# gattia/pyfocusr

Hardware: AMD Instinct MI355X
Metric: lowest-k eigenpairs/sec + KNN-correspondence wall-clock, 250k-vertex mesh pair k=5 (higher is better)
Workload: dtype f64

## Files before the change

pyfocusr_amd/csrc/pf_api.hip:

```cpp
#include <stdarg.h>
#include <stdio.h>
#include <stdlib.h>
#include <string.h>

#include <algorithm>
#include <chrono>
#include <mutex>

#include "pf_internal.h"
#include "pf_launch.h"

static thread_local char g_err[1024] = "";
static std::mutex g_ctx_mutex;
static std::vector<pf_ctx*> g_ctxs;

__global__ __launch_bounds__(PF_BLOCK) void k_copy_words(const unsigned long long* __restrict__ src, unsigned long long* __restrict__ dst,
                                                         size_t n) {
    const size_t i = (size_t)blockIdx.x * PF_BLOCK + threadIdx.x;
    if (i < n) dst[i] = src[i];
}

int pf_copy_by_kernel(hipStream_t st, const void* src, void* dst, size_t bytes) {
    if (bytes == 0) return PF_OK;
    const size_t n = (bytes + 7) / 8;
    k_copy_words<<<(unsigned)((n + PF_BLOCK - 1) / PF_BLOCK), PF_BLOCK, 0, st>>>(static_cast<const unsigned long long*>(src),
                                                                                 static_cast<unsigned long long*>(dst), n);
    PF_HIP(hipGetLastError());
    return PF_OK;
}

static pf_ctx* ctx_of_stream(hipStream_t st) {
    std::lock_guard<std::mutex> lk(g_ctx_mutex);
    for (pf_ctx* c : g_ctxs)
        if (c->stream == st || (c->stream_b && c->stream_b == st)) return c;
    return nullptr;
}

int pf_pinned_scratch(pf_ctx* c, size_t bytes, void** out, int which) {
    void*& buf = which == 2 ? c->pinned_scratch_knn : (which ? c->pinned_scratch_b : c->pinned_scratch);
    size_t& have = which == 2 ? c->pinned_scratch_knn_bytes : (which ? c->pinned_scratch_b_bytes : c->pinned_scratch_bytes);
    if (bytes > have) {
        if (buf) {
            PF_HIP(hipStreamSynchronize(c->stream));
            PF_HIP(hipHostFree(buf));
            buf = nullptr;
            have = 0;
        }
        const size_t cap = bytes > ((size_t)1 << 16) ? bytes : ((size_t)1 << 16);
        PF_HIP(hipHostMalloc(&buf, cap, hipHostMallocDefault));
        have = cap;
    }
    *out = buf;
    return PF_OK;
}

hipError_t pf_create_side_stream(hipStream_t* s, bool low) {
    int least = 0, greatest = 0;
    if (hipDeviceGetStreamPriorityRange(&least, &greatest) == hipSuccess && greatest != least) {
        return hipStreamCreateWithPriority(s, hipStreamNonBlocking, low ? least : greatest);
    }
    (void)hipGetLastError();
    return hipStreamCreateWithFlags(s, hipStreamNonBlocking);
}

hipStream_t pf_stream_b(pf_ctx* c) {
    if (!c->stream_b) {
        hipStream_t s = nullptr;
        if (pf_create_side_stream(&s, true) != hipSuccess ||
            hipEventCreateWithFlags(&c->join_ev, hipEventDisableTiming) != hipSuccess ||
            hipEventCreateWithFlags(&c->fork_ev, hipEventDisableTiming) != hipSuccess) {
            (void)hipGetLastError();
            if (s) (void)hipStreamDestroy(s);
            return nullptr;
        }
        std::lock_guard<std::mutex> lk(g_ctx_mutex);
        c->stream_b = s;
    }
    return c->stream_b;
}

hipError_t pf_malloc(hipStream_t st, void** p, size_t bytes) {
    *p = nullptr;
    pf_ctx* c = ctx_of_stream(st);
    if (!c) return hipErrorInvalidValue;
    std::lock_guard<std::mutex> lk(c->alloc_mutex);
    bytes = (std::max<size_t>(bytes, 1) + 255) & ~(size_t)255;
    const auto it = c->free_blocks.lower_bound(bytes);
    if (it != c->free_blocks.end() && it->first == bytes) {
        *p = it->second;
        c->free_blocks.erase(it);
    }
    if (!*p) {
        c->alloc_misses += 1;
        static const bool dbg_alloc = getenv("PF_DEBUG_ALLOC") != nullptr;
        const auto t_miss = std::chrono::steady_clock::now();
        hipError_t e = hipMalloc(p, bytes);
        if (dbg_alloc)
            fprintf(stderr, "libpyfocusr_hip: allocation %lld of ctx %p went to the driver: %zu bytes, %.0f us\n", (long long)c->alloc_misses,
                    (void*)c, bytes, std::chrono::duration<double, std::micro>(std::chrono::steady_clock::now() - t_miss).count());
        if (e != hipSuccess) {
            (void)hipStreamSynchronize(c->stream);
            if (c->stream_b) (void)hipStreamSynchronize(c->stream_b);
            for (auto& kv : c->free_blocks) (void)hipFree(kv.second);
            c->free_blocks.clear();
            e = hipMalloc(p, bytes);
            if (e != hipSuccess) return e;
        }
    }
    c->live_blocks[*p] = bytes;
    return hipSuccess;
}

void pf_free(hipStream_t st, void* p) {
    if (!p) return;
    if (pfl::tl_rec) {
        pfl::tl_rec->frees.emplace_back(st, p);
        return;
    }
    pf_ctx* c = ctx_of_stream(st);
    if (!c) return;
    std::lock_guard<std::mutex> lk(c->alloc_mutex);
    auto it = c->live_blocks.find(p);
    if (it == c->live_blocks.end()) return;
    c->free_blocks.emplace(it->second, p);
    c->live_blocks.erase(it);
}

namespace pfl {

void flush(Recorder& a, Recorder* b) {
    Recorder* const saved = tl_rec;
    tl_rec = nullptr;
    size_t i = 0, j = 0;
    const size_t na = a.ops.size(), nb = b ? b->ops.size() : 0;
    auto alone = [](const Op& o) { o.key ? o.run1(o, o.st) : o.call(o.st); };
    while (i < na && j < nb) {
        const Op& x = a.ops[i];
        const Op& y = b->ops[j];
        if (x.key != y.key) {
            if (!x.key) {
                alone(x);
                ++i;
                continue;
            }
            if (!y.key) {
                alone(y);
                ++j;
                continue;
            }
            break;
        }
        if (x.key && x.st == y.st && x.block.x == y.block.x && x.block.y == y.block.y && x.block.z == y.block.z) {
            x.run2(x, y, x.st);
        } else {
            alone(x);
            alone(y);
        }
        ++i, ++j;
    }
    for (; i < na; ++i) alone(a.ops[i]);
    for (; j < nb; ++j) alone(b->ops[j]);
    a.ops.clear();
    for (auto& f : a.frees) pf_free(f.first, f.second);
    a.frees.clear();
    if (b) {
        b->ops.clear();
        for (auto& f : b->frees) pf_free(f.first, f.second);
        b->frees.clear();
    }
    tl_rec = saved;
}

void flush_self() {
    if (tl_rec) flush(*tl_rec, nullptr);
}

}

// ... 199 lines not shown
```

pyfocusr_amd/csrc/pf_eigs.hip:

```cpp
#include <math.h>

#include <algorithm>
#include <vector>

#include "pf_internal.h"
#include "pf_krylov.h"

namespace {

struct DeviceOps final : pfk::Ops {
    pf_graph* g;
    explicit DeviceOps(pf_graph* graph) : g(graph) {}
    int64_t n() const override { return g->n; }
    int64_t n_isolated() const override { return g->n_isolated; }
    int32_t n_components() const override { return g->n_components; }
    int32_t n_oneway() const override { return g->n_oneway; }
    bool symmetric() const override { return g->is_symmetric; }
    double spectral_bound() const override { return g->spectral_bound; }
    int ws_ensure(int32_t slots) override { return pf_ws_ensure(g, slots); }
    int lock_nulls(int32_t op, int32_t* locked) override { return pf_lock_null_vectors(g, op, locked); }
    int orth_strict(bool on) override { return pf_orth_strict(g, on ? 1 : 0); }
    int orth_always_twice(bool on, bool strict_otherwise) override { return pf_orth_strict(g, on ? 2 : (strict_otherwise ? 1 : 0)); }
    int orth_device_passes(bool on) override { return pf_orth_device_passes(g, on ? 1 : 0); }
    int start_vector(int32_t slot, uint64_t seed) override { return pf_start_vector(g, slot, seed); }
    int orth_begin(int32_t w, int32_t first, int32_t count) override { return pf_orth_begin(g, w, first, count, 1); }
    int orth_end(double* h, double* nrm, bool* redone) override {
        PF_TRY(pf_orth_end(g, h, nrm));
        const int r = pf_orth_redone(g);
        *redone = r == 1;
        last_twice = r == 2;
        return PF_OK;
    }
    int cheb(int32_t op, int32_t src, int32_t dst, int32_t degree, double c, double e, double rho) override {
        return pf_cheb(g, op, src, dst, degree, c, e, rho);
    }
    int combine(int32_t src_first, int32_t m, const double* Y, int32_t k, int32_t dst_first) override {
        return pf_combine(g, src_first, m, Y, k, dst_first);
    }
    int combine2(int32_t src_first, int32_t m, const double* Y, int32_t k, int32_t dst_first, int32_t src_first2, int32_t dst_first2) override {
        return pf_combine2(g, src_first, m, Y, k, dst_first, src_first2, dst_first2);
    }
    int copy(int32_t src, int32_t dst, int32_t count) override { return pf_ws_copy(g, src, dst, count); }
    int spmv_multi(int32_t op, int32_t src_first, int32_t dst_first, int32_t count) override {
        return pf_spmv_multi(g, op, src_first, dst_first, count);
    }
    int gram(int32_t first_a, int32_t count_a, int32_t first_b, int32_t count_b, double* out) override {
        return pf_gram(g, first_a, count_a, first_b, count_b, out);
    }
    int resnorms(int32_t ax_first, int32_t x_first, const double* lam, int32_t count, double* out) override {
        return pf_resnorms(g, ax_first, x_first, lam, count, out);
    }
    int gram_begin(int32_t first_a, int32_t count_a, int32_t first_b, int32_t count_b, bool self_b) override {
        PF_TRY(pf_gram_begin(g, first_a, count_a, first_b, count_b, 0));
        return self_b ? pf_gram_begin(g, first_b, count_b, first_b, count_b, 1) : PF_OK;
    }
    bool orth_split(int32_t first2, int32_t split) override { return pf_orth_split(g, first2, split) == PF_OK; }
    int gram_end(double* out) override { return pf_small_end(g, out); }
    int resnorms_begin(int32_t ax_first, int32_t x_first, const double* lam, int32_t count) override {
        return pf_resnorms_begin(g, ax_first, x_first, lam, count);
    }
    int resnorms_end(double* out) override { return pf_small_end(g, out); }
    int orth_begin_pair(pfk::Ops& other, const int32_t* o) override {
        return pf_orth_begin2(g, o[0], o[1], o[2], o[3], static_cast<DeviceOps&>(other).g, o[4], o[5], o[6], o[7]);
    }
    int cheb_pair(pfk::Ops& other, const int32_t* ci, const double* cd) override {
        return pf_cheb2(g, ci[0], ci[1], ci[2], ci[3], cd[0], cd[1], cd[2], static_cast<DeviceOps&>(other).g, ci[4], ci[5], ci[6], ci[7], cd[3],
                        cd[4], cd[5]);
    }
    int orth_cheb_pair(pfk::Ops& other, const int32_t* orth, const int32_t* ci, const double* cd) override {
        return pf_orth_cheb2(g, static_cast<DeviceOps&>(other).g, orth, ci, cd);
    }
};

int ellipse_hint() {
    const char* ev = getenv("PF_EIGS_ELLIPSE");
    return ev ? atoi(ev) : -1;
}

void give_up(pf_graph* g) {
    if (!g) return;
    if (g->orth_pending >= 0) {
        std::vector<double> h((size_t)g->orth_pending + 1);
        double nrm = 0.0;
        (void)pf_orth_end(g, h.data(), &nrm);
    }
    if (g->small_pending > 0) {
        (void)hipEventSynchronize(g->small_ev);
        g->small_pending = 0;
    }
    (void)pf_download_cancel(g);
}

int finish(pf_graph* g, pfk::Solver& s, int32_t minmax, double* vals, double* vecs, double* residuals, int32_t* n_out, pf_eigs_stats* stats,
           bool async) {
    *n_out = s.n_out;
    for (int i = 0; i < s.n_out; ++i) {
        vals[i] = s.vals[(size_t)i];
        if (residuals) residuals[i] = s.residuals[(size_t)i];
    }
    if (stats) *stats = s.st;
    if (s.n_out > 0) {
        PF_TRY(pf_finalize_vectors_begin(g, s.first_slot, s.n_out, s.sym ? 1 : 0, minmax ? 1 : 0, vecs));
        if (!async) PF_TRY(pf_finalize_vectors_end(g));
    }
    return PF_OK;
}

}

extern "C" int pf_eigs_smallest_ex(pf_graph* g, int32_t n_wanted, int32_t minmax, int32_t async_download, double* vals, double* vecs,
                                   double* residuals, int32_t* n_out, pf_eigs_stats* stats_out) {
    PF_CHECK(g && vals && vecs && n_out && n_wanted >= 1, PF_E_ARG, "pf_eigs_smallest: bad argument");
    int rc = PF_OK;
    for (int attempt = 0; attempt < 3; ++attempt) {
        DeviceOps ops(g);
        pfk::Solver s;
        *n_out = 0;
        rc = s.init(&ops, n_wanted, ellipse_hint());
        if (rc == PF_OK) rc = pfk::drive_single(s);
        if (rc == PF_OK) rc = pf_sync(g->ctx);
        if (rc == PF_OK) rc = finish(g, s, minmax, vals, vecs, residuals, n_out, stats_out, async_download != 0);
        if (rc != PF_OK) give_up(g);
        if (rc != PF_E_PERSIST_TIMEOUT) break;
    }
    return rc;
}

extern "C" int pf_eigs_smallest(pf_graph* g, int32_t n_wanted, int32_t minmax, double* vals, double* vecs, int32_t* n_out,
                                pf_eigs_stats* stats_out) {
    return pf_eigs_smallest_ex(g, n_wanted, minmax, 0, vals, vecs, nullptr, n_out, stats_out);
}

extern "C" int pf_eigs_smallest2(pf_graph* ga, pf_graph* gb, int32_t n_wanted_a, int32_t n_wanted_b, int32_t minmax, int32_t async_download,
                                 double* vals_a, double* vecs_a, double* res_a, int32_t* n_out_a, pf_eigs_stats* stats_a,
                                 double* vals_b, double* vecs_b, double* res_b, int32_t* n_out_b, pf_eigs_stats* stats_b) {
    PF_CHECK(ga && gb && ga != gb && vals_a && vecs_a && n_out_a && vals_b && vecs_b && n_out_b && n_wanted_a >= 1 && n_wanted_b >= 1,
             PF_E_ARG, "pf_eigs_smallest2: bad argument");
    PF_CHECK(ga->ctx == gb->ctx, PF_E_ARG, "pf_eigs_smallest2: the two graphs must share one ctx (stream)");
    int rc = PF_OK;
    for (int attempt = 0; attempt < 3; ++attempt) {
        DeviceOps oa(ga), ob(gb);
        pfk::Solver a, b;
        *n_out_a = *n_out_b = 0;
        rc = a.init(&oa, n_wanted_a, ellipse_hint());
        if (rc == PF_OK) rc = b.init(&ob, n_wanted_b, ellipse_hint());
        if (rc == PF_OK) rc = pfk::drive_pair(a, b);
        if (rc == PF_OK) rc = pf_sync(ga->ctx);
        if (rc == PF_OK) rc = finish(ga, a, minmax, vals_a, vecs_a, res_a, n_out_a, stats_a, async_download != 0);
        if (rc == PF_OK) rc = finish(gb, b, minmax, vals_b, vecs_b, res_b, n_out_b, stats_b, async_download != 0);
        if (rc != PF_OK) {
            give_up(ga);
            give_up(gb);
        }
        if (rc != PF_E_PERSIST_TIMEOUT) break;
    }
    return rc;
}
```

pyfocusr_amd/csrc/pf_krylov.h:

```cpp
#pragma once
#include <math.h>
#include <stdint.h>
#include <stdio.h>
#include <stdlib.h>
#include <time.h>

#include <algorithm>
#include <condition_variable>
#include <memory>
#include <mutex>
#include <thread>
#include <vector>

#include "../../include/pyfocusr_hip.h"
#include "pf_dense.h"

void pf_set_error(const char* fmt, ...);

#define PFK_CHECK(cond, code, ...)       \
    do {                                 \
        if (!(cond)) {                   \
            pf_set_error(__VA_ARGS__);   \
            return (code);               \
        }                                \
    } while (0)
#define PFK_TRY(call)                \
    do {                             \
        int r_ = (call);             \
        if (r_ != PF_OK) return r_;  \
    } while (0)

namespace pfk {

const int NEED_ELLIPSE = 1000;

struct Ops {
    virtual ~Ops() {}
    bool last_twice = false;
    virtual int64_t n() const = 0;
    virtual int64_t n_isolated() const = 0;
    virtual int32_t n_components() const = 0;
    virtual int32_t n_oneway() const = 0;
    virtual bool symmetric() const = 0;
    virtual double spectral_bound() const = 0;
    virtual int ws_ensure(int32_t slots) = 0;
    virtual int lock_nulls(int32_t op, int32_t* locked) = 0;
    virtual int orth_strict(bool on) = 0;
    virtual int orth_device_passes(bool on) { return on ? PF_OK : PF_OK; }
    virtual int start_vector(int32_t slot, uint64_t seed) = 0;
    virtual int orth_begin(int32_t w, int32_t first, int32_t count) = 0;
    virtual int orth_end(double* h, double* nrm, bool* redone) = 0;
    virtual int cheb(int32_t op, int32_t src, int32_t dst, int32_t degree, double c, double e, double rho) = 0;
    virtual int combine(int32_t src_first, int32_t m, const double* Y, int32_t k, int32_t dst_first) = 0;
    virtual int combine2(int32_t src_first, int32_t m, const double* Y, int32_t k, int32_t dst_first, int32_t src_first2, int32_t dst_first2) {
        const int rc = combine(src_first, m, Y, k, dst_first);
        return rc ? rc : combine(src_first2, m, Y, k, dst_first2);
    }
    virtual int copy(int32_t src, int32_t dst, int32_t count) = 0;
    virtual int spmv_multi(int32_t op, int32_t src_first, int32_t dst_first, int32_t count) = 0;
    virtual int gram(int32_t first_a, int32_t count_a, int32_t first_b, int32_t count_b, double* out) = 0;
    virtual int resnorms(int32_t ax_first, int32_t x_first, const double* lam, int32_t count, double* out) = 0;
    virtual int gram_begin(int32_t first_a, int32_t count_a, int32_t first_b, int32_t count_b, bool self_b = false) {
        held.assign((size_t)count_a * count_b + (self_b ? (size_t)count_b * count_b : 0), 0.0);
        const int rc = gram(first_a, count_a, first_b, count_b, held.data());
        if (rc || !self_b) return rc;
        return gram(first_b, count_b, first_b, count_b, held.data() + (size_t)count_a * count_b);
    }
    virtual int gram_end(double* out) {
        std::copy(held.begin(), held.end(), out);
        return 0;
    }
    virtual int resnorms_begin(int32_t ax_first, int32_t x_first, const double* lam, int32_t count) {
        held.assign((size_t)count, 0.0);
        return resnorms(ax_first, x_first, lam, count, held.data());
    }
    virtual int resnorms_end(double* out) {
        std::copy(held.begin(), held.end(), out);
        return 0;
    }
    std::vector<double> held;
    virtual int orth_always_twice(bool on, bool strict_otherwise) {
        (void)on, (void)strict_otherwise;
        return 0;
    }
    virtual bool orth_split(int32_t first2, int32_t split) {
        (void)first2, (void)split;
        return false;
    }
    virtual int orth_begin_pair(Ops& other, const int32_t* orth ) {
        PFK_TRY(orth_begin(orth[0], orth[1], orth[2]));
        return other.orth_begin(orth[4], orth[5], orth[6]);
    }
    virtual int cheb_pair(Ops& other, const int32_t* ci , const double* cd ) {
        PFK_TRY(cheb(ci[0], ci[1], ci[2], ci[3], cd[0], cd[1], cd[2]));
        return other.cheb(ci[4], ci[5], ci[6], ci[7], cd[3], cd[4], cd[5]);
    }
    virtual int orth_cheb_pair(Ops& other, const int32_t* orth, const int32_t* ci, const double* cd) {
        PFK_TRY(orth_begin_pair(other, orth));
        return cheb_pair(other, ci, cd);
    }
};

inline double cheb_value(double lam, double c, double e, int p) {
    const double t = (c - lam) / e;
    if (fabs(t) <= 1.0) return cos(p * acos(t));
    const double s = (t > 0 || p % 2 == 0) ? 1.0 : -1.0;
    return s * cosh(p * acosh(fabs(t)));
}

inline double cheb_value_scaled(double lam, double c, double e, int p, double rho) {
    if (rho == 1.0) return cheb_value(lam, c, e, p);
    const double t = (c - lam) / e;
    if (fabs(t) <= 1.0) return cos(p * acos(t)) * exp(-p * log(rho));
    const double u = acosh(fabs(t));
    const double s = (t > 0 || p % 2 == 0) ? 1.0 : -1.0;
    return s * 0.5 * exp(p * (u - log(rho))) * (1.0 + exp(-2.0 * p * u));
}

inline double cheb_inverse(double theta, double c, double e, int p) { return c - e * cosh(acosh(std::max(theta, 1.0)) / p); }

inline void choose_filter(double cut, double hi, double strength, int max_degree, double* c, double* e, int* p) {
    cut = std::min(std::max(cut, 1e-12), 0.5 * hi);
    *c = 0.5 * (hi + cut);
    *e = 0.5 * (hi - cut);
    const double growth = acosh((*c - 0.5 * cut) / *e);
    *p = std::max(8, std::min(max_degree, (int)ceil(strength / growth)));
}

inline void choose_filter_ellipse(double cut, double half_height, double hi, double strength, int max_degree, double* c, double* e,
                                  int* p, double* rho) {
    cut = std::min(std::max(cut, 1e-12), 0.5 * hi);
    *c = 0.5 * (hi + cut);
    const double a = 0.5 * (hi - cut);
    const double b = std::min(half_height, 0.9 * a);
    *e = sqrt(a * a - b * b);
    *rho = (a + b) / *e;
    const double t = (*c - 0.5 * cut) / *e;
    const double growth = log(t + sqrt(t * t - 1.0)) - log(*rho);
    *p = std::max(8, std::min(max_degree, (int)ceil(strength / std::max(growth, 1e-12))));
}

struct Dominant {
    int q = 0, n_found = 0;
    double thr = -1.0;
    std::vector<int> order;
};

inline Dominant select_dominant(const std::vector<pfd::cplx>& ev, int n_real, int n_extra, bool count_all) {
    Dominant d;
    const int m = (int)ev.size();
    d.order.resize(m);
    for (int i = 0; i < m; ++i) d.order[i] = i;
    std::stable_sort(d.order.begin(), d.order.end(), [&](int a, int b) { return std::abs(ev[a]) > std::abs(ev[b]); });
    std::vector<char> is_real(m);
    std::vector<int> cnt(m);
    int run = 0;
    for (int i = 0; i < m; ++i) {
        const pfd::cplx z = ev[d.order[i]];
        is_real[i] = count_all || (fabs(z.imag()) <= 1e-9 * std::abs(z) && z.real() > 0);
        run += is_real[i] ? 1 : 0;
        cnt[i] = run;
    }
    int q = m;
    for (int i = 0; i < m; ++i)
        if (cnt[i] >= n_real) {
            q = i + 1;
            break;
        }
    int extra = 0;
    while (q < m && extra < n_extra) {
        const pfd::cplx z = ev[d.order[q]];
        const int step = (is_real[q] || fabs(z.imag()) <= 1e-9 * std::abs(z)) ? 1 : 2;
        if (q + step > m) break;
        q += step;
        extra += step;
    }
    if (q < m) {
        double lo = std::abs(ev[d.order[q - 1]]), nx = std::abs(ev[d.order[q]]);
        d.thr = 0.5 * (lo + nx);
        if (lo == nx) {
            q += 1;
            d.thr = q < m ? 0.5 * (std::abs(ev[d.order[q - 1]]) + std::abs(ev[d.order[q]])) : -1.0;
        }
    }
    d.q = q;
    d.n_found = m ? std::min(cnt[m - 1], n_real) : 0;
    return d;
}

enum ReqKind { REQ_NONE = 0, REQ_CHEB, REQ_ORTH, REQ_ORTH_CHEB };

struct Request {
    ReqKind kind = REQ_NONE;
    int32_t cheb_src = 0, cheb_dst = 0;
    int32_t orth_w = 0, orth_first = 0, orth_count = 0;
};

struct Solver {
    Ops* ops = nullptr;
    int32_t n_wanted = 0;
    std::vector<double> vals, residuals;
    int32_t n_out = 0, first_slot = 0;
    pf_eigs_stats st{};
    bool done = false;
    Request req;
    bool req_launched = false;
    bool sym = true;
    int32_t op = PF_OP_SYM;
    double hi = 2.0, strength = 1.8, tol = 1e-12;
    int64_t n_active = 0;
    int c0 = 0, want = 0, q_target = 0, m_max = 0, reg = 0, A0 = 0, B0 = 0;
    int out_cap = 16;
    int m_max_limit = 0;
    bool ellipse = false, interval_tried = false;
    double half_height = 0.0;
    int ellipse_tries = 0, degree_cap = 4000;
    double cut = 0.0, cut0 = 0.0, c = 0.0, e = 0.0, rho = 1.0, theta0 = 0.0, band = 1.5;
    int p = 0;
    uint64_t seed = 0;
    std::vector<double> H, b, h;
    int j = 0, q = 0, restarts = 0, resets = 0;
    bool hess = true;
    bool spec = false, near_conv = false, have_seen = false, start_pending = false;
    bool expect_final = false;
    int next_check = 0, seen_j = 0;
    double seen_worst = 0.0;
    std::vector<double> theta_re, theta_im;
    std::vector<double> U, T;
    double theta_min = 0.0, theta_absmax = 0.0;
    int n_real = 0;
    std::vector<double> res;
    bool analysis_due = false, inline_analysis = true, exhausted = false;
    int outcome = 0, analysis_rc = PF_OK;
    enum { S_TOP, S_AFTER_CHEB, S_AFTER_ORTH, S_AFTER_ANALYSIS, S_EXTRACT_B, S_EXTRACT_C, S_DONE } state = S_TOP;
    bool stepwise_extract = false, extracting = false;
    bool pro = false, pro_local = false;
    int pro_force = 0;
    double pro_thresh = 1e-9;
    std::vector<double> om_prev, om_cur;
    std::vector<double> ex_Rk;
    int ex_nk = 0;

    int init(Ops* o, int32_t wanted, int ellipse_hint = -1) {
        ops = o;
        n_wanted = wanted;
        PFK_CHECK(ops && n_wanted >= 1, PF_E_ARG, "pf_eigs_smallest: bad argument");
        sym = ops->symmetric();
        op = sym ? PF_OP_SYM : PF_OP_RW;
        hi = sym ? ops->spectral_bound() : 2.0;
        strength = 1.8;
        n_active = ops->n() - ops->n_isolated();
        vals.assign((size_t)n_wanted, 0.0);
// ... 568 lines not shown
            std::vector<double> Zs, wr, wi;
            PFK_CHECK(pfd::real_schur(HA, q, Zs, wr, wi), PF_E_DEGENERATE, "pf_eigs_smallest: QR iteration of the Rayleigh quotient failed");
            std::vector<int> all(q);
            for (int i = 0; i < q; ++i) all[i] = i;
            std::vector<pfd::cplx> Vc, lam_c;
            pfd::schur_eigenvectors(HA, Zs, q, all, Vc, lam_c);
            std::vector<int> order(q);
            for (int i = 0; i < q; ++i) order[i] = i;
            std::stable_sort(order.begin(), order.end(), [&](int a, int bb) { return lam_c[a].real() < lam_c[bb].real(); });
            int take = std::min(q_target, q);
            if (take < q && fabs(lam_c[order[take - 1]].imag()) > 1e-9 &&
                fabs(lam_c[order[take - 1]].real() - lam_c[order[take]].real()) <= 1e-9 * fabs(lam_c[order[take]].real()))
                take += 1;
            std::vector<char> is_cplx(take);
            bool any_cplx = false, above = false;
            for (int i = 0; i < take; ++i) {
                const pfd::cplx z = lam_c[order[i]];
                is_cplx[i] = fabs(z.imag()) > 1e-9 * std::max(std::abs(z), 1e-300);
                any_cplx = any_cplx || is_cplx[i];
                above = above || z.real() > cut;
            }
            (void)any_cplx;
            if (ellipse && above) return NEED_ELLIPSE;
            std::vector<int> keep;
            for (int i = 0; i < take; ++i)
                if (lam_c[order[i]].real() > 1e-10) keep.push_back(i);
            st.n_null = std::min(q_target, take) - (int)keep.size();
            nk = (int)keep.size();
            if (nk == 0) return NEED_ELLIPSE;
            nk = std::min(nk, (int)n_wanted);
            Rk.assign((size_t)q * nk, 0.0);
            for (int cidx = 0; cidx < nk; ++cidx) {
                const int col = order[keep[cidx]];
                pfd::cplx phase = 1.0;
                if (is_cplx[keep[cidx]]) {
                    int piv = 0;
                    double best = -1.0;
                    for (int r = 0; r < q; ++r)
                        if (std::abs(Vc[(size_t)r * q + col]) > best) best = std::abs(Vc[(size_t)r * q + col]), piv = r;
                    phase = std::conj(Vc[(size_t)piv * q + col]) / std::abs(Vc[(size_t)piv * q + col]);
                }
                double nrm = 0.0;
                for (int r = 0; r < q; ++r) {
                    const double v = (Vc[(size_t)r * q + col] * phase).real();
                    Rk[(size_t)r * nk + cidx] = v;
                    nrm += v * v;
                }
                nrm = sqrt(nrm);
                for (int r = 0; r < q; ++r) Rk[(size_t)r * nk + cidx] /= nrm;
                vals[cidx] = lam_c[col].real();
            }
        }
        const int X0 = B0 + q, AX0 = A0 + q;
        PFK_CHECK(X0 + nk <= 2 * reg && AX0 + nk <= reg, PF_E_STATE, "pf_eigs_smallest: workspace too small for the extraction");
        n_out = nk;
        first_slot = X0;
        ex_nk = nk;
        if (nk > 0) {
            PFK_TRY(ops->combine2(B0, q, Rk.data(), nk, X0, A0, AX0));
            PFK_TRY(ops->resnorms_begin(AX0, X0, vals.data(), nk));
        }
        return PF_OK;
    }

    int extract_c() {
        if (ex_nk > 0) {
            PFK_TRY(ops->resnorms_end(residuals.data()));
            st.max_residual = 0.0;
            for (int i = 0; i < ex_nk; ++i) st.max_residual = std::max(st.max_residual, residuals[i]);
        }
        return PF_OK;
    }

    void cheb_args(int32_t* ci, double* cd) const {
        ci[0] = op, ci[1] = req.cheb_src, ci[2] = req.cheb_dst, ci[3] = p;
        cd[0] = c, cd[1] = e, cd[2] = rho;
    }
    void orth_args(int32_t* o) const { o[0] = req.orth_w, o[1] = req.orth_first, o[2] = req.orth_count, o[3] = 1; }
    int run_cheb() { return ops->cheb(op, req.cheb_src, req.cheb_dst, p, c, e, rho); }
    int run_orth() { return ops->orth_begin(req.orth_w, req.orth_first, req.orth_count); }
};

inline int drive_single(Solver& s) {
    for (;;) {
        PFK_TRY(s.advance());
        if (s.done) return PF_OK;
        switch (s.req.kind) {
            case REQ_CHEB: PFK_TRY(s.run_cheb()); break;
            case REQ_ORTH: PFK_TRY(s.run_orth()); break;
            case REQ_ORTH_CHEB:
                PFK_TRY(s.run_orth());
                PFK_TRY(s.run_cheb());
                break;
            default: break;
        }
    }
}

struct AnalysisHelper {
    std::thread th;
    std::mutex m;
    std::condition_variable cv;
    Solver* job = nullptr;
    bool busy = false, quit = false;
    AnalysisHelper() { th = std::thread([this] { loop(); }); }
    ~AnalysisHelper() {
        {
            std::lock_guard<std::mutex> lk(m);
            quit = true;
        }
        cv.notify_all();
        th.join();
    }
    void submit(Solver* s) {
        {
            std::lock_guard<std::mutex> lk(m);
            job = s;
            busy = true;
        }
        cv.notify_all();
    }
    void wait() {
        std::unique_lock<std::mutex> lk(m);
        cv.wait(lk, [&] { return !busy; });
    }
    void loop() {
        std::unique_lock<std::mutex> lk(m);
        for (;;) {
            cv.wait(lk, [&] { return job != nullptr || quit; });
            if (quit) return;
            Solver* s = job;
            job = nullptr;
            lk.unlock();
            s->analyse();
            lk.lock();
            busy = false;
            cv.notify_all();
        }
    }
};

inline int launch_request(Solver& s) {
    switch (s.req.kind) {
        case REQ_CHEB: return s.run_cheb();
        case REQ_ORTH: return s.run_orth();
        case REQ_ORTH_CHEB:
            PFK_TRY(s.run_orth());
            return s.run_cheb();
        default: return PF_OK;
    }
}

inline int advance_pair(Solver& a, Solver& b, bool do_a, bool do_b, AnalysisHelper* helper) {
    if (do_a) PFK_TRY(a.advance());
    if (do_b) PFK_TRY(b.advance());
    auto extractions = [&]() -> int {
        for (;;) {
            bool any = false;
            if (do_a && !a.done && a.extracting) {
                PFK_TRY(a.advance());
                any = true;
            }
            if (do_b && !b.done && b.extracting) {
                PFK_TRY(b.advance());
                any = true;
            }
            if (!any) return PF_OK;
        }
    };
    PFK_TRY(extractions());
    for (;;) {
        const bool da = do_a && !a.done && a.analysis_due, db = do_b && !b.done && b.analysis_due;
        if (!da && !db) return PF_OK;
        if (da && db && helper) {
            helper->submit(&b);
            a.analyse();
            helper->wait();
        } else {
            if (da) a.analyse();
            if (db) b.analyse();
        }
        const bool ea = da && a.analysis_rc == PF_OK && a.outcome == 1, eb = db && b.analysis_rc == PF_OK && b.outcome == 1;
        if (ea != eb) {
            Solver& ex = ea ? a : b;
            Solver& other = ea ? b : a;
            const bool other_due = ea ? db : da, other_active = ea ? do_b : do_a;
            if (other_due) PFK_TRY(other.advance());
            if (other_active && !other.done && !other.analysis_due && !other.req_launched && other.req.kind != REQ_NONE) {
                PFK_TRY(launch_request(other));
                other.req_launched = true;
            }
            PFK_TRY(ex.advance());
            PFK_TRY(extractions());
            continue;
        }
        if (da) PFK_TRY(a.advance());
        if (db) PFK_TRY(b.advance());
        PFK_TRY(extractions());
    }
}

inline int drive_pair(Solver& a, Solver& b) {
    std::unique_ptr<AnalysisHelper> helper;
    if ((!a.done && !a.sym) || (!b.done && !b.sym)) {
        if (!getenv("PF_EIGS_HELPER") || atoi(getenv("PF_EIGS_HELPER")) != 0) helper.reset(new AnalysisHelper());
    }
    a.inline_analysis = b.inline_analysis = false;
    a.stepwise_extract = b.stepwise_extract = true;
    PFK_TRY(advance_pair(a, b, !a.done, !b.done, helper.get()));
    while (!a.done || !b.done) {
        if ((!a.done && a.req_launched) || (!b.done && b.req_launched)) {
            Solver& s = (!a.done && a.req_launched) ? a : b;
            s.req_launched = false;
            PFK_TRY(advance_pair(a, b, &s == &a, &s == &b, helper.get()));
            continue;
        }
        const ReqKind ka = a.done ? REQ_NONE : a.req.kind, kb = b.done ? REQ_NONE : b.req.kind;
        const bool oa = ka == REQ_ORTH || ka == REQ_ORTH_CHEB, ob = kb == REQ_ORTH || kb == REQ_ORTH_CHEB;
        int32_t orth[8], ci[8];
        double cd[6];
        if (ka == REQ_ORTH_CHEB && kb == REQ_ORTH_CHEB) {
            a.orth_args(orth);
            b.orth_args(orth + 4);
            a.cheb_args(ci, cd);
            b.cheb_args(ci + 4, cd + 3);
            PFK_TRY(a.ops->orth_cheb_pair(*b.ops, orth, ci, cd));
            PFK_TRY(advance_pair(a, b, true, true, helper.get()));
        } else if (oa || ob) {
            if (oa && ob) {
                a.orth_args(orth);
                b.orth_args(orth + 4);
                PFK_TRY(a.ops->orth_begin_pair(*b.ops, orth));
            } else {
                PFK_TRY((oa ? a : b).run_orth());
            }
            bool adv[2] = {false, false};
            int i = 0;
            for (Solver* s : {&a, &b}) {
                const ReqKind k = s->done ? REQ_NONE : s->req.kind;
                if (k == REQ_ORTH_CHEB && (s == &a ? oa : ob)) s->req.kind = REQ_CHEB;
                else if (k == REQ_ORTH) adv[i] = true;
                ++i;
            }
            PFK_TRY(advance_pair(a, b, adv[0], adv[1], helper.get()));
        } else if (ka == REQ_CHEB && kb == REQ_CHEB) {
            a.cheb_args(ci, cd);
            b.cheb_args(ci + 4, cd + 3);
            PFK_TRY(a.ops->cheb_pair(*b.ops, ci, cd));
            PFK_TRY(advance_pair(a, b, true, true, helper.get()));
        } else {
            Solver& s = ka == REQ_CHEB ? a : b;
            PFK_CHECK(!s.done && s.req.kind == REQ_CHEB, PF_E_STATE, "pf_eigs_smallest2: driver out of step");
            PFK_TRY(s.run_cheb());
            PFK_TRY(advance_pair(a, b, &s == &a, &s == &b, helper.get()));
        }
    }
    return PF_OK;
}

}
```

pyfocusr_amd/csrc/pf_operator.hip:

```cpp
#include <math.h>
#include <stdlib.h>
#include <string.h>

#include <algorithm>
#include <atomic>
#include <map>
#include <mutex>
#include <vector>

#include "pf_internal.h"

namespace {

inline unsigned nblk(int64_t n) { return (unsigned)((n + PF_BLOCK - 1) / PF_BLOCK); }

#ifndef PF_OP_BLOCK
#define PF_OP_BLOCK 256
#endif
struct OpArgs {
    const int64_t* slice_ptr;
    const int32_t* scol;
    const double* sval;
    const double* diag;
    const double* x;
    const double* prev;
    double* out;
    double alpha, shift, beta;
    unsigned n_blocks;
};

template <bool HAS_PREV>
__device__ __forceinline__ void sell_op_block(const OpArgs& a, unsigned bid) {
#pragma clang fp contract(fast)
    const unsigned per_xcd = a.n_blocks >> 3;
    const unsigned blk = (bid & 7u) * per_xcd + (bid >> 3);
    const int64_t row = (int64_t)blk * PF_OP_BLOCK + threadIdx.x;
    const int64_t s = row >> 6;
    const int lane = threadIdx.x & (PF_WAVE - 1);
    const int64_t base = a.slice_ptr[s];
    const int width = (int)((a.slice_ptr[s + 1] - base) >> 6);
    const double* __restrict__ x = a.x;
    const double xi = x[row];
    double acc = a.diag[row] * xi;
    const int pairs = width >> 1;
    const double2* __restrict__ vp2 = reinterpret_cast<const double2*>(a.sval + base) + lane;
    const int2* __restrict__ cp2 = reinterpret_cast<const int2*>(a.scol + base) + lane;
    int j = 0;
    for (; j + 2 <= pairs; j += 2) {
        const int2 c0 = cp2[(int64_t)(j + 0) * PF_WAVE], c1 = cp2[(int64_t)(j + 1) * PF_WAVE];
        const double2 v0 = vp2[(int64_t)(j + 0) * PF_WAVE], v1 = vp2[(int64_t)(j + 1) * PF_WAVE];
        const double x0 = x[c0.x], x1 = x[c0.y], x2 = x[c1.x], x3 = x[c1.y];
        acc += v0.x * x0;
        acc += v0.y * x1;
        acc += v1.x * x2;
        acc += v1.y * x3;
    }
    for (; j < pairs; ++j) {
        const int2 c0 = cp2[(int64_t)j * PF_WAVE];
        const double2 v0 = vp2[(int64_t)j * PF_WAVE];
        acc += v0.x * x[c0.x];
        acc += v0.y * x[c0.y];
    }
    if (width & 1) {
        const int64_t t = base + (int64_t)pairs * (2 * PF_WAVE) + lane;
        acc += a.sval[t] * x[a.scol[t]];
    }
    double r = a.alpha * (a.shift * xi - acc);
    if (HAS_PREV) r -= a.beta * a.prev[row];
    a.out[row] = r;
}

template <bool HAS_PREV>
__global__ __launch_bounds__(PF_OP_BLOCK) void k_sell_op(OpArgs a) {
    sell_op_block<HAS_PREV>(a, blockIdx.x);
}

__global__ __launch_bounds__(PF_OP_BLOCK) void k_sell_op_slots(OpArgs a, int64_t slot_stride) {
    a.x += (int64_t)blockIdx.y * slot_stride;
    a.out += (int64_t)blockIdx.y * slot_stride;
    sell_op_block<false>(a, blockIdx.x);
}

template <bool HAS_PREV>
__global__ __launch_bounds__(PF_OP_BLOCK) void k_sell_op2(OpArgs a, OpArgs b) {
    if (blockIdx.x < a.n_blocks) sell_op_block<HAS_PREV>(a, blockIdx.x);
    else sell_op_block<HAS_PREV>(b, blockIdx.x - a.n_blocks);
}

__global__ __launch_bounds__(PF_BLOCK) void k_dot_partial(const double* __restrict__ ws, int64_t n_pad, int32_t first,
                                                          int32_t wslot, int64_t n_chunks, double* __restrict__ partial,
                                                          int32_t self_col = -1) {
    __shared__ double red[PF_BLOCK / PF_WAVE];
    const int b = blockIdx.y;
    const int64_t chunk = blockIdx.x;
    const double* v = ws + (int64_t)(b == self_col ? wslot : first + b) * n_pad;
    const double* w = ws + (int64_t)wslot * n_pad;
    const int64_t lo = chunk * PF_DOT_CHUNK;
    const int64_t hi = lo + PF_DOT_CHUNK < n_pad ? lo + PF_DOT_CHUNK : n_pad;
    double s = 0.0;
    for (int64_t i = lo + 2 * threadIdx.x; i < hi; i += 2 * PF_BLOCK) {
        const double2 a = *reinterpret_cast<const double2*>(v + i);
        const double2 c = *reinterpret_cast<const double2*>(w + i);
        s += a.x * c.x;
        s += a.y * c.y;
    }
#pragma unroll
    for (int off = PF_WAVE / 2; off > 0; off >>= 1) s += __shfl_down(s, off, PF_WAVE);
    if ((threadIdx.x & (PF_WAVE - 1)) == 0) red[threadIdx.x / PF_WAVE] = s;
    __syncthreads();
    if (threadIdx.x == 0) partial[(int64_t)b * n_chunks + chunk] = (red[0] + red[1]) + (red[2] + red[3]);
}

__global__ __launch_bounds__(PF_WAVE) void k_dot_finish(const double* __restrict__ partial, int64_t n_chunks,
                                                        double* __restrict__ out, double* __restrict__ acc, int accumulate) {
    const int b = blockIdx.x;
    double s = 0.0;
    for (int64_t k = threadIdx.x; k < n_chunks; k += PF_WAVE) s += partial[(int64_t)b * n_chunks + k];
#pragma unroll
    for (int off = PF_WAVE / 2; off > 0; off >>= 1) s += __shfl_down(s, off, PF_WAVE);
    if (threadIdx.x == 0) {
        out[b] = s;
        if (acc) acc[b] = accumulate ? acc[b] + s : s;
    }
}

__global__ __launch_bounds__(PF_BLOCK) void k_multi_axpy(double* __restrict__ ws, int64_t n_pad, int32_t first,
                                                         int32_t count, int32_t wslot, const double* __restrict__ h) {
    const int64_t i = 2 * ((int64_t)blockIdx.x * PF_BLOCK + threadIdx.x);
    if (i >= n_pad) return;
    double2 acc = *reinterpret_cast<double2*>(ws + (int64_t)wslot * n_pad + i);
    for (int b = 0; b < count; ++b) {
        const double hb = h[b];
        const double2 v = *reinterpret_cast<const double2*>(ws + (int64_t)(first + b) * n_pad + i);
        acc.x -= hb * v.x;
        acc.y -= hb * v.y;
    }
    *reinterpret_cast<double2*>(ws + (int64_t)wslot * n_pad + i) = acc;
}

constexpr int PF_ORTH_MAX = 256;
__global__ __launch_bounds__(PF_BLOCK) void k_axpy_finishing(double* __restrict__ ws, int64_t n_pad, int32_t first, int32_t count,
                                                             int32_t wslot, const double* __restrict__ partial, int64_t n_chunks,
                                                             double* __restrict__ hsum, int accumulate) {
    __shared__ double hs[PF_ORTH_MAX];
    const int lane = threadIdx.x & (PF_WAVE - 1);
    for (int b = threadIdx.x / PF_WAVE; b < count; b += PF_BLOCK / PF_WAVE) {
        double s = 0.0;
        for (int64_t k = lane; k < n_chunks; k += PF_WAVE) s += partial[(int64_t)b * n_chunks + k];
#pragma unroll
        for (int off = PF_WAVE / 2; off > 0; off >>= 1) s += __shfl_down(s, off, PF_WAVE);
        if (lane == 0) hs[b] = s;
    }
    __syncthreads();
    if (blockIdx.x == 0)
        for (int b = threadIdx.x; b < count; b += PF_BLOCK) hsum[b] = accumulate ? hsum[b] + hs[b] : hs[b];
    const int64_t i = 2 * ((int64_t)blockIdx.x * PF_BLOCK + threadIdx.x);
    if (i >= n_pad) return;
    double2 acc = *reinterpret_cast<double2*>(ws + (int64_t)wslot * n_pad + i);
    for (int b = 0; b < count; ++b) {
        const double hb = hs[b];
        const double2 v = *reinterpret_cast<const double2*>(ws + (int64_t)(first + b) * n_pad + i);
        acc.x -= hb * v.x;
        acc.y -= hb * v.y;
    }
    *reinterpret_cast<double2*>(ws + (int64_t)wslot * n_pad + i) = acc;
}
struct OrthArgs {
    double* ws;
    int64_t n_pad, n_chunks;
    int32_t first, count, wslot, normalize;
    int32_t split, first2;
    double* partial;
    double* hsum;
    double* nrm2;
    double* host_out;
    double thresh;
    double ticket;
    int32_t pass;
    double* verdict;
    unsigned long long* counter;
    unsigned long long target;
    uint32_t* abort_flag;
    int32_t* host_abort;
};
struct OrthArgs2 {
    OrthArgs g[2];
};
__device__ __forceinline__ int32_t orth_slot(const OrthArgs& a, int b) { return b < a.split ? a.first + b : a.first2 + (b - a.split); }

template <int VB>
__global__ __launch_bounds__(PF_BLOCK) void k_orth_dots(OrthArgs2 a2) {
    __shared__ double red[VB][PF_BLOCK / PF_WAVE];
    const OrthArgs& a = a2.g[blockIdx.z];
    const int b0 = blockIdx.y * VB;
    const int64_t chunk = blockIdx.x;
    if (a.pass < 0 || b0 > a.count || chunk >= a.n_chunks) return;
    if (a.pass == 2 && *a.verdict == 0.0) return;
    const double* w = a.ws + (int64_t)a.wslot * a.n_pad;
    const int64_t lo = chunk * PF_DOT_CHUNK;
    constexpr int PAIRS = PF_DOT_CHUNK / (2 * PF_BLOCK);
    double2 cs[PAIRS], xs[VB][PAIRS];
#pragma unroll
    for (int it = 0; it < PAIRS; ++it) cs[it] = *reinterpret_cast<const double2*>(w + lo + 2 * threadIdx.x + (int64_t)it * (2 * PF_BLOCK));
#pragma unroll
    for (int u = 0; u < VB; ++u) {
        const int b = b0 + u;
        if (b > a.count) continue;
        const double* v = a.ws + (int64_t)(b == a.count ? a.wslot : orth_slot(a, b)) * a.n_pad;
#pragma unroll
        for (int it = 0; it < PAIRS; ++it) xs[u][it] = *reinterpret_cast<const double2*>(v + lo + 2 * threadIdx.x + (int64_t)it * (2 * PF_BLOCK));
    }
#pragma unroll
    for (int u = 0; u < VB; ++u) {
        if (b0 + u > a.count) continue;
        double s = 0.0;
#pragma unroll
        for (int it = 0; it < PAIRS; ++it) {
            s += xs[u][it].x * cs[it].x;
            s += xs[u][it].y * cs[it].y;
        }
#pragma unroll
        for (int off = PF_WAVE / 2; off > 0; off >>= 1) s += __shfl_down(s, off, PF_WAVE);
        if ((threadIdx.x & (PF_WAVE - 1)) == 0) red[u][threadIdx.x / PF_WAVE] = s;
    }
    __syncthreads();
    if (threadIdx.x < VB && b0 + (int)threadIdx.x <= a.count)
        a.partial[(int64_t)(b0 + threadIdx.x) * a.n_chunks + chunk] =
            (red[threadIdx.x][0] + red[threadIdx.x][1]) + (red[threadIdx.x][2] + red[threadIdx.x][3]);
}

template <int P>
__global__ __launch_bounds__(PF_BLOCK) void k_orth_project(OrthArgs2 a2) {
    __shared__ double hs[PF_ORTH_MAX + 1];
    __shared__ double s_scale, s_after, s_redo;
    const OrthArgs& a = a2.g[blockIdx.z];
    if (a.pass < 0 || 2 * (int64_t)blockIdx.x * PF_BLOCK * P >= a.n_pad) return;
    if (a.pass == 2 && *a.verdict == 0.0) return;
    const int lane = threadIdx.x & (PF_WAVE - 1);
    const int32_t count = a.count;
    for (int b = threadIdx.x / PF_WAVE; b < count + 1; b += PF_BLOCK / PF_WAVE) {
        double s = 0.0;
        for (int64_t k = lane; k < a.n_chunks; k += PF_WAVE) s += a.partial[(int64_t)b * a.n_chunks + k];
#pragma unroll
        for (int off = PF_WAVE / 2; off > 0; off >>= 1) s += __shfl_down(s, off, PF_WAVE);
        if (lane == 0) hs[b] = s;
    }
    __syncthreads();
    if (threadIdx.x == 0) {
        double sum = 0.0;
        for (int b = 0; b < count; ++b) sum += hs[b] * hs[b];
        const double before = hs[count], after = before - sum;
        const bool fine = a.pass == 2 ? (after == after) : after >= a.thresh * before;
        s_redo = fine ? (a.pass == 2 ? 2.0 : 0.0) : 1.0;
        s_after = after;
        s_scale = (fine && a.normalize && after > 1e-280) ? 1.0 / sqrt(after) : 1.0;
    }
    __syncthreads();
    if (blockIdx.x == 0) {
        const bool report = !(a.pass == 1 && s_redo != 0.0);
        for (int b = threadIdx.x; b < count; b += PF_BLOCK) {
            const double hb = a.pass == 2 ? a.hsum[b] + hs[b] : hs[b];
            a.hsum[b] = hb;
            if (report) a.host_out[b] = hb;
        }
        if (threadIdx.x == 0) {
            if (a.pass == 1) *a.verdict = s_redo;
            *a.nrm2 = s_after;
            if (report) {
                a.host_out[count] = s_after;
                a.host_out[count + 1] = s_redo;
            }
        }
        __threadfence_system();
        __syncthreads();
        if (threadIdx.x == 0 && report) {
            __hip_atomic_store(a.host_out + count + 2, a.ticket, __ATOMIC_RELEASE, __HIP_MEMORY_SCOPE_SYSTEM);
        }
// ... 84 lines not shown
            __hip_atomic_load(a.abort_flag, __ATOMIC_RELAXED, __HIP_MEMORY_SCOPE_AGENT) != 0u) {
            __hip_atomic_store(a.abort_flag, 1u, __ATOMIC_RELAXED, __HIP_MEMORY_SCOPE_AGENT);
            *a.host_abort = 1;
            return 0;
        }
        __builtin_amdgcn_s_sleep(2);
    }
    return 1;
}

constexpr int PF_ORTH_LOCAL_MAX = 4;
__global__ __launch_bounds__(PF_BLOCK) void k_orth_local(OrthArgs2 a2) {
    __shared__ double red[PF_ORTH_LOCAL_MAX + 1][PF_BLOCK / PF_WAVE];
    __shared__ double hs[PF_ORTH_LOCAL_MAX + 1];
    __shared__ double s_scale, s_after, s_redo;
    __shared__ int s_ok;
    const OrthArgs& a = a2.g[blockIdx.z];
    const int64_t chunk = blockIdx.x;
    if (a.pass < 0 || chunk >= a.n_chunks) return;
    const int32_t count = a.count;
    const int lane = threadIdx.x & (PF_WAVE - 1);
    double* w = a.ws + (int64_t)a.wslot * a.n_pad;
    const int64_t lo = chunk * PF_DOT_CHUNK;
    constexpr int PAIRS = PF_DOT_CHUNK / (2 * PF_BLOCK);
    double2 cs[PAIRS], xs[PF_ORTH_LOCAL_MAX][PAIRS];
#pragma unroll
    for (int it = 0; it < PAIRS; ++it) cs[it] = *reinterpret_cast<const double2*>(w + lo + 2 * threadIdx.x + (int64_t)it * (2 * PF_BLOCK));
#pragma unroll
    for (int u = 0; u < PF_ORTH_LOCAL_MAX; ++u) {
        const double* v = a.ws + (int64_t)orth_slot(a, u < count ? u : count - 1) * a.n_pad;
#pragma unroll
        for (int it = 0; it < PAIRS; ++it) xs[u][it] = *reinterpret_cast<const double2*>(v + lo + 2 * threadIdx.x + (int64_t)it * (2 * PF_BLOCK));
    }
#pragma unroll
    for (int u = 0; u <= PF_ORTH_LOCAL_MAX; ++u) {
        if (u > count) continue;
        double s = 0.0;
#pragma unroll
        for (int it = 0; it < PAIRS; ++it) {
            const double2 x = u == count ? cs[it] : xs[u < PF_ORTH_LOCAL_MAX ? u : 0][it];
            s += x.x * cs[it].x;
            s += x.y * cs[it].y;
        }
#pragma unroll
        for (int off = PF_WAVE / 2; off > 0; off >>= 1) s += __shfl_down(s, off, PF_WAVE);
        if (lane == 0) red[u][threadIdx.x / PF_WAVE] = s;
    }
    __syncthreads();
    if ((int)threadIdx.x <= count) {
        const double p = (red[threadIdx.x][0] + red[threadIdx.x][1]) + (red[threadIdx.x][2] + red[threadIdx.x][3]);
        __hip_atomic_store(reinterpret_cast<unsigned long long*>(a.partial) + (int64_t)threadIdx.x * a.n_chunks + chunk,
                           (unsigned long long)__double_as_longlong(p), __ATOMIC_RELAXED, __HIP_MEMORY_SCOPE_AGENT);
        asm volatile("s_waitcnt vmcnt(0)" ::: "memory");
    }
    __syncthreads();
    if (threadIdx.x == 0) s_ok = orth_meet(a, a.target);
    __syncthreads();
    if (!s_ok) return;
    {
        const int b0 = threadIdx.x / PF_WAVE, b1 = b0 + PF_BLOCK / PF_WAVE;
        double s0 = 0.0, s1 = 0.0;
        for (int64_t k = lane; k < a.n_chunks; k += PF_WAVE) {
            const double x0 = b0 < count + 1 ? __longlong_as_double((long long)__hip_atomic_load(
                                                   reinterpret_cast<unsigned long long*>(a.partial) + (int64_t)b0 * a.n_chunks + k, __ATOMIC_RELAXED,
                                                   __HIP_MEMORY_SCOPE_AGENT))
                                             : 0.0;
            const double x1 = b1 < count + 1 ? __longlong_as_double((long long)__hip_atomic_load(
                                                   reinterpret_cast<unsigned long long*>(a.partial) + (int64_t)b1 * a.n_chunks + k, __ATOMIC_RELAXED,
                                                   __HIP_MEMORY_SCOPE_AGENT))
                                             : 0.0;
            s0 += x0;
            s1 += x1;
        }
#pragma unroll
        for (int off = PF_WAVE / 2; off > 0; off >>= 1) {
            s0 += __shfl_down(s0, off, PF_WAVE);
            s1 += __shfl_down(s1, off, PF_WAVE);
        }
        if (lane == 0 && b0 < count + 1) hs[b0] = s0;
        if (lane == 0 && b1 < count + 1) hs[b1] = s1;
    }
    __syncthreads();
    if (threadIdx.x == 0) {
        double sum = 0.0;
        for (int b = 0; b < count; ++b) sum += hs[b] * hs[b];
        const double before = hs[count], after = before - sum;
        int fine = after >= a.thresh * before ? 1 : 0;
        asm volatile("" : "+v"(fine));
        s_redo = fine ? 0.0 : 1.0;
        s_after = after;
        s_scale = (fine && a.normalize && after > 1e-280) ? 1.0 / sqrt(after) : 1.0;
    }
    __syncthreads();
    if (chunk == 0) {
        for (int b = threadIdx.x; b < count; b += PF_BLOCK) {
            a.hsum[b] = hs[b];
            a.host_out[b] = hs[b];
        }
        if (threadIdx.x == 0) {
            *a.nrm2 = s_after;
            a.host_out[count] = s_after;
            a.host_out[count + 1] = s_redo;
        }
        __threadfence_system();
        __syncthreads();
        if (threadIdx.x == 0) __hip_atomic_store(a.host_out + count + 2, a.ticket, __ATOMIC_RELEASE, __HIP_MEMORY_SCOPE_SYSTEM);
    }
    const double sc = s_scale;
#pragma unroll
    for (int it = 0; it < PAIRS; ++it) {
        double2 acc = cs[it];
#pragma unroll
        for (int u = 0; u < PF_ORTH_LOCAL_MAX; ++u) {
            if (u >= count) continue;
            const double hb = hs[u];
            acc.x -= hb * xs[u][it].x;
            acc.y -= hb * xs[u][it].y;
        }
        acc.x *= sc;
        acc.y *= sc;
        *reinterpret_cast<double2*>(w + lo + 2 * threadIdx.x + (int64_t)it * (2 * PF_BLOCK)) = acc;
    }
}
__global__ __launch_bounds__(PF_BLOCK) void k_scale_finishing(double* __restrict__ x, int64_t n_pad, const double* __restrict__ partial,
                                                              int64_t n_chunks, int normalize, const double* __restrict__ hsum,
                                                              int32_t count, double* __restrict__ nrm2, double* __restrict__ host_out) {
    __shared__ double s_v;
    if (threadIdx.x < PF_WAVE) {
        double s = 0.0;
        for (int64_t k = threadIdx.x; k < n_chunks; k += PF_WAVE) s += partial[k];
#pragma unroll
        for (int off = PF_WAVE / 2; off > 0; off >>= 1) s += __shfl_down(s, off, PF_WAVE);
        if (threadIdx.x == 0) s_v = s;
    }
    __syncthreads();
    const double v = s_v;
    if (blockIdx.x == 0) {
        for (int b = threadIdx.x; b < count; b += PF_BLOCK) host_out[b] = hsum[b];
        if (threadIdx.x == 0) {
            *nrm2 = v;
            host_out[count] = v;
            host_out[count + 1] = 0.0;
        }
    }
    const int64_t i = (int64_t)blockIdx.x * PF_BLOCK + threadIdx.x;
    if (normalize && i < n_pad && v > 1e-280) x[i] *= 1.0 / sqrt(v);
}

__global__ __launch_bounds__(PF_BLOCK) void k_scale(double* __restrict__ x, int64_t n_pad, double alpha) {
    const int64_t i = (int64_t)blockIdx.x * PF_BLOCK + threadIdx.x;
    if (i < n_pad) x[i] *= alpha;
}

__global__ __launch_bounds__(PF_BLOCK) void k_scale_rsqrt(double* __restrict__ x, int64_t n_pad, const double* __restrict__ nrm2) {
    const int64_t i = (int64_t)blockIdx.x * PF_BLOCK + threadIdx.x;
    const double v = *nrm2;
    if (i < n_pad && v > 1e-280) x[i] *= 1.0 / sqrt(v);
}

__global__ __launch_bounds__(PF_BLOCK) void k_mask_isolated(double* __restrict__ x, const int32_t* __restrict__ rowptr,
                                                            const int32_t* __restrict__ perm, int64_t n) {
    const int64_t r = (int64_t)blockIdx.x * PF_BLOCK + threadIdx.x;
    if (r >= n) return;
    const int32_t i = perm[r];
    if (rowptr[i + 1] == rowptr[i]) x[r] = 0.0;
}

__global__ __launch_bounds__(PF_BLOCK) void k_start_vector(double* __restrict__ x, const double* __restrict__ smooth,
                                                           const int32_t* __restrict__ perm, const int32_t* __restrict__ perm_m,
                                                           const int32_t* __restrict__ rowptr,
                                                           int64_t n_pad, unsigned long long seed, double noise) {
    const int64_t r = (int64_t)blockIdx.x * PF_BLOCK + threadIdx.x;
    if (r >= n_pad) return;
    const int32_t i = perm[r];
    const int32_t m = perm_m[r];
    double v = 0.0;
    if (i >= 0 && rowptr[m + 1] > rowptr[m]) {
        unsigned long long z = seed + 0x9E3779B97F4A7C15ull * (unsigned long long)(i + 1);
        z = (z ^ (z >> 30)) * 0xBF58476D1CE4E5B9ull;
        z = (z ^ (z >> 27)) * 0x94D049BB133111EBull;
        z ^= z >> 31;
        const double u = (double)(z >> 11) * (1.0 / 9007199254740992.0) - 0.5;
        v = smooth[r] + noise * u;
    }
    x[r] = v;
}

__global__ __launch_bounds__(PF_BLOCK) void k_permute_in(const double* __restrict__ src_old, const int32_t* __restrict__ perm,
                                                         int64_t n_pad, double* __restrict__ dst_new) {
    const int64_t r = (int64_t)blockIdx.x * PF_BLOCK + threadIdx.x;
    if (r >= n_pad) return;
    const int32_t i = perm[r];
    dst_new[r] = i >= 0 ? src_old[i] : 0.0;
}

__global__ __launch_bounds__(PF_BLOCK) void k_permute_out(const double* __restrict__ ws, int64_t n_pad, int32_t first,
                                                          int32_t count, const int32_t* __restrict__ iperm, int64_t n,
                                                          double* __restrict__ dst_old ) {
    const int64_t i = (int64_t)blockIdx.x * PF_BLOCK + threadIdx.x;
    if (i >= n) return;
    const int64_t r = iperm[i];
    for (int c = 0; c < count; ++c) dst_old[(int64_t)c * n + i] = ws[(int64_t)(first + c) * n_pad + r];
}

__global__ __launch_bounds__(PF_BLOCK) void k_null_vector(double* __restrict__ x, const int32_t* __restrict__ label,
                                                          const int32_t* __restrict__ rowptr,
                                                          const double* __restrict__ deg, const int32_t* __restrict__ perm,
                                                          int64_t n_pad, int32_t root, int32_t sym,
                                                          const double* __restrict__ weight) {
    const int64_t r = (int64_t)blockIdx.x * PF_BLOCK + threadIdx.x;
    if (r >= n_pad) return;
    const int32_t i = perm[r];
    double v = 0.0;
    if (i >= 0 && label[i] == root && rowptr[i + 1] > rowptr[i]) v = weight ? weight[i] : (sym ? sqrt(deg[i] + 1e-8) : 1.0);
    x[r] = v;
}

constexpr int COMBINE_COLS = 8;
__global__ __launch_bounds__(PF_BLOCK) void k_combine(double* __restrict__ ws, int64_t n_pad, int32_t src_first, int32_t m,
                                                      const double* __restrict__ Y, int32_t k, int32_t c0, int32_t ncols,
                                                      int32_t dst_first, int32_t src_first2, int32_t dst_first2) {
    const int64_t i = (int64_t)blockIdx.x * PF_BLOCK + threadIdx.x;
    if (i >= n_pad) return;
    if (blockIdx.y) src_first = src_first2, dst_first = dst_first2;
    double acc[COMBINE_COLS];
#pragma unroll
    for (int c = 0; c < COMBINE_COLS; ++c) acc[c] = 0.0;
    for (int b = 0; b < m; ++b) {
        const double v = ws[(int64_t)(src_first + b) * n_pad + i];
        const double* yr = Y + (int64_t)b * k + c0;
#pragma unroll
        for (int c = 0; c < COMBINE_COLS; ++c)
            if (c < ncols) acc[c] += v * yr[c];
    }
#pragma unroll
    for (int c = 0; c < COMBINE_COLS; ++c)
        if (c < ncols) ws[(int64_t)(dst_first + c0 + c) * n_pad + i] = acc[c];
}

__global__ __launch_bounds__(PF_BLOCK) void k_resnorm_partial(const double* __restrict__ ax, const double* __restrict__ x,
                                                              double lam, int64_t n_pad, int64_t n_chunks,
                                                              double* __restrict__ partial) {
    __shared__ double red[PF_BLOCK / PF_WAVE];
    const int64_t lo = (int64_t)blockIdx.x * PF_DOT_CHUNK;
    const int64_t hi = lo + PF_DOT_CHUNK < n_pad ? lo + PF_DOT_CHUNK : n_pad;
    double s = 0.0;
    for (int64_t i = lo + threadIdx.x; i < hi; i += PF_BLOCK) {
        const double r = ax[i] - lam * x[i];
        s += r * r;
    }
#pragma unroll
    for (int off = PF_WAVE / 2; off > 0; off >>= 1) s += __shfl_down(s, off, PF_WAVE);
    if ((threadIdx.x & (PF_WAVE - 1)) == 0) red[threadIdx.x / PF_WAVE] = s;
    __syncthreads();
    if (threadIdx.x == 0) partial[blockIdx.x] = (red[0] + red[1]) + (red[2] + red[3]);
}

__global__ __launch_bounds__(PF_BLOCK) void k_gram_partial(const double* __restrict__ ws, int64_t n_pad, int32_t first_a, int32_t first_b,
                                                           int32_t count_b, int64_t n_chunks, double* __restrict__ partial) {
    __shared__ double red[PF_BLOCK / PF_WAVE];
    const int p = blockIdx.y;
    const int i = p / count_b, j = p - i * count_b;
    const double* v = ws + (int64_t)(first_b + j) * n_pad;
    const double* w = ws + (int64_t)(first_a + i) * n_pad;
    const int64_t lo = (int64_t)blockIdx.x * PF_DOT_CHUNK;
    const int64_t hi = lo + PF_DOT_CHUNK < n_pad ? lo + PF_DOT_CHUNK : n_pad;
    double s = 0.0;
    for (int64_t r = lo + 2 * threadIdx.x; r < hi; r += 2 * PF_BLOCK) {
        const double2 a = *reinterpret_cast<const double2*>(v + r);
        const double2 c = *reinterpret_cast<const double2*>(w + r);
        s += a.x * c.x;
        s += a.y * c.y;
    }
#pragma unroll
    for (int off = PF_WAVE / 2; off > 0; off >>= 1) s += __shfl_down(s, off, PF_WAVE);
    if ((threadIdx.x & (PF_WAVE - 1)) == 0) red[threadIdx.x / PF_WAVE] = s;
    __syncthreads();
    if (threadIdx.x == 0) partial[(int64_t)p * n_chunks + blockIdx.x] = (red[0] + red[1]) + (red[2] + red[3]);
}

constexpr int PF_RESNORMS_MAX = 64;
struct LamArgs {
    double lam[PF_RESNORMS_MAX];
};
__global__ __launch_bounds__(PF_BLOCK) void k_resnorms_partial(const double* __restrict__ ws, int64_t n_pad, int32_t ax_first,
                                                               int32_t x_first, LamArgs la, int64_t n_chunks,
                                                               double* __restrict__ partial) {
    __shared__ double red[PF_BLOCK / PF_WAVE];
    const int b = blockIdx.y;
    const double* ax = ws + (int64_t)(ax_first + b) * n_pad;
    const double* x = ws + (int64_t)(x_first + b) * n_pad;
    const double lam = la.lam[b];
    const int64_t lo = (int64_t)blockIdx.x * PF_DOT_CHUNK;
    const int64_t hi = lo + PF_DOT_CHUNK < n_pad ? lo + PF_DOT_CHUNK : n_pad;
    double s = 0.0;
    for (int64_t i = lo + threadIdx.x; i < hi; i += PF_BLOCK) {
        const double r = ax[i] - lam * x[i];
        s += r * r;
    }
#pragma unroll
    for (int off = PF_WAVE / 2; off > 0; off >>= 1) s += __shfl_down(s, off, PF_WAVE);
    if ((threadIdx.x & (PF_WAVE - 1)) == 0) red[threadIdx.x / PF_WAVE] = s;
    __syncthreads();
    if (threadIdx.x == 0) partial[(int64_t)b * n_chunks + blockIdx.x] = (red[0] + red[1]) + (red[2] + red[3]);
}

struct VecStats {
    double sumsq, vmin, vmax, absmax, at_absmax;
    int64_t arg;
};

__device__ __forceinline__ void stats_merge(VecStats& a, const VecStats& b) {
    a.sumsq += b.sumsq;
    a.vmin = fmin(a.vmin, b.vmin);
    a.vmax = fmax(a.vmax, b.vmax);
    if (b.absmax > a.absmax || (b.absmax == a.absmax && b.arg < a.arg)) {
        a.absmax = b.absmax;
        a.at_absmax = b.at_absmax;
        a.arg = b.arg;
    }
}

__device__ __forceinline__ VecStats stats_shfl(const VecStats& v, int off) {
    VecStats o;
    o.sumsq = __shfl_down(v.sumsq, off, PF_WAVE);
    o.vmin = __shfl_down(v.vmin, off, PF_WAVE);
    o.vmax = __shfl_down(v.vmax, off, PF_WAVE);
    o.absmax = __shfl_down(v.absmax, off, PF_WAVE);
    o.at_absmax = __shfl_down(v.at_absmax, off, PF_WAVE);
    o.arg = __shfl_down(v.arg, off, PF_WAVE);
    return o;
}

__global__ __launch_bounds__(PF_BLOCK) void k_vec_stats_partial(const double* __restrict__ ws, int64_t n_pad, int64_t n,
                                                                int32_t first, const double* __restrict__ sg,
                                                                const int32_t* __restrict__ perm, const int32_t* __restrict__ perm_m,
                                                                int32_t from_sym, int64_t n_chunks, VecStats* __restrict__ partial) {
    __shared__ VecStats red[PF_BLOCK / PF_WAVE];
    const int b = blockIdx.y;
    const double* x = ws + (int64_t)(first + b) * n_pad;
    const int64_t lo = (int64_t)blockIdx.x * PF_DOT_CHUNK;
    const int64_t hi0 = lo + PF_DOT_CHUNK;
    const int64_t hi = hi0 < n ? hi0 : n;
    VecStats st{0.0, INFINITY, -INFINITY, -1.0, 0.0, (int64_t)1 << 62};
    for (int64_t r = lo + threadIdx.x; r < hi; r += PF_BLOCK) {
        const int64_t i = perm[r];
        double v = x[r];
        if (from_sym) v *= sg[perm_m[r]];
        VecStats e{v * v, v, v, fabs(v), v, i};
        stats_merge(st, e);
    }
#pragma unroll
    for (int off = PF_WAVE / 2; off > 0; off >>= 1) {
        VecStats o = stats_shfl(st, off);
        stats_merge(st, o);
    }
    if ((threadIdx.x & (PF_WAVE - 1)) == 0) red[threadIdx.x / PF_WAVE] = st;
    __syncthreads();
    if (threadIdx.x == 0) {
        VecStats t = red[0];
        stats_merge(t, red[1]);
        stats_merge(t, red[2]);
        stats_merge(t, red[3]);
        partial[(int64_t)b * n_chunks + blockIdx.x] = t;
    }
}

__global__ __launch_bounds__(PF_WAVE) void k_vec_stats_finish(const VecStats* __restrict__ partial, int64_t n_chunks,
                                                              VecStats* __restrict__ out) {
    const int b = blockIdx.x;
    VecStats st{0.0, INFINITY, -INFINITY, -1.0, 0.0, (int64_t)1 << 62};
    for (int64_t k = threadIdx.x; k < n_chunks; k += PF_WAVE) stats_merge(st, partial[(int64_t)b * n_chunks + k]);
#pragma unroll
    for (int off = PF_WAVE / 2; off > 0; off >>= 1) {
        VecStats o = stats_shfl(st, off);
        stats_merge(st, o);
    }
    if (threadIdx.x == 0) out[b] = st;
}

__global__ void k_vec_params(const VecStats* __restrict__ fin, int32_t count, int32_t minmax, double* __restrict__ params) {
    for (int c = threadIdx.x; c < count; c += blockDim.x) {
        const VecStats s = fin[c];
        const double sgn = s.at_absmax < 0.0 ? -1.0 : 1.0;
        const double scale = sgn / sqrt(s.sumsq);
        const double vmin = (sgn > 0 ? s.vmin : s.vmax) * scale;
        const double vmax = (sgn > 0 ? s.vmax : s.vmin) * scale;
        params[4 * c + 0] = scale;
        params[4 * c + 1] = minmax ? vmin : 0.0;
        params[4 * c + 2] = minmax ? (vmax - vmin) : 0.0;
        params[4 * c + 3] = minmax ? 0.5 : 0.0;
    }
}

__global__ __launch_bounds__(PF_BLOCK) void k_vec_apply(const double* __restrict__ ws, int64_t n_pad, int64_t n,
                                                        int32_t first, int32_t count, const double* __restrict__ sg,
                                                        const int32_t* __restrict__ iperm, const int32_t* __restrict__ mrank,
                                                        int32_t from_sym, const double* __restrict__ params, double* __restrict__ out) {
    const int64_t i = (int64_t)blockIdx.x * PF_BLOCK + threadIdx.x;
    if (i >= n) return;
    const int64_t r = iperm[i];
    const double s = from_sym ? sg[mrank ? mrank[i] : i] : 1.0;
    for (int c = 0; c < count; ++c) {
        const double scale = params[4 * c + 0], off = params[4 * c + 1], ptp = params[4 * c + 2], half = params[4 * c + 3];
        double v = (ws[(int64_t)(first + c) * n_pad + r] * s) * scale;
        if (ptp != 0.0) v = (v - off) / ptp - half;
        out[i * count + c] = v;
    }
}

__global__ __launch_bounds__(PF_BLOCK) void k_final_rows(const double* __restrict__ fin, const int64_t* __restrict__ rows, int64_t n_rows,
                                                         int32_t fc, double* __restrict__ out) {
    const int64_t e = (int64_t)blockIdx.x * PF_BLOCK + threadIdx.x;
    if (e >= n_rows * fc) return;
    const int64_t t = e / fc;
    out[e] = fin[rows[t] * fc + (e - t * fc)];
}

__global__ __launch_bounds__(PF_BLOCK) void k_fill_mean_filter(const int32_t* __restrict__ rowptr, const int32_t* __restrict__ col,
                                                               const double* __restrict__ w, const double* __restrict__ deg,
                                                               const int32_t* __restrict__ perm, const int32_t* __restrict__ iperm,
                                                               const int32_t* __restrict__ key, int64_t n_pad,
                                                               const int64_t* __restrict__ slice_ptr,
                                                               int32_t* __restrict__ mf_col, double* __restrict__ mf_val) {
    const int64_t row = (int64_t)blockIdx.x * PF_BLOCK + threadIdx.x;
    if (row >= n_pad) return;
    const int64_t s = row / PF_WAVE;
    const int lane = (int)(row & (PF_WAVE - 1));
    const int32_t width = (int32_t)((slice_ptr[s + 1] - slice_ptr[s]) / PF_WAVE) + 1;
    const int64_t base = slice_ptr[s] + (int64_t)PF_WAVE * s;
    const int32_t i = perm[row];
    int32_t e = 0;
    if (i >= 0) {
        const double dinv = 1.0 / (1.0 + deg[i]);
        bool diag_done = false;
        const int32_t ki = key ? key[i] : i;
        for (int32_t a = rowptr[i + 1] - 1; a >= rowptr[i]; --a) {
            const int32_t j = col[a];
            if (!diag_done && (key ? key[j] : j) < ki) {
                mf_col[base + (int64_t)PF_WAVE * e + lane] = (int32_t)row;
                mf_val[base + (int64_t)PF_WAVE * e + lane] = dinv;
                ++e;
                diag_done = true;
            }
            mf_col[base + (int64_t)PF_WAVE * e + lane] = iperm[j];
            mf_val[base + (int64_t)PF_WAVE * e + lane] = dinv * w[a];
            ++e;
        }
        if (!diag_done) {
            mf_col[base + (int64_t)PF_WAVE * e + lane] = (int32_t)row;
            mf_val[base + (int64_t)PF_WAVE * e + lane] = dinv;
            ++e;
        }
    }
    for (; e < width; ++e) {
        mf_col[base + (int64_t)PF_WAVE * e + lane] = (int32_t)row;
        mf_val[base + (int64_t)PF_WAVE * e + lane] = 0.0;
    }
}

template <int NC>
__global__ __launch_bounds__(PF_BLOCK) void k_mean_filter(const int64_t* __restrict__ slice_ptr, const int32_t* __restrict__ mf_col,
                                                          const double* __restrict__ mf_val, const int32_t* __restrict__ perm,
                                                          int64_t n_pad, int32_t ncols, const double* __restrict__ in,
                                                          double* __restrict__ out) {
    const int64_t row = (int64_t)blockIdx.x * PF_BLOCK + threadIdx.x;
    if (row >= n_pad) return;
    const int64_t s = row / PF_WAVE;
    const int lane = (int)(row & (PF_WAVE - 1));
    const int32_t width = (int32_t)((slice_ptr[s + 1] - slice_ptr[s]) / PF_WAVE) + 1;
    const int64_t base = slice_ptr[s] + (int64_t)PF_WAVE * s + lane;
    const bool real = perm[row] >= 0;
    if constexpr (NC > 0) {
        double acc[NC];
#pragma unroll
        for (int c = 0; c < NC; ++c) acc[c] = 0.0;
        for (int32_t e = 0; e < width; ++e) {
            const int64_t j = mf_col[base + (int64_t)PF_WAVE * e];
            const double v = mf_val[base + (int64_t)PF_WAVE * e];
            if (v != 0.0 || j != row) {
#pragma unroll
                for (int c = 0; c < NC; ++c) acc[c] += v * in[j * NC + c];
            }
        }
#pragma unroll
        for (int c = 0; c < NC; ++c) out[row * NC + c] = real ? acc[c] : 0.0;
    } else {
        for (int32_t c = 0; c < ncols; ++c) {
            double acc = 0.0;
            for (int32_t e = 0; e < width; ++e) {
                const double v = mf_val[base + (int64_t)PF_WAVE * e];
                const int64_t j = mf_col[base + (int64_t)PF_WAVE * e];
                if (v != 0.0 || j != row) acc += v * in[j * ncols + c];
            }
            out[row * ncols + c] = real ? acc : 0.0;
        }
    }
}

__global__ __launch_bounds__(PF_BLOCK) void k_rows_in(const double* __restrict__ src, const int32_t* __restrict__ perm, int64_t n_pad,
                                                      int32_t ncols, double* __restrict__ dst) {
    const int64_t t = (int64_t)blockIdx.x * PF_BLOCK + threadIdx.x;
    if (t >= n_pad * ncols) return;
    const int64_t row = t / ncols;
    const int32_t old = perm[row];
    dst[t] = old >= 0 ? src[(int64_t)old * ncols + (t - row * ncols)] : 0.0;
}
__global__ __launch_bounds__(PF_BLOCK) void k_rows_out(const double* __restrict__ src, const int32_t* __restrict__ iperm, int64_t n,
                                                       int32_t ncols, double* __restrict__ dst) {
    const int64_t t = (int64_t)blockIdx.x * PF_BLOCK + threadIdx.x;
    if (t >= n * ncols) return;
    const int64_t old = t / ncols;
    dst[t] = src[(int64_t)iperm[old] * ncols + (t - old * ncols)];
}

__global__ __launch_bounds__(PF_BLOCK) void k_rows_to_new(const int64_t* __restrict__ old_idx, const int32_t* __restrict__ iperm,
                                                          int64_t cnt, int32_t* __restrict__ new_idx) {
    const int64_t t = (int64_t)blockIdx.x * PF_BLOCK + threadIdx.x;
    if (t < cnt) new_idx[t] = iperm[old_idx[t]];
}
__global__ __launch_bounds__(PF_BLOCK) void k_rows_gather(const double* __restrict__ x, const int32_t* __restrict__ idx, int64_t cnt,
                                                          double* __restrict__ out) {
    const int64_t t = (int64_t)blockIdx.x * PF_BLOCK + threadIdx.x;
    if (t < cnt) out[t] = x[idx[t]];
}
__global__ __launch_bounds__(PF_BLOCK) void k_rows_scatter(double* __restrict__ x, const int32_t* __restrict__ idx, int64_t cnt,
                                                           const double* __restrict__ in) {
    const int64_t t = (int64_t)blockIdx.x * PF_BLOCK + threadIdx.x;
    if (t < cnt) x[idx[t]] = in[t];
}
__global__ __launch_bounds__(PF_BLOCK) void k_rows_gather2(const double* __restrict__ xa, const double* __restrict__ xb,
                                                           const int32_t* __restrict__ idx, int64_t cnt, int64_t stride,
                                                           double* __restrict__ out) {
    const int64_t t = (int64_t)blockIdx.x * PF_BLOCK + threadIdx.x;
    if (t >= cnt) return;
    const int32_t r = idx[t];
    out[t] = xa[r];
    if (xb) out[stride + t] = xb[r];
}
__global__ __launch_bounds__(PF_BLOCK) void k_rows_scatter2(double* __restrict__ xa, double* __restrict__ xb,
                                                            const int32_t* __restrict__ idx, const int64_t* __restrict__ off,
                                                            int64_t cnt, int64_t stride, const double* __restrict__ src) {
    const int64_t t = (int64_t)blockIdx.x * PF_BLOCK + threadIdx.x;
    if (t >= cnt) return;
    const int32_t r = idx[t];
    const int64_t o = off[t];
    xa[r] = src[o];
    if (xb) xb[r] = src[o + stride];
}
__global__ __launch_bounds__(PF_BLOCK) void k_rows_fill(double* __restrict__ x, const int32_t* __restrict__ idx, int64_t cnt,
                                                        double value) {
    const int64_t t = (int64_t)blockIdx.x * PF_BLOCK + threadIdx.x;
    if (t < cnt) x[idx[t]] = value;
}

int stage_ensure(pf_graph* g, int64_t elems) {
    if (elems <= g->stage_cap) return PF_OK;
    pf_free(g->ctx->stream, g->stage);
    g->stage = nullptr;
    g->stage_cap = 0;
    PF_HIP(pf_malloc(g->ctx->stream, (void**)&g->stage, sizeof(double) * (size_t)elems));
    g->stage_cap = elems;
    return PF_OK;
}

int check_slots(pf_graph* g, int32_t first, int32_t count, const char* who) {
    PF_CHECK(g != nullptr, PF_E_ARG, "%s: graph is NULL", who);
    PF_HIP(hipSetDevice(g->ctx->device));
    PF_CHECK(first >= 0 && count >= 0 && first + count <= g->n_slots, PF_E_ARG, "%s: slots [%d,%d) outside workspace of %d",
             who, first, first + count, g->n_slots);
    return PF_OK;
}

const double* op_values(pf_graph* g, int32_t op) {
    if (op == PF_OP_RW) return g->sval_rw;
    if (op == PF_OP_SYM) return g->sval_sym;
    return nullptr;
}

OpArgs op_args(pf_graph* g, const double* vals, const double* x, const double* prev, double* out, double alpha, double shift,
               double beta) {
    return OpArgs{g->slice_ptr, g->scol, vals, g->diag, x, prev, out, alpha, shift, beta, (unsigned)(g->n_pad / PF_OP_BLOCK)};
}

int64_t op_bytes(const pf_graph* g) {
    return 12 * (g->nnz_w + g->n - g->n_isolated) + 20 * g->n + 4;
}

int launch_op(pf_graph* g, const double* vals, const double* x, const double* prev, double* out, double alpha, double shift,
              double beta) {
    hipStream_t st = g->ctx->stream;
    const OpArgs a = op_args(g, vals, x, prev, out, alpha, shift, beta);
    if (prev)
        k_sell_op<true><<<a.n_blocks, PF_OP_BLOCK, 0, st>>>(a);
    else
        k_sell_op<false><<<a.n_blocks, PF_OP_BLOCK, 0, st>>>(a);
    PF_HIP(hipGetLastError());
    return PF_OK;
}

int launch_op2(pf_graph* ga, const OpArgs& a, const OpArgs& b, bool has_prev) {
    hipStream_t st = ga->ctx->stream;
    if (has_prev)
        k_sell_op2<true><<<a.n_blocks + b.n_blocks, PF_OP_BLOCK, 0, st>>>(a, b);
    else
        k_sell_op2<false><<<a.n_blocks + b.n_blocks, PF_OP_BLOCK, 0, st>>>(a, b);
    PF_HIP(hipGetLastError());
    return PF_OK;
}

struct ChebRun {
    pf_graph* g;
    const double* vals;
    const double* src;
    double* dst;
    int32_t degree;
    double c, e, rho;
    const double* yp = nullptr;
    const double* yc = nullptr;
    int32_t done = 0;

    int32_t left() const { return degree - done; }
    double* free_tmp(int which) const {
        for (int t = 0; t < PF_WS_TMPS; ++t) {
            double* b = pf_tmp(g, t);
            if (b != yp && b != yc && which-- == 0) return b;
        }
        return nullptr;
    }
    OpArgs first() {
        double* target = degree == 1 ? dst : pf_tmp(g, 0);
        const OpArgs a = op_args(g, vals, src, nullptr, target, 1.0 / (e * rho), c, 0.0);
        yp = src, yc = target, done = 1;
        return a;
    }
    OpArgs single() {
        double* target = left() == 1 ? dst : free_tmp(0);
        const OpArgs a = op_args(g, vals, yc, yp, target, 2.0 / (e * rho), c, 1.0 / (rho * rho));
        yp = yc, yc = target, done += 1;
        return a;
    }
};

struct OpTimer {
    pf_ctx* c;
    int64_t launches;
    double bytes;
    bool on;
    int64_t persist_steps = 0;
    double lds_bytes = 0.0;
    hipEvent_t e0 = nullptr, e1 = nullptr;
    OpTimer(pf_ctx* ctx, int64_t n, double b) : c(ctx), launches(n), bytes(b), on(ctx->timing) {
        if (on && ctx->timing_stride > 1) on = (ctx->timing_count++ % ctx->timing_stride) == 0;
        if (!on) return;
        if (c->spans_pending.size() >= 4096) (void)pf_timing_collect(c);
        if (!c->spans_free.empty()) {
            e0 = c->spans_free.back().first;
            e1 = c->spans_free.back().second;
            c->spans_free.pop_back();
        } else if (hipEventCreate(&e0) != hipSuccess || hipEventCreate(&e1) != hipSuccess) {
            on = false;
            return;
        }
        hipEventRecord(e0, c->stream);
    }
    int finish() {
        if (!on) return PF_OK;
        PF_HIP(hipEventRecord(e1, c->stream));
        c->spans_pending.push_back({e0, e1, launches, bytes, persist_steps, lds_bytes});
        return PF_OK;
    }
};

int small_to_host(pf_graph* g, const double* d_src, double* out, size_t count) {
    pf_ctx* c = g->ctx;
    hipStream_t st = c->stream;
    const size_t bytes = sizeof(double) * count;
    void* pin = nullptr;
    if (bytes <= ((size_t)1 << 16) && pf_pinned_scratch(c, bytes, &pin) == PF_OK) {
        PF_TRY(pf_copy_by_kernel(st, d_src, pin, bytes));
        PF_HIP(hipStreamSynchronize(st));
        memcpy(out, pin, bytes);
        return PF_OK;
    }
    PF_HIP(hipMemcpyAsync(out, d_src, bytes, hipMemcpyDeviceToHost, st));
    PF_HIP(hipStreamSynchronize(st));
    return PF_OK;
}

int dots_device(pf_graph* g, int32_t w, int32_t first, int32_t count, double* d_out, double* d_acc, int accumulate) {
    hipStream_t st = g->ctx->stream;
    PF_TRY(pf_reduce_ensure(g, count));
    dim3 grid((unsigned)g->n_chunks, (unsigned)count);
    k_dot_partial<<<grid, PF_BLOCK, 0, st>>>(g->ws, g->n_pad, first, w, g->n_chunks, g->partials);
    PF_HIP(hipGetLastError());
    k_dot_finish<<<(unsigned)count, PF_WAVE, 0, st>>>(g->partials, g->n_chunks, d_out, d_acc, accumulate);
    PF_HIP(hipGetLastError());
    return PF_OK;
}

}

int pf_reduce_ensure(pf_graph* g, int32_t count) {
    if (count > g->partial_cap) {
        pf_free(g->ctx->stream, g->partials);
        g->partials = nullptr;
        const int32_t cap = std::max(count, 64);
        PF_HIP(pf_malloc(g->ctx->stream, (void**)&g->partials, sizeof(VecStats) * (size_t)cap * (size_t)(g->n_chunks + 1)));
        g->partial_cap = cap;
    }
    if (count > g->coef_cap) {
        pf_free(g->ctx->stream, g->coef);
        g->coef = nullptr;
        const int32_t cap = std::max(count, 64);
        PF_HIP(pf_malloc(g->ctx->stream, (void**)&g->coef, sizeof(double) * 8 * (size_t)cap));
        g->coef_cap = cap;
    }
    return PF_OK;
}

extern "C" {

int pf_ws_ensure(pf_graph* g, int32_t n_slots) {
    PF_CHECK(g != nullptr && n_slots > 0, PF_E_ARG, "pf_ws_ensure: bad argument");
    if (n_slots <= g->n_slots) return PF_OK;
    PF_HIP(hipSetDevice(g->ctx->device));
    hipStream_t st = g->ctx->stream;
    double* nw = nullptr;
    const size_t bytes = sizeof(double) * (size_t)(n_slots + PF_WS_TMPS) * (size_t)g->n_pad;
    PF_HIP(pf_malloc(st, (void**)&nw, bytes));
    PF_HIP(hipMemsetAsync(nw, 0, bytes, st));
    if (g->ws && g->n_slots > 0)
        PF_HIP(hipMemcpyAsync(nw, g->ws, sizeof(double) * (size_t)g->n_slots * g->n_pad, hipMemcpyDeviceToDevice, st));
    pf_free(st, g->ws);
    g->ws = nw;
    g->n_slots = n_slots;
    return PF_OK;
}

int pf_ws_upload(pf_graph* g, int32_t slot, const double* x) {
    PF_TRY(check_slots(g, slot, 1, "pf_ws_upload"));
    PF_CHECK(x != nullptr, PF_E_ARG, "pf_ws_upload: x is NULL");
    hipStream_t st = g->ctx->stream;
    PF_TRY(stage_ensure(g, g->n));
    PF_HIP(hipMemcpyAsync(g->stage, x, sizeof(double) * g->n, hipMemcpyHostToDevice, st));
    k_permute_in<<<nblk(g->n_pad), PF_BLOCK, 0, st>>>(g->stage, g->perm, g->n_pad, pf_slot(g, slot));
    PF_HIP(hipGetLastError());
    PF_HIP(hipStreamSynchronize(st));
    return PF_OK;
}

int pf_ws_download(pf_graph* g, int32_t first, int32_t count, double* out) {
    PF_TRY(check_slots(g, first, count, "pf_ws_download"));
    PF_CHECK(out != nullptr, PF_E_ARG, "pf_ws_download: out is NULL");
    if (count == 0) return PF_OK;
    hipStream_t st = g->ctx->stream;
    PF_TRY(stage_ensure(g, (int64_t)count * g->n));
    k_permute_out<<<nblk(g->n), PF_BLOCK, 0, st>>>(g->ws, g->n_pad, first, count, g->iperm, g->n, g->stage);
    PF_HIP(hipGetLastError());
    PF_HIP(hipMemcpyAsync(out, g->stage, sizeof(double) * (size_t)count * g->n, hipMemcpyDeviceToHost, st));
    PF_HIP(hipStreamSynchronize(st));
    return pf_persist_check(g->ctx);
}

int pf_ws_copy(pf_graph* g, int32_t src, int32_t dst, int32_t count) {
    PF_TRY(check_slots(g, src, count, "pf_ws_copy"));
    PF_TRY(check_slots(g, dst, count, "pf_ws_copy"));
    PF_CHECK(src + count <= dst || dst + count <= src || src == dst, PF_E_ARG, "pf_ws_copy: overlapping ranges");
    if (src == dst || count == 0) return PF_OK;
    PF_HIP(hipMemcpyAsync(pf_slot(g, dst), pf_slot(g, src), sizeof(double) * (size_t)count * g->n_pad,
                          hipMemcpyDeviceToDevice, g->ctx->stream));
    return PF_OK;
}

int pf_mask_isolated(pf_graph* g, int32_t slot) {
    PF_TRY(check_slots(g, slot, 1, "pf_mask_isolated"));
    if (g->n_isolated == 0) return PF_OK;
    k_mask_isolated<<<nblk(g->n), PF_BLOCK, 0, g->ctx->stream>>>(pf_slot(g, slot), g->rowptr, g->perm_m, g->n);
    PF_HIP(hipGetLastError());
    return PF_OK;
}

int pf_start_vector(pf_graph* g, int32_t slot, uint64_t seed) {
    PF_TRY(check_slots(g, slot, 1, "pf_start_vector"));
    k_start_vector<<<nblk(g->n_pad), PF_BLOCK, 0, g->ctx->stream>>>(pf_slot(g, slot), g->smooth, g->perm, g->perm_m, g->rowptr, g->n_pad,
                                                                    (unsigned long long)seed, 0.5);
    PF_HIP(hipGetLastError());
    return PF_OK;
}

int pf_lock_null_vectors(pf_graph* g, int32_t op, int32_t* n_locked) {
    PF_CHECK(g != nullptr && n_locked != nullptr, PF_E_ARG, "pf_lock_null_vectors: NULL argument");
    PF_HIP(hipSetDevice(g->ctx->device));
    PF_CHECK(op == PF_OP_RW || (op == PF_OP_SYM && g->is_symmetric), PF_E_ARG,
             "pf_lock_null_vectors: operator %d not available (W symmetric: %d)", op, g->is_symmetric);
    const int32_t nc = g->n_components;
    PF_TRY(pf_ws_ensure(g, nc + 1));
    hipStream_t st = g->ctx->stream;
    PF_TRY(pf_reduce_ensure(g, 1));
    for (int32_t c = 0; c < nc; ++c) {
        k_null_vector<<<nblk(g->n_pad), PF_BLOCK, 0, st>>>(pf_slot(g, c), g->label, g->rowptr, g->deg, g->perm_m, g->n_pad,
                                                          g->roots[c], op == PF_OP_SYM && !g->unit_g, g->is_cotan ? g->cot_sqrtm : nullptr);
        PF_HIP(hipGetLastError());
        PF_TRY(dots_device(g, c, c, 1, g->coef, nullptr, 0));
        k_scale_rsqrt<<<nblk(g->n_pad), PF_BLOCK, 0, st>>>(pf_slot(g, c), g->n_pad, g->coef);
        PF_HIP(hipGetLastError());
    }
    *n_locked = nc;
    return PF_OK;
}

int pf_spmv(pf_graph* g, int32_t op, int32_t src, int32_t dst) {
    PF_TRY(check_slots(g, src, 1, "pf_spmv"));
    PF_TRY(check_slots(g, dst, 1, "pf_spmv"));
    const double* vals = op_values(g, op);
    PF_CHECK(vals != nullptr && src != dst, PF_E_ARG, "pf_spmv: operator %d unavailable or src == dst", op);
    OpTimer t(g->ctx, 1, (double)op_bytes(g));
    PF_TRY(launch_op(g, vals, pf_slot(g, src), nullptr, pf_slot(g, dst), -1.0, 0.0, 0.0));
    return t.finish();
}

int pf_spmv_multi(pf_graph* g, int32_t op, int32_t src_first, int32_t dst_first, int32_t count) {
    PF_CHECK(count >= 0, PF_E_ARG, "pf_spmv_multi: negative count");
    PF_TRY(check_slots(g, src_first, count, "pf_spmv_multi"));
    PF_TRY(check_slots(g, dst_first, count, "pf_spmv_multi"));
    const double* vals = op_values(g, op);
    PF_CHECK(vals != nullptr && (src_first + count <= dst_first || dst_first + count <= src_first), PF_E_ARG,
             "pf_spmv_multi: operator %d unavailable or the slot ranges overlap", op);
    if (count == 0) return PF_OK;
    OpTimer t(g->ctx, count, (double)count * (double)op_bytes(g));
    {
        const OpArgs a = op_args(g, vals, pf_slot(g, src_first), nullptr, pf_slot(g, dst_first), -1.0, 0.0, 0.0);
        k_sell_op_slots<<<dim3(a.n_blocks, (unsigned)count), PF_OP_BLOCK, 0, g->ctx->stream>>>(a, g->n_pad);
        PF_HIP(hipGetLastError());
    }
    return t.finish();
}

int pf_cheb(pf_graph* g, int32_t op, int32_t src, int32_t dst, int32_t degree, double c, double e, double rho) {
    PF_TRY(check_slots(g, src, 1, "pf_cheb"));
    PF_TRY(check_slots(g, dst, 1, "pf_cheb"));
    const double* vals = op_values(g, op);
    PF_CHECK(vals != nullptr && src != dst, PF_E_ARG, "pf_cheb: operator %d unavailable or src == dst", op);
    PF_CHECK(degree >= 1 && e > 0.0 && rho >= 1.0, PF_E_ARG, "pf_cheb: degree %d / half-width %g / rho %g invalid", degree, e, rho);
    OpTimer t(g->ctx, degree, (double)degree * op_bytes(g));
    {
        const pf_persist_args pa{g, vals, pf_slot(g, src), pf_slot(g, dst), degree, c, e, rho};
        int done = 0;
        PF_TRY(pf_persist_cheb(&pa, nullptr, &done, &t.lds_bytes));
        if (done) {
            t.launches = 1;
            t.persist_steps = degree;
            return t.finish();
        }
    }
    ChebRun r{g, vals, pf_slot(g, src), pf_slot(g, dst), degree, c, e, rho};
    int64_t launches = 1;
    {
        const OpArgs a = r.first();
        PF_TRY(launch_op(g, a.sval, a.x, a.prev, a.out, a.alpha, a.shift, a.beta));
    }
    while (r.left() > 0) {
        const OpArgs a = r.single();
        PF_TRY(launch_op(g, a.sval, a.x, a.prev, a.out, a.alpha, a.shift, a.beta));
        ++launches;
    }
    t.launches = launches;
    return t.finish();
}

int pf_cheb2(pf_graph* ga, int32_t op_a, int32_t src_a, int32_t dst_a, int32_t degree_a, double c_a, double e_a, double rho_a,
             pf_graph* gb, int32_t op_b, int32_t src_b, int32_t dst_b, int32_t degree_b, double c_b, double e_b, double rho_b) {
    PF_TRY(check_slots(ga, src_a, 1, "pf_cheb2"));
    PF_TRY(check_slots(ga, dst_a, 1, "pf_cheb2"));
    PF_TRY(check_slots(gb, src_b, 1, "pf_cheb2"));
    PF_TRY(check_slots(gb, dst_b, 1, "pf_cheb2"));
    PF_CHECK(ga != gb && ga->ctx == gb->ctx, PF_E_ARG, "pf_cheb2: the two graphs must differ and share one ctx (stream)");
    const double* va = op_values(ga, op_a);
    const double* vb = op_values(gb, op_b);
    PF_CHECK(va && vb && src_a != dst_a && src_b != dst_b, PF_E_ARG, "pf_cheb2: operator unavailable or src == dst");
    PF_CHECK(degree_a >= 1 && degree_b >= 1 && e_a > 0.0 && e_b > 0.0 && rho_a >= 1.0 && rho_b >= 1.0, PF_E_ARG,
             "pf_cheb2: bad degree / half-width / rho");
    OpTimer t(ga->ctx, std::max(degree_a, degree_b), (double)degree_a * op_bytes(ga) + (double)degree_b * op_bytes(gb));
    {
        const pf_persist_args pa{ga, va, pf_slot(ga, src_a), pf_slot(ga, dst_a), degree_a, c_a, e_a, rho_a};
        const pf_persist_args pb{gb, vb, pf_slot(gb, src_b), pf_slot(gb, dst_b), degree_b, c_b, e_b, rho_b};
        int done = 0;
        PF_TRY(pf_persist_cheb(&pa, &pb, &done, &t.lds_bytes));
        if (done) {
            t.launches = 1;
            t.persist_steps = degree_a + degree_b;
            return t.finish();
        }
        int done_a = 0, done_b = 0;
        PF_TRY(pf_persist_cheb(&pa, nullptr, &done_a, &t.lds_bytes, false));
        PF_TRY(pf_persist_cheb(&pb, nullptr, &done_b, &t.lds_bytes, false));
        if (done_a || done_b) {
            t.launches = done_a + done_b;
            t.persist_steps = (done_a ? degree_a : 0) + (done_b ? degree_b : 0);
            for (int q = 0; q < 2; ++q) {
                if (q == 0 ? done_a : done_b) continue;
                ChebRun r = q == 0 ? ChebRun{ga, va, pf_slot(ga, src_a), pf_slot(ga, dst_a), degree_a, c_a, e_a, rho_a}
                                   : ChebRun{gb, vb, pf_slot(gb, src_b), pf_slot(gb, dst_b), degree_b, c_b, e_b, rho_b};
                OpArgs a = r.first();
                PF_TRY(launch_op(r.g, a.sval, a.x, a.prev, a.out, a.alpha, a.shift, a.beta));
                ++t.launches;
                while (r.left() > 0) {
                    a = r.single();
                    PF_TRY(launch_op(r.g, a.sval, a.x, a.prev, a.out, a.alpha, a.shift, a.beta));
                    ++t.launches;
                }
            }
            return t.finish();
        }
    }
    ChebRun ra{ga, va, pf_slot(ga, src_a), pf_slot(ga, dst_a), degree_a, c_a, e_a, rho_a};
    ChebRun rb{gb, vb, pf_slot(gb, src_b), pf_slot(gb, dst_b), degree_b, c_b, e_b, rho_b};
    int64_t launches = 1;
    {
        const OpArgs a = ra.first(), b = rb.first();
        PF_TRY(launch_op2(ga, a, b, false));
    }
    while (ra.left() > 0 || rb.left() > 0) {
        if (ra.left() > 0 && rb.left() > 0) {
            const OpArgs a = ra.single(), b = rb.single();
            PF_TRY(launch_op2(ga, a, b, true));
        } else {
            ChebRun& r = ra.left() > 0 ? ra : rb;
            const OpArgs a = r.single();
            PF_TRY(launch_op(r.g, a.sval, a.x, a.prev, a.out, a.alpha, a.shift, a.beta));
        }
        ++launches;
    }
    t.launches = launches;
    return t.finish();
}

int pf_orth_cheb2(pf_graph* ga, pf_graph* gb, const int32_t* orth, const int32_t* cheb_i, const double* cheb_d) {
    PF_CHECK(ga && gb && orth && cheb_i && cheb_d, PF_E_ARG, "pf_orth_cheb2: NULL argument");
    PF_TRY(pf_orth_begin2(ga, orth[0], orth[1], orth[2], orth[3], gb, orth[4], orth[5], orth[6], orth[7]));
    return pf_cheb2(ga, cheb_i[0], cheb_i[1], cheb_i[2], cheb_i[3], cheb_d[0], cheb_d[1], cheb_d[2], gb, cheb_i[4], cheb_i[5], cheb_i[6],
                    cheb_i[7], cheb_d[3], cheb_d[4], cheb_d[5]);
}

int pf_dots(pf_graph* g, int32_t w, int32_t first, int32_t count, double* out) {
    PF_TRY(check_slots(g, w, 1, "pf_dots"));
    PF_TRY(check_slots(g, first, count, "pf_dots"));
    PF_CHECK(out != nullptr, PF_E_ARG, "pf_dots: out is NULL");
    if (count == 0) return PF_OK;
    PF_TRY(pf_reduce_ensure(g, count));
    PF_TRY(dots_device(g, w, first, count, g->coef, nullptr, 0));
    return small_to_host(g, g->coef, out, (size_t)count);
}

static std::atomic<int> g_orth_one_launch{-1};

static int64_t orth_local_capacity(int device) {
    static std::mutex m;
    static std::map<int, int64_t> cap;
    std::lock_guard<std::mutex> lk(m);
    auto it = cap.find(device);
    if (it != cap.end()) return it->second;
    int64_t c = 0;
    const char* e = getenv("PF_ORTH_LOCAL");
    if (!(e && e[0] == '0')) {
        int per_cu = 0;
        hipDeviceProp_t prop;
        if (hipOccupancyMaxActiveBlocksPerMultiprocessor(&per_cu, reinterpret_cast<const void*>(k_orth_local), PF_BLOCK, 0) == hipSuccess &&
            hipGetDeviceProperties(&prop, device) == hipSuccess)
            c = (int64_t)per_cu * prop.multiProcessorCount;
        else
            (void)hipGetLastError();
    }
    cap[device] = c;
    return c;
}

static int orth_meetings_prepare(pf_graph* g, OrthArgs& a, unsigned long long arrivals, hipStream_t st) {
    pf_ctx* ctx = g->ctx;
    const uint64_t epoch = pf_persist_abort_epoch();
    if (!g->orth_counter) PF_HIP(pf_malloc(st, (void**)&g->orth_counter, sizeof(unsigned long long)));
    if (g->orth_epoch != epoch) {
        PF_HIP(hipMemsetAsync(g->orth_counter, 0, sizeof(unsigned long long), st));
        g->orth_arrivals = 0;
        g->orth_epoch = epoch;
    }
    g->orth_arrivals += arrivals;
    a.counter = g->orth_counter;
    a.target = g->orth_arrivals;
    a.abort_flag = ctx->persist_sync;
    a.host_abort = ctx->persist_abort;
    return PF_OK;
}

static int orth_launch_pass(OrthArgs2& a2, int ng, int64_t n_chunks, int64_t n_pad, int32_t count, hipStream_t st, pf_graph* const* gs = nullptr) {
    bool local = gs != nullptr && count <= PF_ORTH_LOCAL_MAX && count >= 1;
    for (int q = 0; q < ng && local; ++q) local = a2.g[q].pass == 0 && a2.g[q].count <= PF_ORTH_LOCAL_MAX && a2.g[q].count >= 1;
    if (local && g_orth_one_launch.load() != 0 && pf_persist_trusted() && n_chunks * ng <= orth_local_capacity(gs[0]->ctx->device)) {
        PF_TRY(pf_persist_sync_ensure(gs[0]->ctx));
        for (int q = 0; q < ng; ++q) PF_TRY(orth_meetings_prepare(gs[q], a2.g[q], (unsigned long long)gs[q]->n_chunks, st));
        k_orth_local<<<dim3((unsigned)n_chunks, 1u, (unsigned)ng), PF_BLOCK, 0, st>>>(a2);
        PF_HIP(hipGetLastError());
        return PF_OK;
    }
    if (n_pad >= 400000) {
        k_orth_dots<4><<<dim3((unsigned)n_chunks, (unsigned)((count + 1 + 3) / 4), (unsigned)ng), PF_BLOCK, 0, st>>>(a2);
        PF_HIP(hipGetLastError());
        k_orth_project<8><<<dim3((unsigned)(n_pad / (2 * PF_BLOCK * 8)), 1u, (unsigned)ng), PF_BLOCK, 0, st>>>(a2);
    } else {
        k_orth_dots<1><<<dim3((unsigned)n_chunks, (unsigned)(count + 1), (unsigned)ng), PF_BLOCK, 0, st>>>(a2);
        PF_HIP(hipGetLastError());
        k_orth_project<1><<<dim3(nblk(n_pad / 2), 1u, (unsigned)ng), PF_BLOCK, 0, st>>>(a2);
    }
    PF_HIP(hipGetLastError());
    return PF_OK;
}

static int orth_prepare(pf_graph* g, int32_t w, int32_t first, int32_t count, int32_t normalize) {
    const int32_t split_req = g->orth_split, first2_req = g->orth_first2;
    g->orth_split = -1;
    PF_TRY(check_slots(g, w, 1, "pf_orth_begin"));
    if (split_req < 0) PF_TRY(check_slots(g, first, count, "pf_orth_begin"));
    PF_CHECK(g->orth_pending < 0, PF_E_STATE, "pf_orth_begin: a previous pf_orth_begin has not been collected");
    g->orth_split_now = -1;
    if (split_req >= 0) {
        const int32_t split = split_req, first2 = first2_req;
        PF_CHECK(split <= count && count > 0 && count < PF_ORTH_MAX, PF_E_ARG, "pf_orth_split: %d of %d vectors in the first range", split, count);
        PF_TRY(check_slots(g, first, split, "pf_orth_begin"));
        PF_TRY(check_slots(g, first2, count - split, "pf_orth_begin"));
        PF_CHECK((w < first || w >= first + split) && (w < first2 || w >= first2 + count - split), PF_E_ARG, "pf_orth_begin: w inside the basis ranges");
        PF_CHECK(first + split <= first2 || first2 + count - split <= first, PF_E_ARG, "pf_orth_split: overlapping ranges");
        g->orth_split_now = split;
        g->orth_first2_now = first2;
    } else {
        PF_CHECK(w < first || w >= first + count, PF_E_ARG, "pf_orth_begin: w inside the basis range");
    }
    hipStream_t st = g->ctx->stream;
    PF_TRY(pf_reduce_ensure(g, count + 1));
    if (count + 1 > g->orth_host_cap || !g->orth_host) {
        pf_ctx* c = g->ctx;
        if (g->orth_host) {
            PF_HIP(hipStreamSynchronize(st));
            c->pinned_pool.emplace_back(g->orth_host_cap, g->orth_host);
            g->orth_host = nullptr;
        }
        const int32_t cap = std::max(count + 1, 64);
        for (size_t i = 0; i < c->pinned_pool.size(); ++i)
            if (c->pinned_pool[i].first >= cap) {
                g->orth_host_cap = c->pinned_pool[i].first;
                g->orth_host = c->pinned_pool[i].second;
                c->pinned_pool.erase(c->pinned_pool.begin() + (long)i);
                break;
            }
        if (!g->orth_host) {
            PF_HIP(hipHostMalloc((void**)&g->orth_host, sizeof(double) * (size_t)(cap + 2), hipHostMallocDefault));
            g->orth_host_cap = cap;
        }
    }
    if (!g->orth_ev) {
        pf_ctx* c = g->ctx;
        if (!c->event_pool.empty()) {
            g->orth_ev = c->event_pool.back();
            c->event_pool.pop_back();
        } else {
            PF_HIP(hipEventCreateWithFlags(&g->orth_ev, hipEventDisableTiming));
        }
    }
    g->orth_host[count + 1] = 0.0;
    g->orth_host[count + 2] = 0.0;
    g->orth_ticket = 0.0;
    g->orth_w = w, g->orth_first = first, g->orth_normalize = normalize ? 1 : 0;
    return PF_OK;
}

static OrthArgs orth_args(pf_graph* g, int32_t w, int32_t first, int32_t count, int32_t normalize) {
    OrthArgs a{};
    a.ws = g->ws;
    a.n_pad = g->n_pad;
    a.n_chunks = g->n_chunks;
    a.first = first, a.count = count, a.wslot = w, a.normalize = normalize ? 1 : 0;
    a.split = g->orth_split_now >= 0 ? g->orth_split_now : count;
    a.first2 = g->orth_first2_now;
    a.partial = g->partials;
    a.hsum = g->coef + g->coef_cap;
    a.nrm2 = g->coef + 2 * g->coef_cap;
    a.host_out = g->orth_host;
    a.thresh = g->orth_thresh;
    g->orth_serial += 1.0;
    a.ticket = g->orth_serial;
    g->orth_ticket = a.ticket;
    a.pass = g->orth_device_passes ? 1 : 0;
    a.verdict = g->coef + 3 * g->coef_cap;
    return a;
}

int pf_orth_begin(pf_graph* g, int32_t w, int32_t first, int32_t count, int32_t normalize) {
    PF_TRY(orth_prepare(g, w, first, count, normalize));
    hipStream_t st = g->ctx->stream;
    const int32_t cap = g->coef_cap;
    double* hpass = g->coef;
    double* hsum = g->coef + cap;
    double* nrm2 = g->coef + 2 * cap;
    if (count > 0 && count < PF_ORTH_MAX) {
        OrthArgs2 a2{};
        a2.g[0] = orth_args(g, w, first, count, normalize);
        pf_graph* const one[1] = {g};
        PF_TRY(orth_launch_pass(a2, 1, g->n_chunks, g->n_pad, count, st, one));
        if (a2.g[0].pass == 1) {
            a2.g[0].pass = 2;
            PF_TRY(orth_launch_pass(a2, 1, g->n_chunks, g->n_pad, count, st));
        }
    } else if (count == 0) {
        k_dot_partial<<<dim3((unsigned)g->n_chunks, 1u), PF_BLOCK, 0, st>>>(g->ws, g->n_pad, w, w, g->n_chunks, g->partials);
        PF_HIP(hipGetLastError());
        k_scale_finishing<<<nblk(g->n_pad), PF_BLOCK, 0, st>>>(pf_slot(g, w), g->n_pad, g->partials, g->n_chunks, normalize ? 1 : 0,
                                                              hsum, count, nrm2, g->orth_host);
        PF_HIP(hipGetLastError());
    } else {
        for (int pass = 0; pass < 2; ++pass) {
            PF_TRY(dots_device(g, w, first, count, hpass, hsum, pass));
            k_multi_axpy<<<nblk(g->n_pad / 2), PF_BLOCK, 0, st>>>(g->ws, g->n_pad, first, count, w, hpass);
            PF_HIP(hipGetLastError());
        }
        PF_TRY(dots_device(g, w, w, 1, nrm2, nullptr, 0));
        if (normalize) {
            k_scale_rsqrt<<<nblk(g->n_pad), PF_BLOCK, 0, st>>>(pf_slot(g, w), g->n_pad, nrm2);
            PF_HIP(hipGetLastError());
        }
        PF_HIP(hipMemcpyAsync(g->orth_host, hsum, sizeof(double) * count, hipMemcpyDeviceToHost, st));
        PF_HIP(hipMemcpyAsync(g->orth_host + count, nrm2, sizeof(double), hipMemcpyDeviceToHost, st));
    }
    if (g->orth_ticket == 0.0) PF_HIP(hipEventRecord(g->orth_ev, st));
    g->orth_wait = g->orth_ev;
    g->orth_pending = count;
    return PF_OK;
}

int pf_orth_begin2(pf_graph* ga, int32_t w_a, int32_t first_a, int32_t count_a, int32_t normalize_a, pf_graph* gb, int32_t w_b,
                   int32_t first_b, int32_t count_b, int32_t normalize_b) {
    PF_CHECK(ga != nullptr && gb != nullptr && ga != gb, PF_E_ARG, "pf_orth_begin2: two different graphs are needed");
    if (ga->ctx != gb->ctx || count_a <= 0 || count_b <= 0 || count_a >= PF_ORTH_MAX || count_b >= PF_ORTH_MAX) {
        PF_TRY(pf_orth_begin(ga, w_a, first_a, count_a, normalize_a));
        return pf_orth_begin(gb, w_b, first_b, count_b, normalize_b);
    }
    PF_TRY(orth_prepare(ga, w_a, first_a, count_a, normalize_a));
    PF_TRY(orth_prepare(gb, w_b, first_b, count_b, normalize_b));
    hipStream_t st = ga->ctx->stream;
    OrthArgs2 a2{};
    a2.g[0] = orth_args(ga, w_a, first_a, count_a, normalize_a);
    a2.g[1] = orth_args(gb, w_b, first_b, count_b, normalize_b);
    const int64_t chunks2 = std::max(ga->n_chunks, gb->n_chunks), pad2 = std::max(ga->n_pad, gb->n_pad);
    const int32_t count2 = std::max(count_a, count_b);
    pf_graph* const two[2] = {ga, gb};
    PF_TRY(orth_launch_pass(a2, 2, chunks2, pad2, count2, st, two));
    if (a2.g[0].pass == 1 || a2.g[1].pass == 1) {
        for (int q = 0; q < 2; ++q) a2.g[q].pass = a2.g[q].pass == 1 ? 2 : -1;
        PF_TRY(orth_launch_pass(a2, 2, chunks2, pad2, count2, st));
    }
    ga->orth_wait = ga->orth_ev;
    gb->orth_wait = gb->orth_ev;
    ga->orth_pending = count_a;
    gb->orth_pending = count_b;
    return PF_OK;
}

int pf_orth_end(pf_graph* g, double* h, double* nrm) {
    PF_CHECK(g != nullptr && nrm != nullptr, PF_E_ARG, "pf_orth_end: NULL argument");
    PF_CHECK(g->orth_pending >= 0, PF_E_STATE, "pf_orth_end: no pf_orth_begin in flight");
    const int32_t count = g->orth_pending;
    PF_CHECK(h != nullptr || count == 0, PF_E_ARG, "pf_orth_end: h is NULL");
    PF_HIP(hipSetDevice(g->ctx->device));
    if (g->orth_ticket != 0.0) {
        volatile double* ticket = g->orth_host + count + 2;
        bool got = false;
        for (uint64_t spin = 0;; ++spin) {
            if (__atomic_load_n(reinterpret_cast<volatile uint64_t*>(ticket), __ATOMIC_ACQUIRE) ==
                *reinterpret_cast<const uint64_t*>(&g->orth_ticket)) {
                got = true;
                break;
            }
            if ((spin & 0xfff) == 0xfff) {
                const hipError_t q = hipStreamQuery(g->ctx->stream);
                if (q == hipSuccess) {
                    got = __atomic_load_n(reinterpret_cast<volatile uint64_t*>(ticket), __ATOMIC_ACQUIRE) ==
                          *reinterpret_cast<const uint64_t*>(&g->orth_ticket);
                    break;
                }
                if (q != hipErrorNotReady) {
                    g->orth_pending = -1;
                    PF_HIP(q);
                }
            }
            __builtin_ia32_pause();
        }
        if (!got) {
            g->orth_pending = -1;
            PF_TRY(pf_persist_check(g->ctx));
            PF_CHECK(false, PF_E_HIP, "pf_orth_end: the Gram-Schmidt step never reported (launch failure?)");
        }
    } else {
        PF_HIP(hipEventSynchronize(g->orth_wait));
    }
    g->orth_pending = -1;
    g->orth_redone = 0;
    PF_TRY(pf_persist_check(g->ctx));
    g->orth_twice = g->orth_host[count + 1] == 2.0 ? 1 : 0;
    if (g->orth_host[count + 1] == 1.0) {
        hipStream_t st = g->ctx->stream;
        double* hsum = g->coef + g->coef_cap;
        double* nrm2 = g->coef + 2 * g->coef_cap;
        const int32_t w = g->orth_w, first = g->orth_first;
        const int32_t split = g->orth_split_now >= 0 ? g->orth_split_now : count;
        if (split > 0) {
            k_dot_partial<<<dim3((unsigned)g->n_chunks, (unsigned)split), PF_BLOCK, 0, st>>>(g->ws, g->n_pad, first, w, g->n_chunks, g->partials);
            PF_HIP(hipGetLastError());
        }
        if (count > split) {
            k_dot_partial<<<dim3((unsigned)g->n_chunks, (unsigned)(count - split)), PF_BLOCK, 0, st>>>(g->ws, g->n_pad, g->orth_first2_now, w, g->n_chunks,
                                                                                                   g->partials + (size_t)split * g->n_chunks);
            PF_HIP(hipGetLastError());
        }
        if (split > 0) {
            k_axpy_finishing<<<nblk(g->n_pad / 2), PF_BLOCK, 0, st>>>(g->ws, g->n_pad, first, split, w, g->partials, g->n_chunks, hsum, 1);
            PF_HIP(hipGetLastError());
        }
        if (count > split) {
            k_axpy_finishing<<<nblk(g->n_pad / 2), PF_BLOCK, 0, st>>>(g->ws, g->n_pad, g->orth_first2_now, count - split, w,
                                                                      g->partials + (size_t)split * g->n_chunks, g->n_chunks, hsum + split, 1);
            PF_HIP(hipGetLastError());
        }
        k_dot_partial<<<dim3((unsigned)g->n_chunks, 1u), PF_BLOCK, 0, st>>>(g->ws, g->n_pad, w, w, g->n_chunks, g->partials);
        PF_HIP(hipGetLastError());
        k_scale_finishing<<<nblk(g->n_pad), PF_BLOCK, 0, st>>>(pf_slot(g, w), g->n_pad, g->partials, g->n_chunks, g->orth_normalize,
                                                              hsum, count, nrm2, g->orth_host);
        PF_HIP(hipGetLastError());
        PF_HIP(hipStreamSynchronize(st));
        PF_TRY(pf_persist_check(g->ctx));
        g->orth_redone = 1;
    }
    for (int32_t b = 0; b < count; ++b) h[b] = g->orth_host[b];
    const double v = g->orth_host[count];
    *nrm = sqrt(v > 0.0 ? v : 0.0);
    return PF_OK;
}

int pf_orth_strict(pf_graph* g, int32_t on) {
    PF_CHECK(g != nullptr, PF_E_ARG, "pf_orth_strict: NULL graph");
    g->orth_thresh = on >= 2 ? 4.0 : (on ? 0.5 : 0.09);
    return PF_OK;
}

int pf_orth_device_passes(pf_graph* g, int32_t on) {
    PF_CHECK(g != nullptr, PF_E_ARG, "pf_orth_device_passes: NULL graph");
    g->orth_device_passes = on ? 1 : 0;
    return PF_OK;
}

int pf_orth_one_launch(int32_t on) {
    g_orth_one_launch.store(on < 0 ? -1 : (on ? 1 : 0));
    return PF_OK;
}

int pf_orth_split(pf_graph* g, int32_t first2, int32_t split) {
    PF_CHECK(g != nullptr && split >= 0 && first2 >= 0, PF_E_ARG, "pf_orth_split: bad argument");
    g->orth_split = split;
    g->orth_first2 = first2;
    return PF_OK;
}

int pf_orth_redone(pf_graph* g) {
    PF_CHECK(g != nullptr, PF_E_ARG, "pf_orth_redone: NULL graph");
    return g->orth_redone ? 1 : (g->orth_twice ? 2 : 0);
}

int pf_orth(pf_graph* g, int32_t w, int32_t first, int32_t count, double* h, double* nrm) {
    PF_CHECK(nrm != nullptr && (h != nullptr || count == 0), PF_E_ARG, "pf_orth: NULL output");
    PF_TRY(pf_orth_begin(g, w, first, count, 0));
    return pf_orth_end(g, h, nrm);
}

int pf_scale(pf_graph* g, int32_t slot, double alpha) {
    PF_TRY(check_slots(g, slot, 1, "pf_scale"));
    k_scale<<<nblk(g->n_pad), PF_BLOCK, 0, g->ctx->stream>>>(pf_slot(g, slot), g->n_pad, alpha);
    PF_HIP(hipGetLastError());
    return PF_OK;
}

int pf_combine(pf_graph* g, int32_t src_first, int32_t m, const double* Y, int32_t k, int32_t dst_first) {
    return pf_combine2(g, src_first, m, Y, k, dst_first, -1, -1);
}

}

int pf_combine2(pf_graph* g, int32_t src_first, int32_t m, const double* Y, int32_t k, int32_t dst_first, int32_t src_first2,
                int32_t dst_first2) {
    PF_TRY(check_slots(g, src_first, m, "pf_combine"));
    PF_TRY(check_slots(g, dst_first, k, "pf_combine"));
    PF_CHECK(Y != nullptr && m > 0 && k > 0, PF_E_ARG, "pf_combine: bad argument");
    PF_CHECK(src_first + m <= dst_first || dst_first + k <= src_first, PF_E_ARG, "pf_combine: overlapping ranges");
    const bool two = src_first2 >= 0;
    if (two) {
        PF_TRY(check_slots(g, src_first2, m, "pf_combine"));
        PF_TRY(check_slots(g, dst_first2, k, "pf_combine"));
        PF_CHECK((src_first2 + m <= dst_first2 || dst_first2 + k <= src_first2) && (dst_first + k <= dst_first2 || dst_first2 + k <= dst_first) &&
                     (src_first + m <= dst_first2 || dst_first2 + k <= src_first) && (src_first2 + m <= dst_first || dst_first + k <= src_first2),
                 PF_E_ARG, "pf_combine: overlapping ranges");
    }
    pf_ctx* ctx = g->ctx;
    hipStream_t st = ctx->stream;
    double* dY = nullptr;
    PF_HIP(pf_malloc(st, (void**)&dY, sizeof(double) * (size_t)m * k));
    const size_t bytes = sizeof(double) * (size_t)m * k;
    const void* src = Y;
    bool staged = false;
    if (bytes <= PF_STAGE_BYTES) {
        if (!ctx->stage_ring) {
            if (hipHostMalloc(&ctx->stage_ring, (size_t)PF_STAGE_SLOTS * PF_STAGE_BYTES, hipHostMallocDefault) != hipSuccess) {
                (void)hipGetLastError();
                ctx->stage_ring = nullptr;
            } else {
                for (int i = 0; i < PF_STAGE_SLOTS; ++i) ctx->stage_ev[i] = nullptr;
            }
        }
        if (ctx->stage_ring) {
            const int slot = ctx->stage_next;
            ctx->stage_next = (slot + 1) % PF_STAGE_SLOTS;
            bool ok = true;
            if (!ctx->stage_ev[slot]) ok = hipEventCreateWithFlags(&ctx->stage_ev[slot], hipEventDisableTiming) == hipSuccess;
            else ok = hipEventSynchronize(ctx->stage_ev[slot]) == hipSuccess;
            if (ok) {
                void* dst = static_cast<unsigned char*>(ctx->stage_ring) + (size_t)slot * PF_STAGE_BYTES;
                memcpy(dst, Y, bytes);
                src = dst;
                staged = true;
                hipError_t es = hipMemcpyAsync(dY, src, bytes, hipMemcpyHostToDevice, st);
                if (es == hipSuccess) es = hipEventRecord(ctx->stage_ev[slot], st);
                if (es != hipSuccess) {
                    pf_free(st, dY);
                    PF_HIP(es);
                }
            } else {
                (void)hipGetLastError();
            }
        }
    }
    hipError_t e = staged ? hipSuccess : hipMemcpyAsync(dY, Y, bytes, hipMemcpyHostToDevice, st);
    for (int32_t c0 = 0; c0 < k && e == hipSuccess; c0 += COMBINE_COLS) {
        const int32_t nc = std::min(COMBINE_COLS, k - c0);
        k_combine<<<dim3(nblk(g->n_pad), two ? 2u : 1u), PF_BLOCK, 0, st>>>(g->ws, g->n_pad, src_first, m, dY, k, c0, nc, dst_first, src_first2,
                                                                          dst_first2);
        e = hipGetLastError();
    }
    hipError_t e2 = staged ? hipSuccess : hipStreamSynchronize(st);
    pf_free(st, dY);
    PF_HIP(e);
    PF_HIP(e2);
    return PF_OK;
}

extern "C" {

int pf_resnorm(pf_graph* g, int32_t ax, int32_t x, double lam, double* out) {
    PF_TRY(check_slots(g, ax, 1, "pf_resnorm"));
    PF_TRY(check_slots(g, x, 1, "pf_resnorm"));
    PF_CHECK(out != nullptr, PF_E_ARG, "pf_resnorm: out is NULL");
    hipStream_t st = g->ctx->stream;
    PF_TRY(pf_reduce_ensure(g, 1));
    k_resnorm_partial<<<(unsigned)g->n_chunks, PF_BLOCK, 0, st>>>(pf_slot(g, ax), pf_slot(g, x), lam, g->n_pad, g->n_chunks, g->partials);
    PF_HIP(hipGetLastError());
    k_dot_finish<<<1, PF_WAVE, 0, st>>>(g->partials, g->n_chunks, g->coef, nullptr, 0);
    PF_HIP(hipGetLastError());
    double r2 = 0.0;
    PF_HIP(hipMemcpyAsync(&r2, g->coef, sizeof(double), hipMemcpyDeviceToHost, st));
    PF_HIP(hipStreamSynchronize(st));
    *out = sqrt(r2 > 0.0 ? r2 : 0.0);
    return PF_OK;
}

int pf_gram(pf_graph* g, int32_t first_a, int32_t count_a, int32_t first_b, int32_t count_b, double* out) {
    PF_TRY(check_slots(g, first_a, count_a, "pf_gram"));
    PF_TRY(check_slots(g, first_b, count_b, "pf_gram"));
    PF_CHECK(out != nullptr && count_a > 0 && count_b > 0, PF_E_ARG, "pf_gram: bad argument");
    PF_TRY(pf_reduce_ensure(g, count_a * count_b));
    hipStream_t st = g->ctx->stream;
    k_gram_partial<<<dim3((unsigned)g->n_chunks, (unsigned)(count_a * count_b)), PF_BLOCK, 0, st>>>(g->ws, g->n_pad, first_a, first_b, count_b,
                                                                                                 g->n_chunks, g->partials);
    PF_HIP(hipGetLastError());
    k_dot_finish<<<(unsigned)(count_a * count_b), PF_WAVE, 0, st>>>(g->partials, g->n_chunks, g->coef, nullptr, 0);
    PF_HIP(hipGetLastError());
    return small_to_host(g, g->coef, out, (size_t)count_a * count_b);
}

}

static int small_begin(pf_graph* g, const double* d_src, size_t count, bool root, bool append = false) {
    PF_CHECK(append ? g->small_pending > 0 && !g->small_root && !root : g->small_pending == 0, PF_E_STATE,
             "pf_gram_begin / pf_resnorms_begin: a previous result has not been collected");
    pf_ctx* c = g->ctx;
    hipStream_t st = c->stream;
    const size_t offset = append ? (size_t)g->small_pending : 0;
    if (append) {
        PF_CHECK((int64_t)(offset + count) <= g->small_host_cap, PF_E_STATE, "pf_gram_begin: no room to append");
    } else if ((int64_t)(2 * count) > g->small_host_cap || !g->small_host) {
        if (g->small_host) {
            PF_HIP(hipStreamSynchronize(st));
            c->pinned_pool.emplace_back(g->small_host_cap, g->small_host);
            g->small_host = nullptr;
        }
        const int32_t cap = std::max((int32_t)(2 * count), 128);
        for (size_t i = 0; i < c->pinned_pool.size(); ++i)
            if (c->pinned_pool[i].first >= cap) {
                g->small_host_cap = c->pinned_pool[i].first;
                g->small_host = c->pinned_pool[i].second;
                c->pinned_pool.erase(c->pinned_pool.begin() + (long)i);
                break;
            }
        if (!g->small_host) {
            PF_HIP(hipHostMalloc((void**)&g->small_host, sizeof(double) * (size_t)(cap + 2), hipHostMallocDefault));
            g->small_host_cap = cap;
        }
    }
    if (!g->small_ev) {
        if (!c->event_pool.empty()) {
            g->small_ev = c->event_pool.back();
            c->event_pool.pop_back();
        } else {
            PF_HIP(hipEventCreateWithFlags(&g->small_ev, hipEventDisableTiming));
        }
    }
    PF_TRY(pf_copy_by_kernel(st, d_src, g->small_host + offset, sizeof(double) * count));
    PF_HIP(hipEventRecord(g->small_ev, st));
    g->small_pending = (int32_t)(offset + count);
    g->small_root = root;
    return PF_OK;
}

int pf_small_end(pf_graph* g, double* out) {
    PF_CHECK(g != nullptr && out != nullptr && g->small_pending > 0, PF_E_STATE, "pf_small_end: nothing to collect");
    PF_HIP(hipEventSynchronize(g->small_ev));
    const int32_t count = g->small_pending;
    g->small_pending = 0;
    for (int32_t i = 0; i < count; ++i) {
        const double v = g->small_host[i];
        out[i] = g->small_root ? sqrt(v > 0.0 ? v : 0.0) : v;
    }
    return PF_OK;
}

int pf_gram_begin(pf_graph* g, int32_t first_a, int32_t count_a, int32_t first_b, int32_t count_b, int32_t append) {
    PF_TRY(check_slots(g, first_a, count_a, "pf_gram"));
    PF_TRY(check_slots(g, first_b, count_b, "pf_gram"));
    PF_CHECK(count_a > 0 && count_b > 0, PF_E_ARG, "pf_gram: bad argument");
    PF_TRY(pf_reduce_ensure(g, count_a * count_b));
    hipStream_t st = g->ctx->stream;
    k_gram_partial<<<dim3((unsigned)g->n_chunks, (unsigned)(count_a * count_b)), PF_BLOCK, 0, st>>>(g->ws, g->n_pad, first_a, first_b, count_b,
                                                                                                 g->n_chunks, g->partials);
    PF_HIP(hipGetLastError());
    k_dot_finish<<<(unsigned)(count_a * count_b), PF_WAVE, 0, st>>>(g->partials, g->n_chunks, g->coef, nullptr, 0);
    PF_HIP(hipGetLastError());
    return small_begin(g, g->coef, (size_t)count_a * count_b, false, append != 0);
}

int pf_resnorms_begin(pf_graph* g, int32_t ax_first, int32_t x_first, const double* lam, int32_t count) {
    PF_TRY(check_slots(g, ax_first, count, "pf_resnorms"));
    PF_TRY(check_slots(g, x_first, count, "pf_resnorms"));
    PF_CHECK(lam != nullptr && count > 0, PF_E_ARG, "pf_resnorms: bad argument");
    hipStream_t st = g->ctx->stream;
    PF_TRY(pf_reduce_ensure(g, count));
    for (int32_t at = 0; at < count; at += PF_RESNORMS_MAX) {
        const int32_t nb = std::min(count - at, PF_RESNORMS_MAX);
        LamArgs la{};
        for (int32_t i = 0; i < nb; ++i) la.lam[i] = lam[at + i];
        k_resnorms_partial<<<dim3((unsigned)g->n_chunks, (unsigned)nb), PF_BLOCK, 0, st>>>(g->ws, g->n_pad, ax_first + at, x_first + at, la,
                                                                                        g->n_chunks, g->partials);
        PF_HIP(hipGetLastError());
        k_dot_finish<<<(unsigned)nb, PF_WAVE, 0, st>>>(g->partials, g->n_chunks, g->coef + at, nullptr, 0);
        PF_HIP(hipGetLastError());
    }
    return small_begin(g, g->coef, (size_t)count, true);
}

extern "C" {

int pf_resnorms(pf_graph* g, int32_t ax_first, int32_t x_first, const double* lam, int32_t count, double* out) {
    PF_TRY(check_slots(g, ax_first, count, "pf_resnorms"));
    PF_TRY(check_slots(g, x_first, count, "pf_resnorms"));
    PF_CHECK(out != nullptr && lam != nullptr && count > 0, PF_E_ARG, "pf_resnorms: bad argument");
    hipStream_t st = g->ctx->stream;
    PF_TRY(pf_reduce_ensure(g, count));
    for (int32_t at = 0; at < count; at += PF_RESNORMS_MAX) {
        const int32_t nb = std::min(count - at, PF_RESNORMS_MAX);
        LamArgs la{};
        for (int32_t i = 0; i < nb; ++i) la.lam[i] = lam[at + i];
        k_resnorms_partial<<<dim3((unsigned)g->n_chunks, (unsigned)nb), PF_BLOCK, 0, st>>>(g->ws, g->n_pad, ax_first + at, x_first + at, la,
                                                                                        g->n_chunks, g->partials);
        PF_HIP(hipGetLastError());
        k_dot_finish<<<(unsigned)nb, PF_WAVE, 0, st>>>(g->partials, g->n_chunks, g->coef + at, nullptr, 0);
        PF_HIP(hipGetLastError());
    }
    PF_TRY(small_to_host(g, g->coef, out, (size_t)count));
    for (int32_t i = 0; i < count; ++i) out[i] = sqrt(out[i] > 0.0 ? out[i] : 0.0);
    return PF_OK;
}

static bool downloads_deferred() {
    static const bool on = [] { const char* v = getenv("PF_DOWNLOAD_DEFER"); return !(v && v[0] == '0'); }();
    return on;
}

static int queue_download(pf_graph* g) {
    pf_ctx* ctx = g->ctx;
    const double* src = nullptr;
    {
        std::lock_guard<std::mutex> lk(ctx->deferred_mutex);
        auto it = std::find(ctx->deferred.begin(), ctx->deferred.end(), g);
        if (it != ctx->deferred.end()) ctx->deferred.erase(it);
        src = g->dl_src;
        g->dl_src = nullptr;
    }
    if (!src) return PF_OK;
    PF_HIP(hipEventRecord(g->final_ready, ctx->stream));
    PF_HIP(hipStreamWaitEvent(ctx->copy_stream, g->final_ready, 0));
    PF_HIP(hipMemcpyAsync(g->dl_dst, src, g->dl_bytes, hipMemcpyDeviceToHost, ctx->copy_stream));
    PF_HIP(hipEventRecord(g->final_done, ctx->copy_stream));
    return PF_OK;
}

extern "C++" int pf_download_cancel(pf_graph* g) {
    pf_ctx* ctx = g->ctx;
    bool owed = false;
    {
        std::lock_guard<std::mutex> lk(ctx->deferred_mutex);
        auto it = std::find(ctx->deferred.begin(), ctx->deferred.end(), g);
        if (it != ctx->deferred.end()) ctx->deferred.erase(it);
        owed = g->dl_src != nullptr;
        g->dl_src = nullptr;
    }
    if (g->final_pending != 0) {
        g->final_pending = 0;
        g->final_check = 0;
        if (!owed) (void)hipEventSynchronize(g->final_done);
        pf_free(ctx->stream, g->final_params);
        g->final_params = nullptr;
        pf_free(ctx->stream, g->final_tmp);
        g->final_tmp = nullptr;
    }
    return PF_OK;
}

extern "C++" int pf_downloads_release(pf_ctx* c) {
    for (;;) {
        pf_graph* g = nullptr;
        {
            std::lock_guard<std::mutex> lk(c->deferred_mutex);
            if (c->deferred.empty()) break;
            g = c->deferred.back();
        }
        PF_TRY(queue_download(g));
    }
    return PF_OK;
}

int pf_finalize_vectors_begin(pf_graph* g, int32_t first, int32_t count, int32_t from_sym, int32_t minmax, double* out) {
    PF_TRY(check_slots(g, first, count, "pf_finalize_vectors"));
    PF_CHECK(out != nullptr && count > 0, PF_E_ARG, "pf_finalize_vectors: bad argument");
    PF_CHECK(!from_sym || g->is_symmetric, PF_E_ARG, "pf_finalize_vectors: from_sym on an asymmetric graph");
    PF_TRY(pf_finalize_vectors_end(g));
    pf_ctx* ctx = g->ctx;
    hipStream_t st = ctx->stream;
    if (!ctx->copy_stream) PF_HIP(pf_create_side_stream(&ctx->copy_stream, true));
    for (hipEvent_t* ev : {&g->final_ready, &g->final_done}) {
        if (*ev) continue;
        if (!ctx->event_pool.empty()) {
            *ev = ctx->event_pool.back();
            ctx->event_pool.pop_back();
        } else {
            PF_HIP(hipEventCreateWithFlags(ev, hipEventDisableTiming));
        }
    }
    const int32_t stat_doubles = (int32_t)(sizeof(VecStats) / sizeof(double)) * count;
    if (stat_doubles > g->final_stats_cap + 2 || !g->final_stats) {
        if (g->final_stats) ctx->pinned_pool.emplace_back(g->final_stats_cap, reinterpret_cast<double*>(g->final_stats));
        g->final_stats = nullptr;
        for (size_t i = 0; i < ctx->pinned_pool.size(); ++i)
            if (ctx->pinned_pool[i].first + 2 >= stat_doubles) {
                g->final_stats_cap = ctx->pinned_pool[i].first;
                g->final_stats = ctx->pinned_pool[i].second;
                ctx->pinned_pool.erase(ctx->pinned_pool.begin() + (long)i);
                break;
            }
        if (!g->final_stats) {
            const int32_t cap = std::max(stat_doubles, 384);
            PF_HIP(hipHostMalloc((void**)&g->final_stats, sizeof(double) * (size_t)(cap + 2), hipHostMallocDefault));
            g->final_stats_cap = cap;
        }
    }
    PF_TRY(pf_reduce_ensure(g, count));
    VecStats* part = reinterpret_cast<VecStats*>(g->partials);
    VecStats* fin = part + (size_t)count * g->n_chunks;
    dim3 grid((unsigned)g->n_chunks, (unsigned)count);
    k_vec_stats_partial<<<grid, PF_BLOCK, 0, st>>>(g->ws, g->n_pad, g->n, first, g->sg, g->perm, g->perm_m, from_sym, g->n_chunks, part);
    PF_HIP(hipGetLastError());
    k_vec_stats_finish<<<(unsigned)count, PF_WAVE, 0, st>>>(part, g->n_chunks, fin);
    PF_HIP(hipGetLastError());
    double *d_params = nullptr, *d_out = nullptr;
    pf_free(st, g->final_vecs);
    g->final_vecs = nullptr;
    g->final_count = 0;
    PF_HIP(pf_malloc(st, (void**)&d_params, sizeof(double) * 4 * (size_t)count + sizeof(VecStats) * (size_t)count));
    VecStats* d_stats = reinterpret_cast<VecStats*>(d_params + 4 * (size_t)count);
    hipError_t e = pf_malloc(st, (void**)&d_out, sizeof(double) * (size_t)g->n * count);
    if (e == hipSuccess) {
        k_vec_params<<<1, PF_WAVE, 0, st>>>(fin, count, minmax, d_params);
        k_vec_apply<<<nblk(g->n), PF_BLOCK, 0, st>>>(g->ws, g->n_pad, g->n, first, count, g->sg, g->iperm, g->mrank, from_sym, d_params, d_out);
        e = hipGetLastError();
    }
    if (e == hipSuccess) e = hipMemcpyAsync(d_stats, fin, sizeof(VecStats) * count, hipMemcpyDeviceToDevice, st);
    if (e == hipSuccess) e = hipEventRecord(g->final_ready, st);
    if (e == hipSuccess) e = hipStreamWaitEvent(ctx->copy_stream, g->final_ready, 0);
    if (e == hipSuccess) e = hipMemcpyAsync(g->final_stats, d_stats, sizeof(VecStats) * count, hipMemcpyDeviceToHost, ctx->copy_stream);
    if (e == hipSuccess) e = hipEventRecord(g->final_done, ctx->copy_stream);
    if (e != hipSuccess) {
        (void)hipStreamSynchronize(ctx->copy_stream);
        pf_free(st, d_params);
        pf_free(st, d_out);
        PF_HIP(e);
    }
    g->final_vecs = d_out;
    g->final_count = count;
    g->final_params = d_params;
    g->final_pending = count;
    g->final_check = count;
    g->dl_src = d_out;
    g->dl_dst = out;
    g->dl_bytes = sizeof(double) * (size_t)g->n * count;
    if (downloads_deferred()) {
        std::lock_guard<std::mutex> lk(ctx->deferred_mutex);
        if (std::find(ctx->deferred.begin(), ctx->deferred.end(), g) == ctx->deferred.end()) ctx->deferred.push_back(g);
    } else {
        PF_TRY(queue_download(g));
    }
    return PF_OK;
}

int pf_finalize_vectors_end(pf_graph* g) {
    PF_CHECK(g != nullptr, PF_E_ARG, "pf_finalize_vectors_end: NULL graph");
    if (g->final_pending == 0) return PF_OK;
    g->final_pending = 0;
    const int32_t count = g->final_check;
    g->final_check = 0;
    int rc = queue_download(g);
    const hipError_t e = hipEventSynchronize(g->final_done);
    pf_free(g->ctx->stream, g->final_params);
    g->final_params = nullptr;
    pf_free(g->ctx->stream, g->final_tmp);
    g->final_tmp = nullptr;
    PF_TRY(rc);
    if (count <= 0) {
        PF_HIP(e);
        return PF_OK;
    }
    const VecStats* hs = reinterpret_cast<const VecStats*>(g->final_stats);
    bool sane = e == hipSuccess;
    int32_t bad = 0;
    for (int32_t c = 0; c < count && sane; ++c)
        if (!(hs[c].sumsq > 0.0 && isfinite(hs[c].sumsq))) sane = false, bad = c;
    if (!sane) {
        pf_free(g->ctx->stream, g->final_vecs);
        g->final_vecs = nullptr;
        g->final_count = 0;
    }
    PF_HIP(e);
    PF_CHECK(sane, PF_E_STATE, "pf_finalize_vectors: vector %d has norm^2 %g", bad, hs[(size_t)bad].sumsq);
    return PF_OK;
}

int pf_finalize_vectors(pf_graph* g, int32_t first, int32_t count, int32_t from_sym, int32_t minmax, double* out) {
    PF_TRY(pf_finalize_vectors_begin(g, first, count, from_sym, minmax, out));
    return pf_finalize_vectors_end(g);
}

struct RemapArgs {
    int32_t col[64];
    double sign[64];
};
__global__ __launch_bounds__(PF_BLOCK) void k_final_remap(const double* __restrict__ fin, int64_t n, int32_t fc, int32_t count, RemapArgs m,
                                                          double* __restrict__ out) {
    const int64_t e = (int64_t)blockIdx.x * PF_BLOCK + threadIdx.x;
    if (e >= n * count) return;
    const int64_t i = e / count;
    const int32_t c = (int32_t)(e - i * count);
    out[e] = fin[i * fc + m.col[c]] * m.sign[c];
}

int pf_final_remap_begin(pf_graph* g, const int32_t* col, const double* sign, int32_t count, double* out) {
    PF_CHECK(g && col && sign && out, PF_E_ARG, "pf_final_remap_begin: NULL argument");
    if (!(g->dl_src && g->dl_dst == out)) PF_TRY(pf_finalize_vectors_end(g));
    PF_CHECK(g->final_vecs != nullptr, PF_E_STATE, "pf_final_remap_begin: no pf_finalize_vectors result is resident");
    PF_CHECK(count >= 1 && count <= 64 && count <= g->final_count, PF_E_ARG, "pf_final_remap_begin: count %d out of range", count);
    RemapArgs m{};
    for (int32_t c = 0; c < count; ++c) {
        PF_CHECK(col[c] >= 0 && col[c] < g->final_count, PF_E_ARG, "pf_final_remap_begin: column %d out of range", col[c]);
        m.col[c] = col[c];
        m.sign[c] = sign[c];
    }
    pf_ctx* ctx = g->ctx;
    hipStream_t st = ctx->stream;
    PF_CHECK(ctx->copy_stream && g->final_ready && g->final_done, PF_E_STATE, "pf_final_remap_begin: no download machinery (call after pf_finalize_vectors_begin)");
    double* d_tmp = nullptr;
    PF_HIP(pf_malloc(st, (void**)&d_tmp, sizeof(double) * (size_t)g->n * count));
    k_final_remap<<<nblk(g->n * count), PF_BLOCK, 0, st>>>(g->final_vecs, g->n, g->final_count, count, m, d_tmp);
    const hipError_t e = hipGetLastError();
    if (e != hipSuccess) {
        pf_free(st, d_tmp);
        PF_HIP(e);
    }
    pf_free(st, g->final_tmp);
    g->final_tmp = d_tmp;
    g->dl_src = d_tmp;
    g->dl_dst = out;
    g->dl_bytes = sizeof(double) * (size_t)g->n * count;
    g->final_pending = count;
    if (downloads_deferred()) {
        std::lock_guard<std::mutex> lk(ctx->deferred_mutex);
        if (std::find(ctx->deferred.begin(), ctx->deferred.end(), g) == ctx->deferred.end()) ctx->deferred.push_back(g);
    } else {
        PF_TRY(queue_download(g));
    }
    return PF_OK;
}

static int rows_to_host(pf_graph* g, const double* src, int32_t width, const int64_t* rows, int64_t n_rows, double* out,
                        const char* who) {
    if (n_rows == 0) return PF_OK;
    PF_HIP(hipSetDevice(g->ctx->device));
    hipStream_t st = g->ctx->stream;
    for (int64_t i = 0; i < n_rows; ++i)
        PF_CHECK(rows[i] >= 0 && rows[i] < g->n, PF_E_ARG, "%s: row %lld out of range", who, (long long)rows[i]);
    int64_t* d_rows = nullptr;
    double* d_out = nullptr;
    PF_HIP(pf_malloc(st, (void**)&d_rows, sizeof(int64_t) * n_rows));
    hipError_t e = pf_malloc(st, (void**)&d_out, sizeof(double) * (size_t)n_rows * width);
    if (e == hipSuccess) e = hipMemcpyAsync(d_rows, rows, sizeof(int64_t) * n_rows, hipMemcpyHostToDevice, st);
    if (e == hipSuccess) {
        k_final_rows<<<nblk(n_rows * width), PF_BLOCK, 0, st>>>(src, d_rows, n_rows, width, d_out);
        e = hipGetLastError();
    }
    if (e == hipSuccess) e = hipMemcpyAsync(out, d_out, sizeof(double) * (size_t)n_rows * width, hipMemcpyDeviceToHost, st);
    hipError_t e2 = hipStreamSynchronize(st);
    pf_free(st, d_rows);
    pf_free(st, d_out);
    PF_HIP(e);
    PF_HIP(e2);
    return PF_OK;
}

int pf_final_rows(pf_graph* g, const int64_t* rows, int64_t n_rows, double* out) {
    PF_CHECK(g != nullptr && rows != nullptr && out != nullptr && n_rows >= 0, PF_E_ARG, "pf_final_rows: bad argument");
    PF_CHECK(g->final_vecs != nullptr, PF_E_STATE, "pf_final_rows: no pf_finalize_vectors result is resident");
    return rows_to_host(g, g->final_vecs, g->final_count, rows, n_rows, out, "pf_final_rows");
}

int pf_point_rows(pf_graph* g, const int64_t* rows, int64_t n_rows, double* out) {
    PF_CHECK(g != nullptr && rows != nullptr && out != nullptr && n_rows >= 0, PF_E_ARG, "pf_point_rows: bad argument");
    PF_CHECK(g->pts != nullptr, PF_E_STATE, "pf_point_rows: this graph was not built from a mesh");
    return rows_to_host(g, g->pts, 3, rows, n_rows, out, "pf_point_rows");
}

int pf_spmv_host(pf_graph* g, int32_t op, const double* x, double* y) {
    PF_CHECK(g != nullptr && x != nullptr && y != nullptr, PF_E_ARG, "pf_spmv_host: NULL argument");
    const double* vals = op_values(g, op);
    PF_CHECK(vals != nullptr, PF_E_ARG, "pf_spmv_host: operator %d unavailable", op);
    PF_TRY(pf_ws_ensure(g, 2));
    PF_TRY(pf_ws_upload(g, 0, x));
    PF_TRY(launch_op(g, vals, pf_slot(g, 0), nullptr, pf_slot(g, 1), -1.0, 0.0, 0.0));
// ... 229 lines not shown
```

Baseline: 993.4.

## Record and co-launch paired solver kernels through a deferred launch recorder

Converts many kernels into launchable functor structs and routes their launches through a thread-local recorder. During paired init, shared extraction advances and finalization of the two meshes, the launches are held and flushed together, with held orth_begin calls merged into a paired orth_begin2. The goal is to cut per-kernel launch overhead and let the two independent eigensolves run their small kernels concurrently or fused. It adds deferred-execution complexity, and any operation that needs results must flush first, so errors or missed flushes could cause ordering bugs.

New measurement: 988.8. Within noise of the previous version (-0.5%).

```diff
diff --git a/pyfocusr_amd/csrc/pf_api.hip b/pyfocusr_amd/csrc/pf_api.hip
--- a/pyfocusr_amd/csrc/pf_api.hip
+++ b/pyfocusr_amd/csrc/pf_api.hip
@@ -14,16 +14,19 @@
 static std::mutex g_ctx_mutex;
 static std::vector<pf_ctx*> g_ctxs;
 
-__global__ __launch_bounds__(PF_BLOCK) void k_copy_words(const unsigned long long* __restrict__ src, unsigned long long* __restrict__ dst,
-                                                         size_t n) {
-    const size_t i = (size_t)blockIdx.x * PF_BLOCK + threadIdx.x;
-    if (i < n) dst[i] = src[i];
-}
+struct k_copy_words {
+    static constexpr int BOUNDS = PF_BLOCK;
+    static __device__ __forceinline__ void run(const unsigned long long* __restrict__ src, unsigned long long* __restrict__ dst,
+                                                             size_t n) {
+        const size_t i = (size_t)blockIdx.x * PF_BLOCK + threadIdx.x;
+        if (i < n) dst[i] = src[i];
+    }
+};
 
 int pf_copy_by_kernel(hipStream_t st, const void* src, void* dst, size_t bytes) {
     if (bytes == 0) return PF_OK;
     const size_t n = (bytes + 7) / 8;
-    k_copy_words<<<(unsigned)((n + PF_BLOCK - 1) / PF_BLOCK), PF_BLOCK, 0, st>>>(static_cast<const unsigned long long*>(src),
+    pfl::launch<k_copy_words>(dim3((unsigned)((n + PF_BLOCK - 1) / PF_BLOCK)), dim3(PF_BLOCK), 0, st, static_cast<const unsigned long long*>(src),
                                                                                  static_cast<unsigned long long*>(dst), n);
     PF_HIP(hipGetLastError());
     return PF_OK;
diff --git a/pyfocusr_amd/csrc/pf_eigs.hip b/pyfocusr_amd/csrc/pf_eigs.hip
--- a/pyfocusr_amd/csrc/pf_eigs.hip
+++ b/pyfocusr_amd/csrc/pf_eigs.hip
@@ -5,26 +5,81 @@
 
 #include "pf_internal.h"
 #include "pf_krylov.h"
+#include "pf_launch.h"
 
 namespace {
 
 struct DeviceOps final : pfk::Ops {
     pf_graph* g;
+    pfl::Recorder rec;
+    bool holding = false, orth_held = false;
+    int32_t held_w = 0, held_first = 0, held_count = 0;
     explicit DeviceOps(pf_graph* graph) : g(graph) {}
+    ~DeviceOps() override { pfl::flush(rec, nullptr); }
+    int send_own() {
+        pfl::flush(rec, nullptr);
+        if (!orth_held) return PF_OK;
+        orth_held = false;
+        return pf_orth_begin(g, held_w, held_first, held_count, 1);
+    }
+    template <typename F>
+    int recorded(F f) {
+        if (!holding) return f();
+        if (orth_held) PF_TRY(send_own());
+        pfl::tl_rec = &rec;
+        const int rc = f();
+        pfl::tl_rec = nullptr;
+        return rc;
+    }
+    template <typename F>
+    int direct(F f) {
+        if (holding) PF_TRY(send_own());
+        return f();
+    }
+    int send_both(pfk::Ops& other) {
+        DeviceOps& o = static_cast<DeviceOps&>(other);
+        if (holding) PF_TRY(send_own());
+        return o.holding ? o.send_own() : PF_OK;
+    }
+    void hold() override { holding = true; }
+    int release_pair(pfk::Ops& other) override {
+        DeviceOps& o = static_cast<DeviceOps&>(other);
+        holding = o.holding = false;
+        pfl::flush(rec, &o.rec);
+        if (orth_held && o.orth_held) {
+            orth_held = o.orth_held = false;
+            return pf_orth_begin2(g, held_w, held_first, held_count, 1, o.g, o.held_w, o.held_first, o.held_count, 1);
+        }
+        PF_TRY(send_own());
+        return o.send_own();
+    }
     int64_t n() const override { return g->n; }
     int64_t n_isolated() const override { return g->n_isolated; }
     int32_t n_components() const override { return g->n_components; }
     int32_t n_oneway() const override { return g->n_oneway; }
     bool symmetric() const override { return g->is_symmetric; }
     double spectral_bound() const override { return g->spectral_bound; }
-    int ws_ensure(int32_t slots) override { return pf_ws_ensure(g, slots); }
-    int lock_nulls(int32_t op, int32_t* locked) override { return pf_lock_null_vectors(g, op, locked); }
+    int ws_ensure(int32_t slots) override {
+        return recorded([&] { return pf_ws_ensure(g, slots); });
+    }
+    int lock_nulls(int32_t op, int32_t* locked) override {
+        return recorded([&] { return pf_lock_null_vectors(g, op, locked); });
+    }
     int orth_strict(bool on) override { return pf_orth_strict(g, on ? 1 : 0); }
     int orth_always_twice(bool on, bool strict_otherwise) override { return pf_orth_strict(g, on ? 2 : (strict_otherwise ? 1 : 0)); }
     int orth_device_passes(bool on) override { return pf_orth_device_passes(g, on ? 1 : 0); }
-    int start_vector(int32_t slot, uint64_t seed) override { return pf_start_vector(g, slot, seed); }
-    int orth_begin(int32_t w, int32_t first, int32_t count) override { return pf_orth_begin(g, w, first, count, 1); }
+    int start_vector(int32_t slot, uint64_t seed) override {
+        return recorded([&] { return pf_start_vector(g, slot, seed); });
+    }
+    int orth_begin(int32_t w, int32_t first, int32_t count) override {
+        if (!holding) return pf_orth_begin(g, w, first, count, 1);
+        if (orth_held) PF_TRY(send_own());
+        orth_held = true;
+        held_w = w, held_first = first, held_count = count;
+        return PF_OK;
+    }
     int orth_end(double* h, double* nrm, bool* redone) override {
+        if (holding) PF_TRY(send_own());
         PF_TRY(pf_orth_end(g, h, nrm));
         const int r = pf_orth_redone(g);
         *redone = r == 1;
@@ -32,42 +87,53 @@
         return PF_OK;
     }
     int cheb(int32_t op, int32_t src, int32_t dst, int32_t degree, double c, double e, double rho) override {
-        return pf_cheb(g, op, src, dst, degree, c, e, rho);
+        return direct([&] { return pf_cheb(g, op, src, dst, degree, c, e, rho); });
     }
     int combine(int32_t src_first, int32_t m, const double* Y, int32_t k, int32_t dst_first) override {
-        return pf_combine(g, src_first, m, Y, k, dst_first);
+        return recorded([&] { return pf_combine(g, src_first, m, Y, k, dst_first); });
     }
     int combine2(int32_t src_first, int32_t m, const double* Y, int32_t k, int32_t dst_first, int32_t src_first2, int32_t dst_first2) override {
-        return pf_combine2(g, src_first, m, Y, k, dst_first, src_first2, dst_first2);
-    }
-    int copy(int32_t src, int32_t dst, int32_t count) override { return pf_ws_copy(g, src, dst, count); }
+        return recorded([&] { return pf_combine2(g, src_first, m, Y, k, dst_first, src_first2, dst_first2); });
+    }
+    int copy(int32_t src, int32_t dst, int32_t count) override {
+        return direct([&] { return pf_ws_copy(g, src, dst, count); });
+    }
     int spmv_multi(int32_t op, int32_t src_first, int32_t dst_first, int32_t count) override {
-        return pf_spmv_multi(g, op, src_first, dst_first, count);
+        return recorded([&] { return pf_spmv_multi(g, op, src_first, dst_first, count); });
     }
     int gram(int32_t first_a, int32_t count_a, int32_t first_b, int32_t count_b, double* out) override {
-        return pf_gram(g, first_a, count_a, first_b, count_b, out);
+        return direct([&] { return pf_gram(g, first_a, count_a, first_b, count_b, out); });
     }
     int resnorms(int32_t ax_first, int32_t x_first, const double* lam, int32_t count, double* out) override {
-        return pf_resnorms(g, ax_first, x_first, lam, count, out);
+        return direct([&] { return pf_resnorms(g, ax_first, x_first, lam, count, out); });
     }
     int gram_begin(int32_t first_a, int32_t count_a, int32_t first_b, int32_t count_b, bool self_b) override {
-        PF_TRY(pf_gram_begin(g, first_a, count_a, first_b, count_b, 0));
-        return self_b ? pf_gram_begin(g, first_b, count_b, first_b, count_b, 1) : PF_OK;
+        return recorded([&] {
+            PF_TRY(pf_gram_begin(g, first_a, count_a, first_b, count_b, 0));
+            return self_b ? pf_gram_begin(g, first_b, count_b, first_b, count_b, 1) : PF_OK;
+        });
     }
     bool orth_split(int32_t first2, int32_t split) override { return pf_orth_split(g, first2, split) == PF_OK; }
-    int gram_end(double* out) override { return pf_small_end(g, out); }
+    int gram_end(double* out) override {
+        return direct([&] { return pf_small_end(g, out); });
+    }
     int resnorms_begin(int32_t ax_first, int32_t x_first, const double* lam, int32_t count) override {
-        return pf_resnorms_begin(g, ax_first, x_first, lam, count);
-    }
-    int resnorms_end(double* out) override { return pf_small_end(g, out); }
+        return recorded([&] { return pf_resnorms_begin(g, ax_first, x_first, lam, count); });
+    }
+    int resnorms_end(double* out) override {
+        return direct([&] { return pf_small_end(g, out); });
+    }
     int orth_begin_pair(pfk::Ops& other, const int32_t* o) override {
+        PF_TRY(send_both(other));
         return pf_orth_begin2(g, o[0], o[1], o[2], o[3], static_cast<DeviceOps&>(other).g, o[4], o[5], o[6], o[7]);
     }
     int cheb_pair(pfk::Ops& other, const int32_t* ci, const double* cd) override {
+        PF_TRY(send_both(other));
         return pf_cheb2(g, ci[0], ci[1], ci[2], ci[3], cd[0], cd[1], cd[2], static_cast<DeviceOps&>(other).g, ci[4], ci[5], ci[6], ci[7], cd[3],
                         cd[4], cd[5]);
     }
     int orth_cheb_pair(pfk::Ops& other, const int32_t* orth, const int32_t* ci, const double* cd) override {
+        PF_TRY(send_both(other));
         return pf_orth_cheb2(g, static_cast<DeviceOps&>(other).g, orth, ci, cd);
     }
 };
@@ -142,12 +208,27 @@
         DeviceOps oa(ga), ob(gb);
         pfk::Solver a, b;
         *n_out_a = *n_out_b = 0;
+        oa.hold();
         rc = a.init(&oa, n_wanted_a, ellipse_hint());
+        ob.hold();
         if (rc == PF_OK) rc = b.init(&ob, n_wanted_b, ellipse_hint());
+        {
+            const int rr = oa.release_pair(ob);
+            if (rc == PF_OK) rc = rr;
+        }
         if (rc == PF_OK) rc = pfk::drive_pair(a, b);
         if (rc == PF_OK) rc = pf_sync(ga->ctx);
-        if (rc == PF_OK) rc = finish(ga, a, minmax, vals_a, vecs_a, res_a, n_out_a, stats_a, async_download != 0);
-        if (rc == PF_OK) rc = finish(gb, b, minmax, vals_b, vecs_b, res_b, n_out_b, stats_b, async_download != 0);
+        if (rc == PF_OK) {
+            pfl::Recorder ra, rb;
+            pfl::tl_rec = &ra;
+            rc = finish(ga, a, minmax, vals_a, vecs_a, res_a, n_out_a, stats_a, true);
+            pfl::tl_rec = &rb;
+            if (rc == PF_OK) rc = finish(gb, b, minmax, vals_b, vecs_b, res_b, n_out_b, stats_b, true);
+            pfl::tl_rec = nullptr;
+            pfl::flush(ra, &rb);
+            if (rc == PF_OK && !async_download && a.n_out > 0) rc = pf_finalize_vectors_end(ga);
+            if (rc == PF_OK && !async_download && b.n_out > 0) rc = pf_finalize_vectors_end(gb);
+        }
         if (rc != PF_OK) {
             give_up(ga);
             give_up(gb);
diff --git a/pyfocusr_amd/csrc/pf_krylov.h b/pyfocusr_amd/csrc/pf_krylov.h
--- a/pyfocusr_amd/csrc/pf_krylov.h
+++ b/pyfocusr_amd/csrc/pf_krylov.h
@@ -98,6 +98,11 @@
     virtual int orth_cheb_pair(Ops& other, const int32_t* orth, const int32_t* ci, const double* cd) {
         PFK_TRY(orth_begin_pair(other, orth));
         return cheb_pair(other, ci, cd);
+    }
+    virtual void hold() {}
+    virtual int release_pair(Ops& other) {
+        (void)other;
+        return PF_OK;
     }
 };
 
@@ -972,11 +977,23 @@
 }
 
 inline int advance_pair(Solver& a, Solver& b, bool do_a, bool do_b, AnalysisHelper* helper) {
+    auto advance_shared = [&]() -> int {
+        a.ops->hold();
+        const int ra = a.advance();
+        b.ops->hold();
+        const int rb = ra == PF_OK ? b.advance() : PF_OK;
+        const int rr = a.ops->release_pair(*b.ops);
+        return ra != PF_OK ? ra : (rb != PF_OK ? rb : rr);
+    };
     if (do_a) PFK_TRY(a.advance());
     if (do_b) PFK_TRY(b.advance());
     auto extractions = [&]() -> int {
         for (;;) {
             bool any = false;
+            if (do_a && !a.done && a.extracting && do_b && !b.done && b.extracting) {
+                PFK_TRY(advance_shared());
+                continue;
+            }
             if (do_a && !a.done && a.extracting) {
                 PFK_TRY(a.advance());
                 any = true;
@@ -1014,8 +1031,12 @@
             PFK_TRY(extractions());
             continue;
         }
-        if (da) PFK_TRY(a.advance());
-        if (db) PFK_TRY(b.advance());
+        if (ea && eb) {
+            PFK_TRY(advance_shared());
+        } else {
+            if (da) PFK_TRY(a.advance());
+            if (db) PFK_TRY(b.advance());
+        }
         PFK_TRY(extractions());
     }
 }
diff --git a/pyfocusr_amd/csrc/pf_operator.hip b/pyfocusr_amd/csrc/pf_operator.hip
--- a/pyfocusr_amd/csrc/pf_operator.hip
+++ b/pyfocusr_amd/csrc/pf_operator.hip
@@ -9,6 +9,7 @@
 #include <vector>
 
 #include "pf_internal.h"
+#include "pf_launch.h"
 
 namespace {
 
@@ -75,11 +76,14 @@
     sell_op_block<HAS_PREV>(a, blockIdx.x);
 }
 
-__global__ __launch_bounds__(PF_OP_BLOCK) void k_sell_op_slots(OpArgs a, int64_t slot_stride) {
-    a.x += (int64_t)blockIdx.y * slot_stride;
-    a.out += (int64_t)blockIdx.y * slot_stride;
-    sell_op_block<false>(a, blockIdx.x);
-}
+struct k_sell_op_slots {
+    static constexpr int BOUNDS = PF_OP_BLOCK;
+    static __device__ __forceinline__ void run(OpArgs a, int64_t slot_stride) {
+        a.x += (int64_t)blockIdx.y * slot_stride;
+        a.out += (int64_t)blockIdx.y * slot_stride;
+        sell_op_block<false>(a, blockIdx.x);
+    }
+};
 
 template <bool HAS_PREV>
 __global__ __launch_bounds__(PF_OP_BLOCK) void k_sell_op2(OpArgs a, OpArgs b) {
@@ -87,42 +91,48 @@
     else sell_op_block<HAS_PREV>(b, blockIdx.x - a.n_blocks);
 }
 
-__global__ __launch_bounds__(PF_BLOCK) void k_dot_partial(const double* __restrict__ ws, int64_t n_pad, int32_t first,
-                                                          int32_t wslot, int64_t n_chunks, double* __restrict__ partial,
-                                                          int32_t self_col = -1) {
-    __shared__ double red[PF_BLOCK / PF_WAVE];
-    const int b = blockIdx.y;
-    const int64_t chunk = blockIdx.x;
-    const double* v = ws + (int64_t)(b == self_col ? wslot : first + b) * n_pad;
-    const double* w = ws + (int64_t)wslot * n_pad;
-    const int64_t lo = chunk * PF_DOT_CHUNK;
-    const int64_t hi = lo + PF_DOT_CHUNK < n_pad ? lo + PF_DOT_CHUNK : n_pad;
-    double s = 0.0;
-    for (int64_t i = lo + 2 * threadIdx.x; i < hi; i += 2 * PF_BLOCK) {
-        const double2 a = *reinterpret_cast<const double2*>(v + i);
-        const double2 c = *reinterpret_cast<const double2*>(w + i);
-        s += a.x * c.x;
-        s += a.y * c.y;
-    }
-#pragma unroll
-    for (int off = PF_WAVE / 2; off > 0; off >>= 1) s += __shfl_down(s, off, PF_WAVE);
-    if ((threadIdx.x & (PF_WAVE - 1)) == 0) red[threadIdx.x / PF_WAVE] = s;
-    __syncthreads();
-    if (threadIdx.x == 0) partial[(int64_t)b * n_chunks + chunk] = (red[0] + red[1]) + (red[2] + red[3]);
-}
-
-__global__ __launch_bounds__(PF_WAVE) void k_dot_finish(const double* __restrict__ partial, int64_t n_chunks,
-                                                        double* __restrict__ out, double* __restrict__ acc, int accumulate) {
-    const int b = blockIdx.x;
-    double s = 0.0;
-    for (int64_t k = threadIdx.x; k < n_chunks; k += PF_WAVE) s += partial[(int64_t)b * n_chunks + k];
-#pragma unroll
-    for (int off = PF_WAVE / 2; off > 0; off >>= 1) s += __shfl_down(s, off, PF_WAVE);
-    if (threadIdx.x == 0) {
-        out[b] = s;
-        if (acc) acc[b] = accumulate ? acc[b] + s : s;
-    }
-}
+struct k_dot_partial {
+    static constexpr int BOUNDS = PF_BLOCK;
+    static __device__ __forceinline__ void run(const double* __restrict__ ws, int64_t n_pad, int32_t first,
+                                                              int32_t wslot, int64_t n_chunks, double* __restrict__ partial,
+                                                              int32_t self_col) {
+        __shared__ double red[PF_BLOCK / PF_WAVE];
+        const int b = blockIdx.y;
+        const int64_t chunk = blockIdx.x;
+        const double* v = ws + (int64_t)(b == self_col ? wslot : first + b) * n_pad;
+        const double* w = ws + (int64_t)wslot * n_pad;
+        const int64_t lo = chunk * PF_DOT_CHUNK;
+        const int64_t hi = lo + PF_DOT_CHUNK < n_pad ? lo + PF_DOT_CHUNK : n_pad;
+        double s = 0.0;
+        for (int64_t i = lo + 2 * threadIdx.x; i < hi; i += 2 * PF_BLOCK) {
+            const double2 a = *reinterpret_cast<const double2*>(v + i);
+            const double2 c = *reinterpret_cast<const double2*>(w + i);
+            s += a.x * c.x;
+            s += a.y * c.y;
+        }
+    #pragma unroll
+        for (int off = PF_WAVE / 2; off > 0; off >>= 1) s += __shfl_down(s, off, PF_WAVE);
+        if ((threadIdx.x & (PF_WAVE - 1)) == 0) red[threadIdx.x / PF_WAVE] = s;
+        __syncthreads();
+        if (threadIdx.x == 0) partial[(int64_t)b * n_chunks + chunk] = (red[0] + red[1]) + (red[2] + red[3]);
+    }
+};
+
+struct k_dot_finish {
+    static constexpr int BOUNDS = PF_WAVE;
+    static __device__ __forceinline__ void run(const double* __restrict__ partial, int64_t n_chunks,
+                                                            double* __restrict__ out, double* __restrict__ acc, int accumulate) {
+        const int b = blockIdx.x;
+        double s = 0.0;
+        for (int64_t k = threadIdx.x; k < n_chunks; k += PF_WAVE) s += partial[(int64_t)b * n_chunks + k];
+    #pragma unroll
+        for (int off = PF_WAVE / 2; off > 0; off >>= 1) s += __shfl_down(s, off, PF_WAVE);
+        if (threadIdx.x == 0) {
+            out[b] = s;
+            if (acc) acc[b] = accumulate ? acc[b] + s : s;
+        }
+    }
+};
 
 __global__ __launch_bounds__(PF_BLOCK) void k_multi_axpy(double* __restrict__ ws, int64_t n_pad, int32_t first,
                                                          int32_t count, int32_t wslot, const double* __restrict__ h) {
@@ -513,11 +523,14 @@
     if (i < n_pad) x[i] *= alpha;
 }
 
-__global__ __launch_bounds__(PF_BLOCK) void k_scale_rsqrt(double* __restrict__ x, int64_t n_pad, const double* __restrict__ nrm2) {
-    const int64_t i = (int64_t)blockIdx.x * PF_BLOCK + threadIdx.x;
-    const double v = *nrm2;
-    if (i < n_pad && v > 1e-280) x[i] *= 1.0 / sqrt(v);
-}
+struct k_scale_rsqrt {
+    static constexpr int BOUNDS = PF_BLOCK;
+    static __device__ __forceinline__ void run(double* __restrict__ x, int64_t n_pad, const double* __restrict__ nrm2) {
+        const int64_t i = (int64_t)blockIdx.x * PF_BLOCK + threadIdx.x;
+        const double v = *nrm2;
+        if (i < n_pad && v > 1e-280) x[i] *= 1.0 / sqrt(v);
+    }
+};
 
 __global__ __launch_bounds__(PF_BLOCK) void k_mask_isolated(double* __restrict__ x, const int32_t* __restrict__ rowptr,
                                                             const int32_t* __restrict__ perm, int64_t n) {
@@ -527,25 +540,28 @@
     if (rowptr[i + 1] == rowptr[i]) x[r] = 0.0;
 }
 
-__global__ __launch_bounds__(PF_BLOCK) void k_start_vector(double* __restrict__ x, const double* __restrict__ smooth,
-                                                           const int32_t* __restrict__ perm, const int32_t* __restrict__ perm_m,
-                                                           const int32_t* __restrict__ rowptr,
-                                                           int64_t n_pad, unsigned long long seed, double noise) {
-    const int64_t r = (int64_t)blockIdx.x * PF_BLOCK + threadIdx.x;
-    if (r >= n_pad) return;
-    const int32_t i = perm[r];
-    const int32_t m = perm_m[r];
-    double v = 0.0;
-    if (i >= 0 && rowptr[m + 1] > rowptr[m]) {
-        unsigned long long z = seed + 0x9E3779B97F4A7C15ull * (unsigned long long)(i + 1);
-        z = (z ^ (z >> 30)) * 0xBF58476D1CE4E5B9ull;
-        z = (z ^ (z >> 27)) * 0x94D049BB133111EBull;
-        z ^= z >> 31;
-        const double u = (double)(z >> 11) * (1.0 / 9007199254740992.0) - 0.5;
-        v = smooth[r] + noise * u;
-    }
-    x[r] = v;
-}
+struct k_start_vector {
+    static constexpr int BOUNDS = PF_BLOCK;
+    static __device__ __forceinline__ void run(double* __restrict__ x, const double* __restrict__ smooth,
+                                                               const int32_t* __restrict__ perm, const int32_t* __restrict__ perm_m,
+                                                               const int32_t* __restrict__ rowptr,
+                                                               int64_t n_pad, unsigned long long seed, double noise) {
+        const int64_t r = (int64_t)blockIdx.x * PF_BLOCK + threadIdx.x;
+        if (r >= n_pad) return;
+        const int32_t i = perm[r];
+        const int32_t m = perm_m[r];
+        double v = 0.0;
+        if (i >= 0 && rowptr[m + 1] > rowptr[m]) {
+            unsigned long long z = seed + 0x9E3779B97F4A7C15ull * (unsigned long long)(i + 1);
+            z = (z ^ (z >> 30)) * 0xBF58476D1CE4E5B9ull;
+            z = (z ^ (z >> 27)) * 0x94D049BB133111EBull;
+            z ^= z >> 31;
+            const double u = (double)(z >> 11) * (1.0 / 9007199254740992.0) - 0.5;
+            v = smooth[r] + noise * u;
+        }
+        x[r] = v;
+    }
+};
 
 __global__ __launch_bounds__(PF_BLOCK) void k_permute_in(const double* __restrict__ src_old, const int32_t* __restrict__ perm,
                                                          int64_t n_pad, double* __restrict__ dst_new) {
@@ -564,40 +580,46 @@
     for (int c = 0; c < count; ++c) dst_old[(int64_t)c * n + i] = ws[(int64_t)(first + c) * n_pad + r];
 }
 
-__global__ __launch_bounds__(PF_BLOCK) void k_null_vector(double* __restrict__ x, const int32_t* __restrict__ label,
-                                                          const int32_t* __restrict__ rowptr,
-                                                          const double* __restrict__ deg, const int32_t* __restrict__ perm,
-                                                          int64_t n_pad, int32_t root, int32_t sym,
-                                                          const double* __restrict__ weight) {
-    const int64_t r = (int64_t)blockIdx.x * PF_BLOCK + threadIdx.x;
-    if (r >= n_pad) return;
-    const int32_t i = perm[r];
-    double v = 0.0;
-    if (i >= 0 && label[i] == root && rowptr[i + 1] > rowptr[i]) v = weight ? weight[i] : (sym ? sqrt(deg[i] + 1e-8) : 1.0);
-    x[r] = v;
-}
+struct k_null_vector {
+    static constexpr int BOUNDS = PF_BLOCK;
+    static __device__ __forceinline__ void run(double* __restrict__ x, const int32_t* __restrict__ label,
+                                                              const int32_t* __restrict__ rowptr,
+                                                              const double* __restrict__ deg, const int32_t* __restrict__ perm,
+                                                              int64_t n_pad, int32_t root, int32_t sym,
+                                                              const double* __restrict__ weight) {
+        const int64_t r = (int64_t)blockIdx.x * PF_BLOCK + threadIdx.x;
+        if (r >= n_pad) return;
+        const int32_t i = perm[r];
+        double v = 0.0;
+        if (i >= 0 && label[i] == root && rowptr[i + 1] > rowptr[i]) v = weight ? weight[i] : (sym ? sqrt(deg[i] + 1e-8) : 1.0);
+        x[r] = v;
+    }
+};
 
 constexpr int COMBINE_COLS = 8;
-__global__ __launch_bounds__(PF_BLOCK) void k_combine(double* __restrict__ ws, int64_t n_pad, int32_t src_first, int32_t m,
-                                                      const double* __restrict__ Y, int32_t k, int32_t c0, int32_t ncols,
-                                                      int32_t dst_first, int32_t src_first2, int32_t dst_first2) {
-    const int64_t i = (int64_t)blockIdx.x * PF_BLOCK + threadIdx.x;
-    if (i >= n_pad) return;
-    if (blockIdx.y) src_first = src_first2, dst_first = dst_first2;
-    double acc[COMBINE_COLS];
-#pragma unroll
-    for (int c = 0; c < COMBINE_COLS; ++c) acc[c] = 0.0;
-    for (int b = 0; b < m; ++b) {
-        const double v = ws[(int64_t)(src_first + b) * n_pad + i];
-        const double* yr = Y + (int64_t)b * k + c0;
-#pragma unroll
+struct k_combine {
+    static constexpr int BOUNDS = PF_BLOCK;
+    static __device__ __forceinline__ void run(double* __restrict__ ws, int64_t n_pad, int32_t src_first, int32_t m,
+                                                          const double* __restrict__ Y, int32_t k, int32_t c0, int32_t ncols,
+                                                          int32_t dst_first, int32_t src_first2, int32_t dst_first2) {
+        const int64_t i = (int64_t)blockIdx.x * PF_BLOCK + threadIdx.x;
+        if (i >= n_pad) return;
+        if (blockIdx.y) src_first = src_first2, dst_first = dst_first2;
+        double acc[COMBINE_COLS];
+    #pragma unroll
+        for (int c = 0; c < COMBINE_COLS; ++c) acc[c] = 0.0;
+        for (int b = 0; b < m; ++b) {
+            const double v = ws[(int64_t)(src_first + b) * n_pad + i];
+            const double* yr = Y + (int64_t)b * k + c0;
+    #pragma unroll
+            for (int c = 0; c < COMBINE_COLS; ++c)
+                if (c < ncols) acc[c] += v * yr[c];
+        }
+    #pragma unroll
         for (int c = 0; c < COMBINE_COLS; ++c)
-            if (c < ncols) acc[c] += v * yr[c];
-    }
-#pragma unroll
-    for (int c = 0; c < COMBINE_COLS; ++c)
-        if (c < ncols) ws[(int64_t)(dst_first + c0 + c) * n_pad + i] = acc[c];
-}
+            if (c < ncols) ws[(int64_t)(dst_first + c0 + c) * n_pad + i] = acc[c];
+    }
+};
 
 __global__ __launch_bounds__(PF_BLOCK) void k_resnorm_partial(const double* __restrict__ ax, const double* __restrict__ x,
                                                               double lam, int64_t n_pad, int64_t n_chunks,
@@ -617,54 +639,60 @@
     if (threadIdx.x == 0) partial[blockIdx.x] = (red[0] + red[1]) + (red[2] + red[3]);
 }
 
-__global__ __launch_bounds__(PF_BLOCK) void k_gram_partial(const double* __restrict__ ws, int64_t n_pad, int32_t first_a, int32_t first_b,
-                                                           int32_t count_b, int64_t n_chunks, double* __restrict__ partial) {
-    __shared__ double red[PF_BLOCK / PF_WAVE];
-    const int p = blockIdx.y;
-    const int i = p / count_b, j = p - i * count_b;
-    const double* v = ws + (int64_t)(first_b + j) * n_pad;
-    const double* w = ws + (int64_t)(first_a + i) * n_pad;
-    const int64_t lo = (int64_t)blockIdx.x * PF_DOT_CHUNK;
-    const int64_t hi = lo + PF_DOT_CHUNK < n_pad ? lo + PF_DOT_CHUNK : n_pad;
-    double s = 0.0;
-    for (int64_t r = lo + 2 * threadIdx.x; r < hi; r += 2 * PF_BLOCK) {
-        const double2 a = *reinterpret_cast<const double2*>(v + r);
-        const double2 c = *reinterpret_cast<const double2*>(w + r);
-        s += a.x * c.x;
-        s += a.y * c.y;
-    }
-#pragma unroll
-    for (int off = PF_WAVE / 2; off > 0; off >>= 1) s += __shfl_down(s, off, PF_WAVE);
-    if ((threadIdx.x & (PF_WAVE - 1)) == 0) red[threadIdx.x / PF_WAVE] = s;
-    __syncthreads();
-    if (threadIdx.x == 0) partial[(int64_t)p * n_chunks + blockIdx.x] = (red[0] + red[1]) + (red[2] + red[3]);
-}
+struct k_gram_partial {
+    static constexpr int BOUNDS = PF_BLOCK;
+    static __device__ __forceinline__ void run(const double* __restrict__ ws, int64_t n_pad, int32_t first_a, int32_t first_b,
+                                                               int32_t count_b, int64_t n_chunks, double* __restrict__ partial) {
+        __shared__ double red[PF_BLOCK / PF_WAVE];
+        const int p = blockIdx.y;
+        const int i = p / count_b, j = p - i * count_b;
+        const double* v = ws + (int64_t)(first_b + j) * n_pad;
+        const double* w = ws + (int64_t)(first_a + i) * n_pad;
+        const int64_t lo = (int64_t)blockIdx.x * PF_DOT_CHUNK;
+        const int64_t hi = lo + PF_DOT_CHUNK < n_pad ? lo + PF_DOT_CHUNK : n_pad;
+        double s = 0.0;
+        for (int64_t r = lo + 2 * threadIdx.x; r < hi; r += 2 * PF_BLOCK) {
+            const double2 a = *reinterpret_cast<const double2*>(v + r);
+            const double2 c = *reinterpret_cast<const double2*>(w + r);
+            s += a.x * c.x;
+            s += a.y * c.y;
+        }
+    #pragma unroll
+        for (int off = PF_WAVE / 2; off > 0; off >>= 1) s += __shfl_down(s, off, PF_WAVE);
+        if ((threadIdx.x & (PF_WAVE - 1)) == 0) red[threadIdx.x / PF_WAVE] = s;
+        __syncthreads();
+        if (threadIdx.x == 0) partial[(int64_t)p * n_chunks + blockIdx.x] = (red[0] + red[1]) + (red[2] + red[3]);
+    }
+};
 
 constexpr int PF_RESNORMS_MAX = 64;
 struct LamArgs {
     double lam[PF_RESNORMS_MAX];
 };
-__global__ __launch_bounds__(PF_BLOCK) void k_resnorms_partial(const double* __restrict__ ws, int64_t n_pad, int32_t ax_first,
-                                                               int32_t x_first, LamArgs la, int64_t n_chunks,
-                                                               double* __restrict__ partial) {
-    __shared__ double red[PF_BLOCK / PF_WAVE];
-    const int b = blockIdx.y;
-    const double* ax = ws + (int64_t)(ax_first + b) * n_pad;
-    const double* x = ws + (int64_t)(x_first + b) * n_pad;
-    const double lam = la.lam[b];
-    const int64_t lo = (int64_t)blockIdx.x * PF_DOT_CHUNK;
-    const int64_t hi = lo + PF_DOT_CHUNK < n_pad ? lo + PF_DOT_CHUNK : n_pad;
-    double s = 0.0;
-    for (int64_t i = lo + threadIdx.x; i < hi; i += PF_BLOCK) {
-        const double r = ax[i] - lam * x[i];
-        s += r * r;
-    }
-#pragma unroll
-    for (int off = PF_WAVE / 2; off > 0; off >>= 1) s += __shfl_down(s, off, PF_WAVE);
-    if ((threadIdx.x & (PF_WAVE - 1)) == 0) red[threadIdx.x / PF_WAVE] = s;
-    __syncthreads();
-    if (threadIdx.x == 0) partial[(int64_t)b * n_chunks + blockIdx.x] = (red[0] + red[1]) + (red[2] + red[3]);
-}
+struct k_resnorms_partial {
+    static constexpr int BOUNDS = PF_BLOCK;
+    static __device__ __forceinline__ void run(const double* __restrict__ ws, int64_t n_pad, int32_t ax_first,
+                                                                   int32_t x_first, LamArgs la, int64_t n_chunks,
+                                                                   double* __restrict__ partial) {
+        __shared__ double red[PF_BLOCK / PF_WAVE];
+        const int b = blockIdx.y;
+        const double* ax = ws + (int64_t)(ax_first + b) * n_pad;
+        const double* x = ws + (int64_t)(x_first + b) * n_pad;
+        const double lam = la.lam[b];
+        const int64_t lo = (int64_t)blockIdx.x * PF_DOT_CHUNK;
+        const int64_t hi = lo + PF_DOT_CHUNK < n_pad ? lo + PF_DOT_CHUNK : n_pad;
+        double s = 0.0;
+        for (int64_t i = lo + threadIdx.x; i < hi; i += PF_BLOCK) {
+            const double r = ax[i] - lam * x[i];
+            s += r * r;
+        }
+    #pragma unroll
+        for (int off = PF_WAVE / 2; off > 0; off >>= 1) s += __shfl_down(s, off, PF_WAVE);
+        if ((threadIdx.x & (PF_WAVE - 1)) == 0) red[threadIdx.x / PF_WAVE] = s;
+        __syncthreads();
+        if (threadIdx.x == 0) partial[(int64_t)b * n_chunks + blockIdx.x] = (red[0] + red[1]) + (red[2] + red[3]);
+    }
+};
 
 struct VecStats {
     double sumsq, vmin, vmax, absmax, at_absmax;
@@ -693,82 +721,94 @@
     return o;
 }
 
-__global__ __launch_bounds__(PF_BLOCK) void k_vec_stats_partial(const double* __restrict__ ws, int64_t n_pad, int64_t n,
-                                                                int32_t first, const double* __restrict__ sg,
-                                                                const int32_t* __restrict__ perm, const int32_t* __restrict__ perm_m,
-                                                                int32_t from_sym, int64_t n_chunks, VecStats* __restrict__ partial) {
-    __shared__ VecStats red[PF_BLOCK / PF_WAVE];
-    const int b = blockIdx.y;
-    const double* x = ws + (int64_t)(first + b) * n_pad;
-    const int64_t lo = (int64_t)blockIdx.x * PF_DOT_CHUNK;
-    const int64_t hi0 = lo + PF_DOT_CHUNK;
-    const int64_t hi = hi0 < n ? hi0 : n;
-    VecStats st{0.0, INFINITY, -INFINITY, -1.0, 0.0, (int64_t)1 << 62};
-    for (int64_t r = lo + threadIdx.x; r < hi; r += PF_BLOCK) {
-        const int64_t i = perm[r];
-        double v = x[r];
-        if (from_sym) v *= sg[perm_m[r]];
-        VecStats e{v * v, v, v, fabs(v), v, i};
-        stats_merge(st, e);
-    }
-#pragma unroll
-    for (int off = PF_WAVE / 2; off > 0; off >>= 1) {
-        VecStats o = stats_shfl(st, off);
-        stats_merge(st, o);
-    }
-    if ((threadIdx.x & (PF_WAVE - 1)) == 0) red[threadIdx.x / PF_WAVE] = st;
-    __syncthreads();
-    if (threadIdx.x == 0) {
-        VecStats t = red[0];
-        stats_merge(t, red[1]);
-        stats_merge(t, red[2]);
-        stats_merge(t, red[3]);
-        partial[(int64_t)b * n_chunks + blockIdx.x] = t;
-    }
-}
-
-__global__ __launch_bounds__(PF_WAVE) void k_vec_stats_finish(const VecStats* __restrict__ partial, int64_t n_chunks,
-                                                              VecStats* __restrict__ out) {
-    const int b = blockIdx.x;
-    VecStats st{0.0, INFINITY, -INFINITY, -1.0, 0.0, (int64_t)1 << 62};
-    for (int64_t k = threadIdx.x; k < n_chunks; k += PF_WAVE) stats_merge(st, partial[(int64_t)b * n_chunks + k]);
-#pragma unroll
-    for (int off = PF_WAVE / 2; off > 0; off >>= 1) {
-        VecStats o = stats_shfl(st, off);
-        stats_merge(st, o);
-    }
-    if (threadIdx.x == 0) out[b] = st;
-}
-
-__global__ void k_vec_params(const VecStats* __restrict__ fin, int32_t count, int32_t minmax, double* __restrict__ params) {
-    for (int c = threadIdx.x; c < count; c += blockDim.x) {
-        const VecStats s = fin[c];
-        const double sgn = s.at_absmax < 0.0 ? -1.0 : 1.0;
-        const double scale = sgn / sqrt(s.sumsq);
-        const double vmin = (sgn > 0 ? s.vmin : s.vmax) * scale;
-        const double vmax = (sgn > 0 ? s.vmax : s.vmin) * scale;
-        params[4 * c + 0] = scale;
-        params[4 * c + 1] = minmax ? vmin : 0.0;
-        params[4 * c + 2] = minmax ? (vmax - vmin) : 0.0;
-        params[4 * c + 3] = minmax ? 0.5 : 0.0;
-    }
-}
-
-__global__ __launch_bounds__(PF_BLOCK) void k_vec_apply(const double* __restrict__ ws, int64_t n_pad, int64_t n,
-                                                        int32_t first, int32_t count, const double* __restrict__ sg,
-                                                        const int32_t* __restrict__ iperm, const int32_t* __restrict__ mrank,
-                                                        int32_t from_sym, const double* __restrict__ params, double* __restrict__ out) {
-    const int64_t i = (int64_t)blockIdx.x * PF_BLOCK + threadIdx.x;
-    if (i >= n) return;
-    const int64_t r = iperm[i];
-    const double s = from_sym ? sg[mrank ? mrank[i] : i] : 1.0;
-    for (int c = 0; c < count; ++c) {
-        const double scale = params[4 * c + 0], off = params[4 * c + 1], ptp = params[4 * c + 2], half = params[4 * c + 3];
-        double v = (ws[(int64_t)(first + c) * n_pad + r] * s) * scale;
-        if (ptp != 0.0) v = (v - off) / ptp - half;
-        out[i * count + c] = v;
-    }
-}
+struct k_vec_stats_partial {
+    static constexpr int BOUNDS = PF_BLOCK;
+    static __device__ __forceinline__ void run(const double* __restrict__ ws, int64_t n_pad, int64_t n,
+                                                                    int32_t first, const double* __restrict__ sg,
+                                                                    const int32_t* __restrict__ perm, const int32_t* __restrict__ perm_m,
+                                                                    int32_t from_sym, int64_t n_chunks, VecStats* __restrict__ partial) {
+        __shared__ VecStats red[PF_BLOCK / PF_WAVE];
+        const int b = blockIdx.y;
+        const double* x = ws + (int64_t)(first + b) * n_pad;
+        const int64_t lo = (int64_t)blockIdx.x * PF_DOT_CHUNK;
+        const int64_t hi0 = lo + PF_DOT_CHUNK;
+        const int64_t hi = hi0 < n ? hi0 : n;
+        VecStats st{0.0, INFINITY, -INFINITY, -1.0, 0.0, (int64_t)1 << 62};
+        for (int64_t r = lo + threadIdx.x; r < hi; r += PF_BLOCK) {
+            const int64_t i = perm[r];
+            double v = x[r];
+            if (from_sym) v *= sg[perm_m[r]];
+            VecStats e{v * v, v, v, fabs(v), v, i};
+            stats_merge(st, e);
+        }
+    #pragma unroll
+        for (int off = PF_WAVE / 2; off > 0; off >>= 1) {
+            VecStats o = stats_shfl(st, off);
+            stats_merge(st, o);
+        }
+        if ((threadIdx.x & (PF_WAVE - 1)) == 0) red[threadIdx.x / PF_WAVE] = st;
+        __syncthreads();
+        if (threadIdx.x == 0) {
+            VecStats t = red[0];
+            stats_merge(t, red[1]);
+            stats_merge(t, red[2]);
+            stats_merge(t, red[3]);
+            partial[(int64_t)b * n_chunks + blockIdx.x] = t;
+        }
+    }
+};
+
+struct k_vec_stats_finish {
+    static constexpr int BOUNDS = PF_WAVE;
+    static __device__ __forceinline__ void run(const VecStats* __restrict__ partial, int64_t n_chunks,
+                                                                  VecStats* __restrict__ out) {
+        const int b = blockIdx.x;
+        VecStats st{0.0, INFINITY, -INFINITY, -1.0, 0.0, (int64_t)1 << 62};
+        for (int64_t k = threadIdx.x; k < n_chunks; k += PF_WAVE) stats_merge(st, partial[(int64_t)b * n_chunks + k]);
+    #pragma unroll
+        for (int off = PF_WAVE / 2; off > 0; off >>= 1) {
+            VecStats o = stats_shfl(st, off);
+            stats_merge(st, o);
+        }
+        if (threadIdx.x == 0) out[b] = st;
+    }
+};
+
+struct k_vec_params {
+    static constexpr int BOUNDS = 1024;
+    static __device__ __forceinline__ void run(const VecStats* __restrict__ fin, int32_t count, int32_t minmax, double* __restrict__ params) {
+        for (int c = threadIdx.x; c < count; c += blockDim.x) {
+            const VecStats s = fin[c];
+            const double sgn = s.at_absmax < 0.0 ? -1.0 : 1.0;
+            const double scale = sgn / sqrt(s.sumsq);
+            const double vmin = (sgn > 0 ? s.vmin : s.vmax) * scale;
+            const double vmax = (sgn > 0 ? s.vmax : s.vmin) * scale;
+            params[4 * c + 0] = scale;
+            params[4 * c + 1] = minmax ? vmin : 0.0;
+            params[4 * c + 2] = minmax ? (vmax - vmin) : 0.0;
+            params[4 * c + 3] = minmax ? 0.5 : 0.0;
+        }
+    }
+};
+
+struct k_vec_apply {
+    static constexpr int BOUNDS = PF_BLOCK;
+    static __device__ __forceinline__ void run(const double* __restrict__ ws, int64_t n_pad, int64_t n,
+                                                            int32_t first, int32_t count, const double* __restrict__ sg,
+                                                            const int32_t* __restrict__ iperm, const int32_t* __restrict__ mrank,
+                                                            int32_t from_sym, const double* __restrict__ params, double* __restrict__ out) {
+        const int64_t i = (int64_t)blockIdx.x * PF_BLOCK + threadIdx.x;
+        if (i >= n) return;
+        const int64_t r = iperm[i];
+        const double s = from_sym ? sg[mrank ? mrank[i] : i] : 1.0;
+        for (int c = 0; c < count; ++c) {
+            const double scale = params[4 * c + 0], off = params[4 * c + 1], ptp = params[4 * c + 2], half = params[4 * c + 3];
+            double v = (ws[(int64_t)(first + c) * n_pad + r] * s) * scale;
+            if (ptp != 0.0) v = (v - off) / ptp - half;
+            out[i * count + c] = v;
+        }
+    }
+};
 
 __global__ __launch_bounds__(PF_BLOCK) void k_final_rows(const double* __restrict__ fin, const int64_t* __restrict__ rows, int64_t n_rows,
                                                          int32_t fc, double* __restrict__ out) {
@@ -1023,11 +1063,11 @@
             on = false;
             return;
         }
-        hipEventRecord(e0, c->stream);
+        (void)pfl::event_record(c->stream, e0);
     }
     int finish() {
         if (!on) return PF_OK;
-        PF_HIP(hipEventRecord(e1, c->stream));
+        PF_HIP(pfl::event_record(c->stream, e1));
         c->spans_pending.push_back({e0, e1, launches, bytes, persist_steps, lds_bytes});
         return PF_OK;
     }
@@ -1053,9 +1093,9 @@
     hipStream_t st = g->ctx->stream;
     PF_TRY(pf_reduce_ensure(g, count));
     dim3 grid((unsigned)g->n_chunks, (unsigned)count);
-    k_dot_partial<<<grid, PF_BLOCK, 0, st>>>(g->ws, g->n_pad, first, w, g->n_chunks, g->partials);
-    PF_HIP(hipGetLastError());
-    k_dot_finish<<<(unsigned)count, PF_WAVE, 0, st>>>(g->partials, g->n_chunks, d_out, d_acc, accumulate);
+    pfl::launch<k_dot_partial>(dim3(grid), dim3(PF_BLOCK), 0, st, g->ws, g->n_pad, first, w, g->n_chunks, g->partials, -1);
+    PF_HIP(hipGetLastError());
+    pfl::launch<k_dot_finish>(dim3((unsigned)count), dim3(PF_WAVE), 0, st, g->partials, g->n_chunks, d_out, d_acc, accumulate);
     PF_HIP(hipGetLastError());
     return PF_OK;
 }
@@ -1090,9 +1130,9 @@
     double* nw = nullptr;
     const size_t bytes = sizeof(double) * (size_t)(n_slots + PF_WS_TMPS) * (size_t)g->n_pad;
     PF_HIP(pf_malloc(st, (void**)&nw, bytes));
-    PF_HIP(hipMemsetAsync(nw, 0, bytes, st));
+    pfl::call(st, [=](hipStream_t s) { (void)hipMemsetAsync(nw, 0, bytes, s); });
     if (g->ws && g->n_slots > 0)
-        PF_HIP(hipMemcpyAsync(nw, g->ws, sizeof(double) * (size_t)g->n_slots * g->n_pad, hipMemcpyDeviceToDevice, st));
+        PF_HIP(pfl::memcpy_async(st, nw, g->ws, sizeof(double) * (size_t)g->n_slots * g->n_pad, hipMemcpyDeviceToDevice));
     pf_free(st, g->ws);
     g->ws = nw;
     g->n_slots = n_slots;
@@ -1144,7 +1184,7 @@
 
 int pf_start_vector(pf_graph* g, int32_t slot, uint64_t seed) {
     PF_TRY(check_slots(g, slot, 1, "pf_start_vector"));
-    k_start_vector<<<nblk(g->n_pad), PF_BLOCK, 0, g->ctx->stream>>>(pf_slot(g, slot), g->smooth, g->perm, g->perm_m, g->rowptr, g->n_pad,
+    pfl::launch<k_start_vector>(dim3(nblk(g->n_pad)), dim3(PF_BLOCK), 0, g->ctx->stream, pf_slot(g, slot), g->smooth, g->perm, g->perm_m, g->rowptr, g->n_pad,
                                                                     (unsigned long long)seed, 0.5);
     PF_HIP(hipGetLastError());
     return PF_OK;
@@ -1160,11 +1200,11 @@
     hipStream_t st = g->ctx->stream;
     PF_TRY(pf_reduce_ensure(g, 1));
     for (int32_t c = 0; c < nc; ++c) {
-        k_null_vector<<<nblk(g->n_pad), PF_BLOCK, 0, st>>>(pf_slot(g, c), g->label, g->rowptr, g->deg, g->perm_m, g->n_pad,
+        pfl::launch<k_null_vector>(dim3(nblk(g->n_pad)), dim3(PF_BLOCK), 0, st, pf_slot(g, c), g->label, g->rowptr, g->deg, g->perm_m, g->n_pad,
                                                           g->roots[c], op == PF_OP_SYM && !g->unit_g, g->is_cotan ? g->cot_sqrtm : nullptr);
         PF_HIP(hipGetLastError());
         PF_TRY(dots_device(g, c, c, 1, g->coef, nullptr, 0));
-        k_scale_rsqrt<<<nblk(g->n_pad), PF_BLOCK, 0, st>>>(pf_slot(g, c), g->n_pad, g->coef);
+        pfl::launch<k_scale_rsqrt>(dim3(nblk(g->n_pad)), dim3(PF_BLOCK), 0, st, pf_slot(g, c), g->n_pad, g->coef);
         PF_HIP(hipGetLastError());
     }
     *n_locked = nc;
@@ -1192,7 +1232,7 @@
     OpTimer t(g->ctx, count, (double)count * (double)op_bytes(g));
     {
         const OpArgs a = op_args(g, vals, pf_slot(g, src_first), nullptr, pf_slot(g, dst_first), -1.0, 0.0, 0.0);
-        k_sell_op_slots<<<dim3(a.n_blocks, (unsigned)count), PF_OP_BLOCK, 0, g->ctx->stream>>>(a, g->n_pad);
+        pfl::launch<k_sell_op_slots>(dim3(a.n_blocks, (unsigned)count), dim3(PF_OP_BLOCK), 0, g->ctx->stream, a, g->n_pad);
         PF_HIP(hipGetLastError());
     }
     return t.finish();
@@ -1472,7 +1512,7 @@
             PF_TRY(orth_launch_pass(a2, 1, g->n_chunks, g->n_pad, count, st));
         }
     } else if (count == 0) {
-        k_dot_partial<<<dim3((unsigned)g->n_chunks, 1u), PF_BLOCK, 0, st>>>(g->ws, g->n_pad, w, w, g->n_chunks, g->partials);
+        pfl::launch<k_dot_partial>(dim3((unsigned)g->n_chunks, 1u), dim3(PF_BLOCK), 0, st, g->ws, g->n_pad, w, w, g->n_chunks, g->partials, -1);
         PF_HIP(hipGetLastError());
         k_scale_finishing<<<nblk(g->n_pad), PF_BLOCK, 0, st>>>(pf_slot(g, w), g->n_pad, g->partials, g->n_chunks, normalize ? 1 : 0,
                                                               hsum, count, nrm2, g->orth_host);
@@ -1485,7 +1525,7 @@
         }
         PF_TRY(dots_device(g, w, w, 1, nrm2, nullptr, 0));
         if (normalize) {
-            k_scale_rsqrt<<<nblk(g->n_pad), PF_BLOCK, 0, st>>>(pf_slot(g, w), g->n_pad, nrm2);
+            pfl::launch<k_scale_rsqrt>(dim3(nblk(g->n_pad)), dim3(PF_BLOCK), 0, st, pf_slot(g, w), g->n_pad, nrm2);
             PF_HIP(hipGetLastError());
         }
         PF_HIP(hipMemcpyAsync(g->orth_host, hsum, sizeof(double) * count, hipMemcpyDeviceToHost, st));
@@ -1573,12 +1613,12 @@
         const int32_t w = g->orth_w, first = g->orth_first;
         const int32_t split = g->orth_split_now >= 0 ? g->orth_split_now : count;
         if (split > 0) {
-            k_dot_partial<<<dim3((unsigned)g->n_chunks, (unsigned)split), PF_BLOCK, 0, st>>>(g->ws, g->n_pad, first, w, g->n_chunks, g->partials);
+            pfl::launch<k_dot_partial>(dim3((unsigned)g->n_chunks, (unsigned)split), dim3(PF_BLOCK), 0, st, g->ws, g->n_pad, first, w, g->n_chunks, g->partials, -1);
             PF_HIP(hipGetLastError());
         }
         if (count > split) {
-            k_dot_partial<<<dim3((unsigned)g->n_chunks, (unsigned)(count - split)), PF_BLOCK, 0, st>>>(g->ws, g->n_pad, g->orth_first2_now, w, g->n_chunks,
-                                                                                                   g->partials + (size_t)split * g->n_chunks);
+            pfl::launch<k_dot_partial>(dim3((unsigned)g->n_chunks, (unsigned)(count - split)), dim3(PF_BLOCK), 0, st, g->ws, g->n_pad, g->orth_first2_now, w, g->n_chunks,
+                                                                                                   g->partials + (size_t)split * g->n_chunks, -1);
             PF_HIP(hipGetLastError());
         }
         if (split > 0) {
@@ -1590,7 +1630,7 @@
                                                                       g->partials + (size_t)split * g->n_chunks, g->n_chunks, hsum + split, 1);
             PF_HIP(hipGetLastError());
         }
-        k_dot_partial<<<dim3((unsigned)g->n_chunks, 1u), PF_BLOCK, 0, st>>>(g->ws, g->n_pad, w, w, g->n_chunks, g->partials);
+        pfl::launch<k_dot_partial>(dim3((unsigned)g->n_chunks, 1u), dim3(PF_BLOCK), 0, st, g->ws, g->n_pad, w, w, g->n_chunks, g->partials, -1);
         PF_HIP(hipGetLastError());
         k_scale_finishing<<<nblk(g->n_pad), PF_BLOCK, 0, st>>>(pf_slot(g, w), g->n_pad, g->partials, g->n_chunks, g->orth_normalize,
                                                               hsum, count, nrm2, g->orth_host);
@@ -1694,8 +1734,8 @@
                 memcpy(dst, Y, bytes);
                 src = dst;
                 staged = true;
-                hipError_t es = hipMemcpyAsync(dY, src, bytes, hipMemcpyHostToDevice, st);
-                if (es == hipSuccess) es = hipEventRecord(ctx->stage_ev[slot], st);
+                hipError_t es = pfl::memcpy_async(st, dY, src, bytes, hipMemcpyHostToDevice);
+                if (es == hipSuccess) es = pfl::event_record(st, ctx->stage_ev[slot]);
                 if (es != hipSuccess) {
                     pf_free(st, dY);
                     PF_HIP(es);
@@ -1705,14 +1745,14 @@
             }
         }
     }
-    hipError_t e = staged ? hipSuccess : hipMemcpyAsync(dY, Y, bytes, hipMemcpyHostToDevice, st);
+    hipError_t e = staged ? hipSuccess : pfl::memcpy_async(st, dY, Y, bytes, hipMemcpyHostToDevice);
     for (int32_t c0 = 0; c0 < k && e == hipSuccess; c0 += COMBINE_COLS) {
         const int32_t nc = std::min(COMBINE_COLS, k - c0);
-        k_combine<<<dim3(nblk(g->n_pad), two ? 2u : 1u), PF_BLOCK, 0, st>>>(g->ws, g->n_pad, src_first, m, dY, k, c0, nc, dst_first, src_first2,
+        pfl::launch<k_combine>(dim3(nblk(g->n_pad), two ? 2u : 1u), dim3(PF_BLOCK), 0, st, g->ws, g->n_pad, src_first, m, dY, k, c0, nc, dst_first, src_first2,
                                                                           dst_first2);
         e = hipGetLastError();
     }
-    hipError_t e2 = staged ? hipSuccess : hipStreamSynchronize(st);
+    hipError_t e2 = staged ? hipSuccess : pfl::sync(st);
     pf_free(st, dY);
     PF_HIP(e);
     PF_HIP(e2);
@@ -1729,7 +1769,7 @@
     PF_TRY(pf_reduce_ensure(g, 1));
     k_resnorm_partial<<<(unsigned)g->n_chunks, PF_BLOCK, 0, st>>>(pf_slot(g, ax), pf_slot(g, x), lam, g->n_pad, g->n_chunks, g->partials);
     PF_HIP(hipGetLastError());
-    k_dot_finish<<<1, PF_WAVE, 0, st>>>(g->partials, g->n_chunks, g->coef, nullptr, 0);
+    pfl::launch<k_dot_finish>(dim3(1), dim3(PF_WAVE), 0, st, g->partials, g->n_chunks, g->coef, nullptr, 0);
     PF_HIP(hipGetLastError());
     double r2 = 0.0;
     PF_HIP(hipMemcpyAsync(&r2, g->coef, sizeof(double), hipMemcpyDeviceToHost, st));
@@ -1744,10 +1784,10 @@
     PF_CHECK(out != nullptr && count_a > 0 && count_b > 0, PF_E_ARG, "pf_gram: bad argument");
     PF_TRY(pf_reduce_ensure(g, count_a * count_b));
     hipStream_t st = g->ctx->stream;
-    k_gram_partial<<<dim3((unsigned)g->n_chunks, (unsigned)(count_a * count_b)), PF_BLOCK, 0, st>>>(g->ws, g->n_pad, first_a, first_b, count_b,
+    pfl::launch<k_gram_partial>(dim3((unsigned)g->n_chunks, (unsigned)(count_a * count_b)), dim3(PF_BLOCK), 0, st, g->ws, g->n_pad, first_a, first_b, count_b,
                                                                                                  g->n_chunks, g->partials);
     PF_HIP(hipGetLastError());
-    k_dot_finish<<<(unsigned)(count_a * count_b), PF_WAVE, 0, st>>>(g->partials, g->n_chunks, g->coef, nullptr, 0);
+    pfl::launch<k_dot_finish>(dim3((unsigned)(count_a * count_b)), dim3(PF_WAVE), 0, st, g->partials, g->n_chunks, g->coef, nullptr, 0);
     PF_HIP(hipGetLastError());
     return small_to_host(g, g->coef, out, (size_t)count_a * count_b);
 }
@@ -1764,7 +1804,7 @@
         PF_CHECK((int64_t)(offset + count) <= g->small_host_cap, PF_E_STATE, "pf_gram_begin: no room to append");
     } else if ((int64_t)(2 * count) > g->small_host_cap || !g->small_host) {
         if (g->small_host) {
-            PF_HIP(hipStreamSynchronize(st));
+            PF_HIP(pfl::sync(st));
             c->pinned_pool.emplace_back(g->small_host_cap, g->small_host);
             g->small_host = nullptr;
         }
@@ -1790,7 +1830,7 @@
         }
     }
     PF_TRY(pf_copy_by_kernel(st, d_src, g->small_host + offset, sizeof(double) * count));
-    PF_HIP(hipEventRecord(g->small_ev, st));
+    PF_HIP(pfl::event_record(st, g->small_ev));
     g->small_pending = (int32_t)(offset + count);
     g->small_root = root;
     return PF_OK;
@@ -1814,10 +1854,10 @@
     PF_CHECK(count_a > 0 && count_b > 0, PF_E_ARG, "pf_gram: bad argument");
     PF_TRY(pf_reduce_ensure(g, count_a * count_b));
     hipStream_t st = g->ctx->stream;
-    k_gram_partial<<<dim3((unsigned)g->n_chunks, (unsigned)(count_a * count_b)), PF_BLOCK, 0, st>>>(g->ws, g->n_pad, first_a, first_b, count_b,
+    pfl::launch<k_gram_partial>(dim3((unsigned)g->n_chunks, (unsigned)(count_a * count_b)), dim3(PF_BLOCK), 0, st, g->ws, g->n_pad, first_a, first_b, count_b,
                                                                                                  g->n_chunks, g->partials);
     PF_HIP(hipGetLastError());
-    k_dot_finish<<<(unsigned)(count_a * count_b), PF_WAVE, 0, st>>>(g->partials, g->n_chunks, g->coef, nullptr, 0);
+    pfl::launch<k_dot_finish>(dim3((unsigned)(count_a * count_b)), dim3(PF_WAVE), 0, st, g->partials, g->n_chunks, g->coef, nullptr, 0);
     PF_HIP(hipGetLastError());
     return small_begin(g, g->coef, (size_t)count_a * count_b, false, append != 0);
 }
@@ -1832,10 +1872,10 @@
         const int32_t nb = std::min(count - at, PF_RESNORMS_MAX);
         LamArgs la{};
         for (int32_t i = 0; i < nb; ++i) la.lam[i] = lam[at + i];
-        k_resnorms_partial<<<dim3((unsigned)g->n_chunks, (unsigned)nb), PF_BLOCK, 0, st>>>(g->ws, g->n_pad, ax_first + at, x_first + at, la,
+        pfl::launch<k_resnorms_partial>(dim3((unsigned)g->n_chunks, (unsigned)nb), dim3(PF_BLOCK), 0, st, g->ws, g->n_pad, ax_first + at, x_first + at, la,
                                                                                         g->n_chunks, g->partials);
         PF_HIP(hipGetLastError());
-        k_dot_finish<<<(unsigned)nb, PF_WAVE, 0, st>>>(g->partials, g->n_chunks, g->coef + at, nullptr, 0);
+        pfl::launch<k_dot_finish>(dim3((unsigned)nb), dim3(PF_WAVE), 0, st, g->partials, g->n_chunks, g->coef + at, nullptr, 0);
         PF_HIP(hipGetLastError());
     }
     return small_begin(g, g->coef, (size_t)count, true);
@@ -1853,10 +1893,10 @@
         const int32_t nb = std::min(count - at, PF_RESNORMS_MAX);
         LamArgs la{};
         for (int32_t i = 0; i < nb; ++i) la.lam[i] = lam[at + i];
-        k_resnorms_partial<<<dim3((unsigned)g->n_chunks, (unsigned)nb), PF_BLOCK, 0, st>>>(g->ws, g->n_pad, ax_first + at, x_first + at, la,
+        pfl::launch<k_resnorms_partial>(dim3((unsigned)g->n_chunks, (unsigned)nb), dim3(PF_BLOCK), 0, st, g->ws, g->n_pad, ax_first + at, x_first + at, la,
                                                                                         g->n_chunks, g->partials);
         PF_HIP(hipGetLastError());
-        k_dot_finish<<<(unsigned)nb, PF_WAVE, 0, st>>>(g->partials, g->n_chunks, g->coef + at, nullptr, 0);
+        pfl::launch<k_dot_finish>(dim3((unsigned)nb), dim3(PF_WAVE), 0, st, g->partials, g->n_chunks, g->coef + at, nullptr, 0);
         PF_HIP(hipGetLastError());
     }
     PF_TRY(small_to_host(g, g->coef, out, (size_t)count));
@@ -1960,9 +2000,9 @@
     VecStats* part = reinterpret_cast<VecStats*>(g->partials);
     VecStats* fin = part + (size_t)count * g->n_chunks;
     dim3 grid((unsigned)g->n_chunks, (unsigned)count);
-    k_vec_stats_partial<<<grid, PF_BLOCK, 0, st>>>(g->ws, g->n_pad, g->n, first, g->sg, g->perm, g->perm_m, from_sym, g->n_chunks, part);
-    PF_HIP(hipGetLastError());
-    k_vec_stats_finish<<<(unsigned)count, PF_WAVE, 0, st>>>(part, g->n_chunks, fin);
+    pfl::launch<k_vec_stats_partial>(dim3(grid), dim3(PF_BLOCK), 0, st, g->ws, g->n_pad, g->n, first, g->sg, g->perm, g->perm_m, from_sym, g->n_chunks, part);
+    PF_HIP(hipGetLastError());
+    pfl::launch<k_vec_stats_finish>(dim3((unsigned)count), dim3(PF_WAVE), 0, st, part, g->n_chunks, fin);
     PF_HIP(hipGetLastError());
     double *d_params = nullptr, *d_out = nullptr;
     pf_free(st, g->final_vecs);
@@ -1972,16 +2012,21 @@
     VecStats* d_stats = reinterpret_cast<VecStats*>(d_params + 4 * (size_t)count);
     hipError_t e = pf_malloc(st, (void**)&d_out, sizeof(double) * (size_t)g->n * count);
     if (e == hipSuccess) {
-        k_vec_params<<<1, PF_WAVE, 0, st>>>(fin, count, minmax, d_params);
-        k_vec_apply<<<nblk(g->n), PF_BLOCK, 0, st>>>(g->ws, g->n_pad, g->n, first, count, g->sg, g->iperm, g->mrank, from_sym, d_params, d_out);
+        pfl::launch<k_vec_params>(dim3(1), dim3(PF_WAVE), 0, st, fin, count, minmax, d_params);
+        pfl::launch<k_vec_apply>(dim3(nblk(g->n)), dim3(PF_BLOCK), 0, st, g->ws, g->n_pad, g->n, first, count, g->sg, g->iperm, g->mrank, from_sym, d_params, d_out);
         e = hipGetLastError();
     }
-    if (e == hipSuccess) e = hipMemcpyAsync(d_stats, fin, sizeof(VecStats) * count, hipMemcpyDeviceToDevice, st);
-    if (e == hipSuccess) e = hipEventRecord(g->final_ready, st);
-    if (e == hipSuccess) e = hipStreamWaitEvent(ctx->copy_stream, g->final_ready, 0);
-    if (e == hipSuccess) e = hipMemcpyAsync(g->final_stats, d_stats, sizeof(VecStats) * count, hipMemcpyDeviceToHost, ctx->copy_stream);
-    if (e == hipSuccess) e = hipEventRecord(g->final_done, ctx->copy_stream);
+    if (e == hipSuccess) e = pfl::memcpy_async(st, d_stats, fin, sizeof(VecStats) * count, hipMemcpyDeviceToDevice);
+    if (e == hipSuccess) e = pfl::event_record(st, g->final_ready);
+    if (e == hipSuccess) {
+        hipStream_t cs = ctx->copy_stream;
+        hipEvent_t ready = g->final_ready;
+        pfl::call(cs, [=](hipStream_t s) { (void)hipStreamWaitEvent(s, ready, 0); });
+    }
+    if (e == hipSuccess) e = pfl::memcpy_async(ctx->copy_stream, g->final_stats, d_stats, sizeof(VecStats) * count, hipMemcpyDeviceToHost);
+    if (e == hipSuccess) e = pfl::event_record(ctx->copy_stream, g->final_done);
     if (e != hipSuccess) {
+        pfl::flush_self();
         (void)hipStreamSynchronize(ctx->copy_stream);
         pf_free(st, d_params);
         pf_free(st, d_out);
```
